# RaphaelHaddad/Real-Time-Brain-Inspired-Video-Memory

Measured on NVIDIA B200. Metric: queries_per_sec_top10_384d, higher is better.
Workload: dtype tf32

## Files before the change

### real-time-brain-inspired-video-memory_b200/csrc/api.cu

```cuda
#include "common.cuh"

#include <dlfcn.h>
#include <stdarg.h>
#include <stdlib.h>
#include <string.h>
#include <time.h>
#include <new>
#include <vector>

namespace vm {

static thread_local char g_err[512] = "";
void set_error(const char *fmt, ...)
{
    va_list ap;
    va_start(ap, fmt);
    vsnprintf(g_err, sizeof(g_err), fmt, ap);
    va_end(ap);
}

int k_convert_rows(const void *src, int src_dtype, void *dst, int dst_dtype, int64_t n, int dim, int ld, cudaStream_t st);
int k_row_inv_norms(const void *rows, int dtype, float *inv_norms, int64_t row0, int64_t n, int ld, int *extreme, cudaStream_t st,
                    const double *exact = nullptr);
int k_invalidate_rows(float *inv_norms, const int64_t *rows_dev, int64_t n, int64_t size, cudaStream_t st);
int k_normalize_queries(const void *q, int q_dtype, int nq, int nq_pad, int dim, int ld, float *out_f32, void *out_bf16,
                        int32_t *zero_me, uint32_t *zero_tab, int zero_tab_n, int tf32_round, int split, bool pdl, cudaStream_t st);
int k_synth_fill(void *rows, int dtype, uint64_t seed, int64_t row0, int64_t n, int dim, int ld, uint64_t dup_period,
                 cudaStream_t st);
int k_merge_candidates(const uint64_t *cand, int lists, int nq, int kp, uint64_t *merged, cudaStream_t st);

int k_slab_top(const SelectArgs &sa, int nq, int kp, uint64_t *merged, int *incomplete, cudaStream_t st);
int k_rescore(const RescoreArgs &a, cudaStream_t st, const int *incomplete);
int k_select_rescore(const SelectArgs &sa, const RescoreArgs &a, cudaStream_t st, bool pdl);
bool select_rescore_fits(int lists, int list_len, int kp, int dtype, int dim, int ld);
int k_collect_rescore(const uint64_t *buf, const int *cnt, int cap, const RescoreArgs &a, cudaStream_t st);
int k_exact(const ExactArgs &a, cudaStream_t st, bool pdl);
int k_merge_topk_lists(const void *idx, const void *score, const void *count, size_t stride_bytes, int lists, int nq, int k,
                       int64_t *out_idx, double *out_score, int32_t *out_count, cudaStream_t st);
int k_p2p_publish(void *flag, unsigned long long gen, cudaStream_t st);
int k_merge_topk_p2p(void *const *peers, int nranks, size_t slot_off, size_t flag_off, unsigned long long gen, int nq, int k,
                     int64_t *out_idx, double *out_score, int32_t *out_count, cudaStream_t st);
int k_merge_max_by_id(const int64_t *idx, const double *score, const int32_t *count, int nq, int k, int k2,
                      int64_t *out_idx, double *out_score, int32_t *out_count, cudaStream_t st);
int k_cosine_pairs(const void *a, const void *b, int dtype, int64_t n, int dim, int zero_rule, int sum_mode, double *out,
                   cudaStream_t st);
int k_pairs_above(int device, const void *x, int dtype, int64_t n, int dim, int ld, float threshold, int64_t cap,
                  int64_t *out_i, int64_t *out_j, float *out_score, int64_t *out_count, int part, int nparts, int flags,
                  cudaStream_t st);
int k_pairs_concat(const void *gathered, size_t per_rank_bytes, int64_t slot, const int64_t *counts, int nranks, int64_t cap,
                   int64_t *out_i, int64_t *out_j, float *out_score, int64_t *out_count, cudaStream_t st);

struct Arena;
int arena_create(Arena **out, int device, size_t max_bytes);
int arena_grow(Arena *a, size_t bytes);
void arena_destroy(Arena *a);
void *arena_base(const Arena *a);
size_t arena_mapped(const Arena *a);

static constexpr int MAXQ = 64;
static constexpr int MAXK = 64;
static constexpr int XCTAS = 148;
static constexpr int MAX_DEVICES = 64;
static constexpr int COLLECT_CAP = 4096;
static constexpr int FLAG_INTERNAL_CAPTURE = 1 << 30;

struct ResultBlock {
    int64_t *idx;
    double *score;
    int32_t *count;
    static ResultBlock at(void *base, int nq, int k)
    {
        char *b = (char *)base;
        return {(int64_t *)b, (double *)(b + (size_t)nq * k * 8), (int32_t *)(b + (size_t)nq * k * 16)};
    }
    ResultBlock from(int q0, int k) const { return {idx + (size_t)q0 * k, score + (size_t)q0 * k, count + q0}; }
};
static constexpr size_t result_bytes(int nq, int k) { return (size_t)nq * k * 16 + (size_t)nq * 4; }
static constexpr size_t packed_bytes(int nq, int k) { return (result_bytes(nq, k) + 7) & ~(size_t)7; }

static void unpack_to_host(const void *pack, int nq, int k, const ResultBlock &out)
{
    const ResultBlock p = ResultBlock::at(const_cast<void *>(pack), nq, k);
    memcpy(out.idx, p.idx, (size_t)nq * k * 8);
    memcpy(out.score, p.score, (size_t)nq * k * 8);
    memcpy(out.count, p.count, (size_t)nq * 4);
}

struct DeviceGuard {
    int prev = -1;
    bool ok = true;
    explicit DeviceGuard(int dev)
    {
        if (cudaGetDevice(&prev) != cudaSuccess) { ok = false; return; }
        if (prev != dev && cudaSetDevice(dev) != cudaSuccess) ok = false;
    }
    ~DeviceGuard() { if (prev >= 0) cudaSetDevice(prev); }
};

struct Buf {
    void *p = nullptr;
    size_t bytes = 0;
    int ensure(size_t need)
    {
        if (need <= bytes) return VM_OK;
        if (p) cudaFree(p);
        p = nullptr; bytes = 0;
        cudaError_t e = cudaMalloc(&p, need);
        if (e != cudaSuccess) { set_error("cudaMalloc(%zu) failed: %s", need, cudaGetErrorString(e)); return VM_ERR_OOM; }
        bytes = need;
        return VM_OK;
    }
    void release() { if (p) cudaFree(p); p = nullptr; bytes = 0; }
};

struct Workspace {
    bool ready = false;
    int lists_max = 0;
    Buf q_raw, q_f32, q_bf16, seed, cand, merged, o_idx, flags, col_thr, col_cnt, col_buf, xs, xr, xc, taken, gather_send, gather_recv, misc, ubuf, done, scnt, sel_inc;
    int32_t *h_uncert = nullptr;
    unsigned char *h_pack = nullptr;
    unsigned char *h_q = nullptr;
    void release()
    {
        Buf *all[] = {&q_raw, &q_f32, &q_bf16, &seed, &cand, &merged, &o_idx, &flags, &col_thr, &col_cnt, &col_buf, &xs, &xr, &xc, &taken,
                      &gather_send, &gather_recv, &misc, &ubuf, &done, &scnt, &sel_inc};
        for (Buf *b : all) b->release();
        if (h_uncert) cudaFreeHost(h_uncert);
        if (h_pack) cudaFreeHost(h_pack);
        if (h_q) cudaFreeHost(h_q);
        h_uncert = nullptr; h_pack = nullptr; h_q = nullptr;
        ready = false;
    }
};

}

using namespace vm;

struct vm_store {
    int device = 0, dim = 0, ld = 0, dtype = VM_F32, sm_count = 148;
    int64_t capacity = 0, size = 0;
    void *rows = nullptr;
    float *inv_norms = nullptr;
    double *rows_exact = nullptr;
    bool owns = false;
    Arena *ar_rows = nullptr, *ar_inv = nullptr, *ar_exact = nullptr;
    int64_t max_capacity = 0;
    const void *exact_rows() const { return rows_exact ? (const void *)rows_exact : (const void *)rows; }
    int exact_dtype() const { return rows_exact ? (int)VM_F64 : dtype; }
    int *extreme = nullptr;
    unsigned long long *cum = nullptr;
    int64_t n_batches = 0, n_queries = 0;
    int last_band_ctas = 0, last_band_nq = 0;
    Buf stage, stage_idx;
    Workspace ws;
    static constexpr int EV_RING = 64;
    cudaEvent_t evr[EV_RING][2] = {};
    int ev_next = 0;
    int ev_pending = 0;
    int ev_cur = -1;
    bool timed = false;
    struct GraphEntry {
        cudaGraphExec_t exec = nullptr;
        uint64_t version = 0;
        int nq = 0, k = 0, flags = 0, score_mode = 0, sum_mode = 0, q_dtype = 0;
        double min_score = 0.0;
        int64_t row_offset = 0;
        vm_topk_stats stats{};
    };
    GraphEntry graphs[4];
    int graph_next = 0;
    uint64_t version = 1;
    uint64_t seen_version = 0;
    int stable_calls = 0;
    cudaStream_t gstream = nullptr;
};

static constexpr size_t XCHG_SLOT_BYTES = (result_bytes(MAXQ, MAXK) + 255) & ~(size_t)255;
static constexpr size_t XCHG_FLAG_OFF = 2 * XCHG_SLOT_BYTES;
static constexpr size_t XCHG_BYTES = XCHG_FLAG_OFF + 256;

struct vm_comm {
    void *nccl = nullptr;
    int nranks = 1, rank = 0, device = 0;
    void *peer[16] = {};
    bool p2p = false;
    unsigned long long gen = 0;
    Buf pl_i, pl_j, pl_s, pl_cnt, pg_cnt, pg_send, pg_recv;
    int64_t *h_counts = nullptr;
};

struct Id128 { char b[128]; };
namespace {
struct NcclApi {
    void *h = nullptr;
    int (*GetUniqueId)(void *) = nullptr;
    int (*CommInitRank)(void **, int,  Id128, int) = nullptr;
    int (*AllGather)(const void *, void *, size_t, int, void *, cudaStream_t) = nullptr;
    int (*Broadcast)(const void *, void *, size_t, int, int, void *, cudaStream_t) = nullptr;
    int (*CommDestroy)(void *) = nullptr;
    const char *(*GetErrorString)(int) = nullptr;
};
}
static NcclApi g_nccl;

static int nccl_load()
{
    if (g_nccl.h) return VM_OK;
    void *h = dlopen("libnccl.so.2", RTLD_NOW | RTLD_GLOBAL);
    if (!h) h = dlopen("libnccl.so", RTLD_NOW | RTLD_GLOBAL);
    VM_REQUIRE(h, VM_ERR_NCCL, "cannot load libnccl.so.2: %s", dlerror());
    g_nccl.GetUniqueId = (int (*)(void *))dlsym(h, "ncclGetUniqueId");
    g_nccl.CommInitRank = (int (*)(void **, int, Id128, int))dlsym(h, "ncclCommInitRank");
    g_nccl.AllGather = (int (*)(const void *, void *, size_t, int, void *, cudaStream_t))dlsym(h, "ncclAllGather");
    g_nccl.Broadcast = (int (*)(const void *, void *, size_t, int, int, void *, cudaStream_t))dlsym(h, "ncclBroadcast");
    g_nccl.CommDestroy = (int (*)(void *))dlsym(h, "ncclCommDestroy");
    g_nccl.GetErrorString = (const char *(*)(int))dlsym(h, "ncclGetErrorString");
    VM_REQUIRE(g_nccl.GetUniqueId && g_nccl.CommInitRank && g_nccl.AllGather && g_nccl.Broadcast && g_nccl.CommDestroy, VM_ERR_NCCL,
               "libnccl lacks a required symbol");
    g_nccl.h = h;
    return VM_OK;
}
#define VM_NCCL_CHECK(expr)                                                                            \
    do {                                                                                               \
        int _r = (expr);                                                                               \
        if (_r != 0) {                                                                                 \
            set_error("%s failed: %s", #expr, g_nccl.GetErrorString ? g_nccl.GetErrorString(_r) : "?"); \
            return VM_ERR_NCCL;                                                                        \
        }                                                                                              \
    } while (0)

static int check_arch(int device, int *sm_count)
{
    cudaDeviceProp p;
    VM_CUDA_CHECK(cudaGetDeviceProperties(&p, device));
    VM_REQUIRE(p.major == 10, VM_ERR_UNSUPPORTED, "device %d is sm_%d%d; libvidmem is built for sm_100a only", device,
               p.major, p.minor);
    if (sm_count) *sm_count = p.multiProcessorCount;
    return VM_OK;
}

static int ws_prepare(vm_store *s)
{
    Workspace &w = s->ws;
    if (w.ready) return VM_OK;
    int lists = 2 * s->sm_count;
    w.lists_max = lists;
    int rc;
#define ENS(b, bytes) if ((rc = (b).ensure(bytes)) != VM_OK) return rc
    ENS(w.q_raw, (size_t)MAXQ * s->dim * 8);
    ENS(w.q_f32, (size_t)MAXQ * s->ld * 4);
    ENS(w.q_bf16, (size_t)2 * MAXQ * s->ld * 2);
    ENS(w.cand, (size_t)lists * MAXQ * (MAXK > SCAN_SLAB ? MAXK : SCAN_SLAB) * 8);
    ENS(w.merged, (size_t)MAXQ * MAXK * 8);
    ENS(w.o_idx, result_bytes(MAXQ, MAXK) + 64);
    ENS(w.flags, (size_t)(MAXQ + 2) * 4);
    ENS(w.seed, (size_t)(SEED_TAB_WORDS + 3 * MAXQ) * 4);
    ENS(w.ubuf, (size_t)MAXQ * SCAN_UNION_CAP * 8);
    ENS(w.done, 64);
    ENS(w.scnt, (size_t)256 * MAXQ * 4);
    ENS(w.sel_inc, (size_t)MAXQ * 4);
    VM_CUDA_CHECK(cudaMemset(w.done.p, 0, 64));
    ENS(w.col_thr, (size_t)MAXQ * 4);
    ENS(w.col_cnt, (size_t)MAXQ * 4);
    ENS(w.col_buf, (size_t)MAXQ * COLLECT_CAP * 8);
    ENS(w.xs, (size_t)XCTAS * MAXQ * MAXK * 8);
    ENS(w.xr, (size_t)XCTAS * MAXQ * MAXK * 4);
    ENS(w.xc, (size_t)XCTAS * MAXQ * 4);
    ENS(w.taken, (size_t)MAXQ * XCTAS * MAXK);
#undef ENS
    VM_CUDA_CHECK(cudaMallocHost((void **)&w.h_uncert, 64));
    VM_CUDA_CHECK(cudaMallocHost((void **)&w.h_pack, result_bytes(MAXQ, MAXK) + 64));
    VM_CUDA_CHECK(cudaMallocHost((void **)&w.h_q, (size_t)MAXQ * s->dim * 8));
    w.ready = true;
    return VM_OK;
}

static double scan_eps_stored(int kernel, int store_dtype, int dim, int split);
static double scan_eps(int kernel, int store_dtype, int dim, int split, bool shadow = false)
{
    const double base = scan_eps_stored(kernel, store_dtype, dim, split);
    if (!shadow) return base;
    return base + (store_dtype == VM_F32 ? 1.1920928955078125e-07 : 1.953125e-3 * 1.01);
}
static double scan_eps_stored(int kernel, int store_dtype, int dim, int split)
{
    const double u = 1.1920928955078125e-07;
    const double fp32_acc = (double)(dim + 16) * u;
    if (kernel == 1) return fp32_acc;
    if (store_dtype == VM_F32)
        return 9.765625e-4 + 4.8828125e-4 + 1e-6 + fp32_acc;
    if (!split) return 3.90625e-3 + fp32_acc;
    return 1.52587890625e-5 * 1.01 + (double)(dim + dim / 8 + 32) * u;
}

extern "C" int vm_version(void) { return VM_ABI_VERSION; }
extern "C" const char *vm_last_error(void) { return g_err; }

extern "C" int vm_device_info(int device, int *sm_count, int *cc_major, int *cc_minor, size_t *total_mem)
{
    cudaDeviceProp p;
    VM_CUDA_CHECK(cudaGetDeviceProperties(&p, device));
    if (sm_count) *sm_count = p.multiProcessorCount;
    if (cc_major) *cc_major = p.major;
    if (cc_minor) *cc_minor = p.minor;
    if (total_mem) *total_mem = p.totalGlobalMem;
    return VM_OK;
}

extern "C" int vm_ld(int dim) { return ld_for_dim(dim); }

static int store_new(vm_store **out, int device, int dim, int dtype, int64_t capacity)
{
    VM_REQUIRE(out, VM_ERR_BADARG, "out is NULL");
    VM_REQUIRE(dim >= 1 && dim <= 4096, VM_ERR_BADARG, "dim %d outside [1, 4096]", dim);
    VM_REQUIRE(dtype == VM_F32 || dtype == VM_BF16, VM_ERR_BADARG, "store dtype must be VM_F32 or VM_BF16");
    VM_REQUIRE(capacity >= 1 && capacity < 0xFFFFFFFFLL, VM_ERR_BADARG, "capacity %lld outside [1, 2^32-2]", (long long)capacity);
    int sms = 0;
    int rc = check_arch(device, &sms);
    if (rc != VM_OK) return rc;
    vm_store *s = new (std::nothrow) vm_store();
    VM_REQUIRE(s, VM_ERR_OOM, "host allocation failed");
    s->device = device; s->dim = dim; s->ld = ld_for_dim(dim); s->dtype = dtype; s->capacity = capacity; s->sm_count = sms;
    {
        DeviceGuard g(device);
        if (cudaMalloc((void **)&s->extreme, 4) != cudaSuccess || cudaMemset(s->extreme, 0, 4) != cudaSuccess ||
            cudaMalloc((void **)&s->cum, 64) != cudaSuccess || cudaMemset(s->cum, 0, 64) != cudaSuccess) {
            set_error("store allocation failed");
            vm_store_destroy(s);
            return VM_ERR_OOM;
        }
    }
    *out = s;
    return VM_OK;
}

extern "C" int vm_store_create(vm_store **out, int device, int dim, int dtype, int64_t capacity)
{
    int rc = store_new(out, device, dim, dtype, capacity);
    if (rc != VM_OK) return rc;
    vm_store *s = *out;
    DeviceGuard g(device);
    s->owns = true;
    size_t bytes = (size_t)capacity * s->ld * dtype_size(dtype);
    cudaError_t e = cudaMalloc(&s->rows, bytes);
    if (e == cudaSuccess) e = cudaMalloc((void **)&s->inv_norms, (size_t)capacity * 4);
    if (e != cudaSuccess) {
        set_error("store allocation of %zu bytes failed: %s", bytes, cudaGetErrorString(e));
        vm_store_destroy(s);
        *out = nullptr;
        return VM_ERR_OOM;
    }
    return VM_OK;
}

extern "C" int vm_store_create_exact(vm_store **out, int device, int dim, int shadow_dtype, int64_t capacity)
{
    int rc = vm_store_create(out, device, dim, shadow_dtype, capacity);
    if (rc != VM_OK) return rc;
    vm_store *s = *out;
    DeviceGuard g(device);
    const size_t bytes = (size_t)capacity * s->ld * 8;
    cudaError_t e = cudaMalloc((void **)&s->rows_exact, bytes);
    if (e != cudaSuccess) {
        set_error("store allocation of %zu bytes (binary64 rows) failed: %s", bytes, cudaGetErrorString(e));
        vm_store_destroy(s);
        *out = nullptr;
        return VM_ERR_OOM;
    }
    return VM_OK;
}

static int store_back(vm_store *s, int64_t capacity)
{
    int rc = arena_grow(s->ar_rows, (size_t)capacity * s->ld * dtype_size(s->dtype));
    if (rc == VM_OK) rc = arena_grow(s->ar_inv, (size_t)capacity * 4);
    if (rc == VM_OK && s->ar_exact) rc = arena_grow(s->ar_exact, (size_t)capacity * s->ld * 8);
    return rc;
}

extern "C" int vm_store_create_growable(vm_store **out, int device, int dim, int dtype, int exact, int64_t initial_capacity,
                                        int64_t max_capacity)
{
    VM_REQUIRE(initial_capacity >= 1 && max_capacity >= initial_capacity, VM_ERR_BADARG, "need 1 <= initial_capacity <= max_capacity");
    int rc = store_new(out, device, dim, dtype, max_capacity);
    if (rc != VM_OK) return rc;
    vm_store *s = *out;
    DeviceGuard g(device);
    s->max_capacity = max_capacity;
    s->capacity = initial_capacity;
    rc = arena_create(&s->ar_rows, device, (size_t)max_capacity * s->ld * dtype_size(dtype));
    if (rc == VM_OK) rc = arena_create(&s->ar_inv, device, (size_t)max_capacity * 4);
    if (rc == VM_OK && exact) rc = arena_create(&s->ar_exact, device, (size_t)max_capacity * s->ld * 8);
    if (rc == VM_OK) rc = store_back(s, initial_capacity);
    if (rc != VM_OK) { vm_store_destroy(s); *out = nullptr; return rc; }
    s->rows = arena_base(s->ar_rows);
    s->inv_norms = (float *)arena_base(s->ar_inv);
    if (exact) s->rows_exact = (double *)arena_base(s->ar_exact);
    return VM_OK;
}

extern "C" int vm_store_reserve(vm_store *s, int64_t capacity)
{
    VM_REQUIRE(s, VM_ERR_BADARG, "store is NULL");
    if (capacity <= s->capacity) return VM_OK;
    VM_REQUIRE(s->ar_rows, VM_ERR_STATE, "store is not growable (created over fixed buffers of %lld rows)", (long long)s->capacity);
    VM_REQUIRE(capacity <= s->max_capacity, VM_ERR_OVERFLOW, "capacity %lld exceeds the reserved maximum %lld", (long long)capacity,
               (long long)s->max_capacity);
    DeviceGuard g(s->device);
    int rc = store_back(s, capacity);
    if (rc != VM_OK) return rc;
    s->capacity = capacity;
    return VM_OK;
}

extern "C" int64_t vm_store_max_capacity(const vm_store *s) { return s ? (s->ar_rows ? s->max_capacity : s->capacity) : -1; }
extern "C" void *vm_store_rows_ptr(const vm_store *s) { return s ? s->rows : nullptr; }
extern "C" float *vm_store_inv_norms_ptr(const vm_store *s) { return s ? s->inv_norms : nullptr; }
extern "C" double *vm_store_rows_exact_ptr(const vm_store *s) { return s ? s->rows_exact : nullptr; }
extern "C" size_t vm_store_resident_bytes(const vm_store *s)
{
    if (!s) return 0;
    if (s->ar_rows) return arena_mapped(s->ar_rows) + arena_mapped(s->ar_inv) + (s->ar_exact ? arena_mapped(s->ar_exact) : 0);
    return (size_t)s->capacity * ((size_t)s->ld * (dtype_size(s->dtype) + (s->rows_exact ? 8 : 0)) + 4);
}

extern "C" int vm_store_attach_exact(vm_store **out, int device, int dim, int shadow_dtype, int64_t capacity, void *rows_dev,
                                     float *inv_norms_dev, double *rows_exact_dev)
{
    VM_REQUIRE(rows_exact_dev && ((uintptr_t)rows_exact_dev & 15) == 0, VM_ERR_BADARG, "binary64 rows buffer must be 16-byte aligned");
    int rc = vm_store_attach(out, device, dim, shadow_dtype, capacity, rows_dev, inv_norms_dev);
    if (rc != VM_OK) return rc;
    (*out)->rows_exact = rows_exact_dev;
    return VM_OK;
}

extern "C" int vm_store_attach(vm_store **out, int device, int dim, int dtype, int64_t capacity, void *rows_dev,
                               float *inv_norms_dev)
{
    VM_REQUIRE(rows_dev && inv_norms_dev, VM_ERR_BADARG, "attach needs device buffers");
    VM_REQUIRE(((uintptr_t)rows_dev & 127) == 0, VM_ERR_BADARG, "rows buffer must be 128-byte aligned");
    int rc = store_new(out, device, dim, dtype, capacity);
    if (rc != VM_OK) return rc;
    (*out)->rows = rows_dev;
    (*out)->inv_norms = inv_norms_dev;
    (*out)->owns = false;
    return VM_OK;
}

extern "C" int vm_store_destroy(vm_store *s)
{
    if (!s) return VM_OK;
    DeviceGuard g(s->device);
    cudaDeviceSynchronize();
    if (s->owns) { cudaFree(s->rows); cudaFree(s->inv_norms); if (s->rows_exact) cudaFree(s->rows_exact); }
    arena_destroy(s->ar_rows); arena_destroy(s->ar_inv); arena_destroy(s->ar_exact);
    if (s->extreme) cudaFree(s->extreme);
    if (s->cum) cudaFree(s->cum);
    s->stage.release(); s->stage_idx.release();
    s->ws.release();
    for (auto &pr : s->evr) { if (pr[0]) cudaEventDestroy(pr[0]); if (pr[1]) cudaEventDestroy(pr[1]); }
    for (auto &ge : s->graphs) if (ge.exec) cudaGraphExecDestroy(ge.exec);
    if (s->gstream) cudaStreamDestroy(s->gstream);
    delete s;
    return VM_OK;
}

extern "C" int64_t vm_store_size(const vm_store *s) { return s ? s->size : -1; }
extern "C" int64_t vm_store_capacity(const vm_store *s) { return s ? s->capacity : -1; }
extern "C" int vm_store_dim(const vm_store *s) { return s ? s->dim : -1; }
extern "C" int vm_store_ld(const vm_store *s) { return s ? s->ld : -1; }

static int store_write(vm_store *s, int64_t row0, const void *rows, int src_dtype, int src_mem, int64_t n, cudaStream_t st)
{
    VM_REQUIRE(src_dtype == VM_F32 || src_dtype == VM_BF16 || src_dtype == VM_F64, VM_ERR_BADARG, "bad source dtype");
    if (n == 0) return VM_OK;
    VM_REQUIRE(rows, VM_ERR_BADARG, "rows is NULL");
    DeviceGuard g(s->device);
    const void *src = rows;
    if (src_mem == VM_MEM_HOST) {
        size_t bytes = (size_t)n * s->dim * dtype_size(src_dtype);
        int rc = s->stage.ensure(bytes);
        if (rc != VM_OK) return rc;
        VM_CUDA_CHECK(cudaMemcpyAsync(s->stage.p, rows, bytes, cudaMemcpyHostToDevice, st));
        src = s->stage.p;
    }
    char *dst = (char *)s->rows + (size_t)row0 * s->ld * dtype_size(s->dtype);
    int rc = k_convert_rows(src, src_dtype, dst, s->dtype, n, s->dim, s->ld, st);
    if (rc != VM_OK) return rc;
    if (s->rows_exact) {
        rc = k_convert_rows(src, src_dtype, s->rows_exact + (size_t)row0 * s->ld, VM_F64, n, s->dim, s->ld, st);
        if (rc != VM_OK) return rc;
    }
    return k_row_inv_norms(s->rows, s->dtype, s->inv_norms, row0, row0 + n, s->ld, s->extreme, st, s->rows_exact);
}

extern "C" int vm_store_append(vm_store *s, const void *rows, int src_dtype, int src_mem, int64_t n, int64_t *first_row,
                               void *stream)
{
    VM_REQUIRE(s, VM_ERR_BADARG, "store is NULL");
    VM_REQUIRE(n >= 0, VM_ERR_BADARG, "n < 0");
    if (s->ar_rows && s->size + n > s->capacity) {
        const int64_t row_bytes = (int64_t)s->ld * (int64_t)(dtype_size(s->dtype) + (s->rows_exact ? 8 : 0)) + 4;
        const int64_t slack_rows = ((int64_t)256 << 20) / row_bytes + 1;
        int64_t want = s->size + n + slack_rows;
        if (want > s->max_capacity) want = s->max_capacity;
        if (want >= s->size + n) {
            int rc = vm_store_reserve(s, want);
            if (rc != VM_OK && want > s->size + n) rc = vm_store_reserve(s, s->size + n);
            if (rc != VM_OK) return rc;
        }
    }
    VM_REQUIRE(s->size + n <= s->capacity, VM_ERR_OVERFLOW, "append of %lld rows exceeds capacity %lld (size %lld)",
               (long long)n, (long long)s->capacity, (long long)s->size);
    int rc = store_write(s, s->size, rows, src_dtype, src_mem, n, (cudaStream_t)stream);
    if (rc != VM_OK) return rc;
    if (first_row) *first_row = s->size;
    s->size += n;
    ++s->version;
    return VM_OK;
}

extern "C" int vm_store_update(vm_store *s, int64_t row0, const void *rows, int src_dtype, int src_mem, int64_t n, void *stream)
{
    VM_REQUIRE(s, VM_ERR_BADARG, "store is NULL");
    VM_REQUIRE(row0 >= 0 && n >= 0 && row0 + n <= s->size, VM_ERR_BADARG, "update range [%lld, %lld) outside [0, %lld)",
               (long long)row0, (long long)(row0 + n), (long long)s->size);
    ++s->version;
    return store_write(s, row0, rows, src_dtype, src_mem, n, (cudaStream_t)stream);
}

extern "C" int vm_store_invalidate(vm_store *s, const int64_t *rows_host, int64_t n, void *stream)
{
    VM_REQUIRE(s, VM_ERR_BADARG, "store is NULL");
    if (n <= 0) return VM_OK;
    VM_REQUIRE(rows_host, VM_ERR_BADARG, "rows is NULL");
    DeviceGuard g(s->device);
    int rc = s->stage_idx.ensure((size_t)n * 8);
    if (rc != VM_OK) return rc;
    VM_CUDA_CHECK(cudaMemcpyAsync(s->stage_idx.p, rows_host, (size_t)n * 8, cudaMemcpyHostToDevice, (cudaStream_t)stream));
    ++s->version;
    return k_invalidate_rows(s->inv_norms, (const int64_t *)s->stage_idx.p, n, s->size, (cudaStream_t)stream);
}

extern "C" int vm_store_set_size(vm_store *s, int64_t n, int64_t recompute_from_row, void *stream)
{
    VM_REQUIRE(s, VM_ERR_BADARG, "store is NULL");
    VM_REQUIRE(n >= 0 && n <= s->capacity, VM_ERR_BADARG, "size %lld outside [0, capacity]", (long long)n);
    DeviceGuard g(s->device);
    s->size = n;
    ++s->version;
    if (recompute_from_row >= 0 && recompute_from_row < n) {
        if (s->rows_exact) {
            const int64_t r0 = recompute_from_row;
            int rc = k_convert_rows((const char *)s->rows + (size_t)r0 * s->ld * dtype_size(s->dtype), s->dtype,
                                    s->rows_exact + (size_t)r0 * s->ld, VM_F64, n - r0, s->ld, s->ld, (cudaStream_t)stream);
            if (rc != VM_OK) return rc;
        }
        return k_row_inv_norms(s->rows, s->dtype, s->inv_norms, recompute_from_row, n, s->ld, s->extreme, (cudaStream_t)stream, s->rows_exact);
    }
    return VM_OK;
}

extern "C" int vm_store_last_scan_ms(vm_store *s, float *ms)
{
    VM_REQUIRE(s && ms, VM_ERR_BADARG, "NULL argument");
    VM_REQUIRE(s->timed, VM_ERR_STATE, "no vm_topk call with VM_FLAG_TIMING has run the scan kernel yet");
    DeviceGuard g(s->device);
    VM_CUDA_CHECK(cudaEventSynchronize(s->evr[s->ev_cur][1]));
    VM_CUDA_CHECK(cudaEventElapsedTime(ms, s->evr[s->ev_cur][0], s->evr[s->ev_cur][1]));
    return VM_OK;
}

extern "C" int vm_store_avg_scan_ms(vm_store *s, float *ms, int *calls)
{
    VM_REQUIRE(s && ms, VM_ERR_BADARG, "NULL argument");
    VM_REQUIRE(s->timed && s->ev_pending > 0, VM_ERR_STATE, "no vm_topk call with VM_FLAG_TIMING since the last read");
    DeviceGuard g(s->device);
    VM_CUDA_CHECK(cudaEventSynchronize(s->evr[s->ev_cur][1]));
    double sum = 0.0;
    const int n = s->ev_pending;
    for (int i = 0; i < n; ++i) {
        const int slot = (s->ev_cur - i + 2 * vm_store::EV_RING) % vm_store::EV_RING;
        float t = 0.0f;
        VM_CUDA_CHECK(cudaEventElapsedTime(&t, s->evr[slot][0], s->evr[slot][1]));
        sum += t;
    }
    *ms = (float)(sum / n);
    if (calls) *calls = n;
    s->ev_pending = 0;
    return VM_OK;
}

extern "C" int vm_store_band_keys(vm_store *s, int nq_cap, int64_t *kept_per_query, int64_t *spilled_per_query, int *nq_out)
{
    VM_REQUIRE(s && kept_per_query && spilled_per_query, VM_ERR_BADARG, "NULL argument");
    VM_REQUIRE(s->ws.ready && s->last_band_ctas > 0, VM_ERR_STATE, "the last top-k call of this store was not a band-keeping tcgen05 scan");
    const int ctas = s->last_band_ctas, nq = s->last_band_nq;
    VM_REQUIRE(nq_cap >= nq, VM_ERR_BADARG, "room for %d queries needed", nq);
    DeviceGuard g(s->device);
    VM_CUDA_CHECK(cudaDeviceSynchronize());
    std::vector<int> sc((size_t)ctas * nq), uc(nq);
    VM_CUDA_CHECK(cudaMemcpy(sc.data(), s->ws.scnt.p, sc.size() * 4, cudaMemcpyDeviceToHost));
    VM_CUDA_CHECK(cudaMemcpy(uc.data(), (int *)s->ws.seed.p + SEED_TAB_WORDS + 2 * MAXQ, (size_t)nq * 4, cudaMemcpyDeviceToHost));
    for (int q = 0; q < nq; ++q) {
        int64_t k = 0;
        for (int c = 0; c < ctas; ++c) k += sc[(size_t)c * nq + q];
        kept_per_query[q] = k;
        spilled_per_query[q] = uc[q];
    }
    if (nq_out) *nq_out = nq;
    return VM_OK;
}

extern "C" int vm_store_read_counters(vm_store *s, vm_store_counters *out, int reset)
{
    VM_REQUIRE(s && out, VM_ERR_BADARG, "NULL argument");
    DeviceGuard g(s->device);
    unsigned long long h[8] = {0, 0, 0, 0, 0, 0, 0, 0};
    VM_CUDA_CHECK(cudaMemcpy(h, s->cum, sizeof(h), cudaMemcpyDeviceToHost));
    out->batches = s->n_batches; out->queries = s->n_queries;
    out->uncertified = (int64_t)h[0]; out->band_settled = (int64_t)h[1]; out->collect_settled = (int64_t)h[2];
    out->full_rescans = (int64_t)h[3];
    out->bound_violations = (int64_t)h[4];
    if (reset) {
        VM_CUDA_CHECK(cudaMemset(s->cum, 0, sizeof(h)));
        s->n_batches = 0; s->n_queries = 0;
    }
    return VM_OK;
}

extern "C" int vm_store_clear(vm_store *s)
{
    VM_REQUIRE(s, VM_ERR_BADARG, "store is NULL");
    DeviceGuard g(s->device);
    VM_CUDA_CHECK(cudaMemset(s->extreme, 0, 4));
    s->size = 0;
    ++s->version;
    return VM_OK;
}

extern "C" size_t vm_topk_packed_bytes(int nq, int k) { return nq > 0 && k > 0 ? packed_bytes(nq, k) : 0; }

namespace {
struct TopkCall {
    vm_store *s;
    const void *queries;
    int q_dtype, q_mem, nq, k;
    double min_score;
    int score_mode, sum_mode, flags;
    int64_t row_offset;
    ResultBlock d;
    cudaStream_t st;
    vm_topk_stats *stats;
    ResultBlock h = {};
};
}

static cudaError_t wait_stream(cudaStream_t st, const vm_store *s = nullptr)
{
    static const bool block = [] { const char *e = getenv("VIDMEM_SYNC"); return e && !strcmp(e, "block"); }();
    if (block) return cudaStreamSynchronize(st);
    if (s) {
        const double est_us = (double)s->size * s->ld * (double)dtype_size(s->dtype) / 6.5e6;
        if (est_us > 400.0) {
            struct timespec ts;
            const long ns = (long)(est_us * 750.0);
            ts.tv_sec = ns / 1000000000L; ts.tv_nsec = ns % 1000000000L;
            nanosleep(&ts, nullptr);
        }
    }
    for (;;) {
        const cudaError_t e = cudaStreamQuery(st);
        if (e != cudaErrorNotReady) return e;
#if defined(__x86_64__) || defined(__i386__)
        __builtin_ia32_pause();
#endif
    }
}

static int pack_out_enqueue(const TopkCall &c)
{
    VM_CUDA_CHECK(cudaMemcpyAsync(c.s->ws.h_pack, c.d.idx, result_bytes(c.nq, c.k), cudaMemcpyDeviceToHost, c.st));
    return VM_OK;
}

static int tc_list_len(int k) { return k <= 16 ? 32 : (k <= 48 ? 64 : 0); }

static int queries_per_pass(const vm_store *s, int k, int flags)
{
    const int kp = tc_list_len(k);
    if (!(flags & (VM_FLAG_FORCE_EXACT | VM_FLAG_FORCE_SIMT)) && kp)
        for (int nq = 64; nq >= 16; nq -= 16)
            if (scan_tc_supported(s->dtype, s->dim, nq, kp)) return nq;
    return MAXQ;
}

static int topk_batch(const TopkCall &c)
{
    vm_store *s = c.s;
    Workspace &w = s->ws;
    cudaStream_t st = c.st;
    const void *q_dev = c.queries;
    if (c.q_mem == VM_MEM_HOST) {
        const size_t qbytes = (size_t)c.nq * s->dim * dtype_size(c.q_dtype);
        memcpy(w.h_q, c.queries, qbytes);
        VM_CUDA_CHECK(cudaMemcpyAsync(w.q_raw.p, w.h_q, qbytes, cudaMemcpyHostToDevice, st));
        q_dev = w.q_raw.p;
    }
    FinalizeArgs fin{c.k, c.min_score, c.score_mode, c.row_offset, c.d.idx, c.d.score, c.d.count};
    ExactArgs ex{s->exact_rows(), s->inv_norms, s->exact_dtype(), s->ld, s->dim, s->size, q_dev, c.q_dtype, c.nq, c.k, c.sum_mode,
                 nullptr, (double *)w.xs.p, (uint32_t *)w.xr.p, (int32_t *)w.xc.p, (uint8_t *)w.taken.p, XCTAS, fin, s->cum,
                 (int *)w.done.p};
    if (!(c.flags & FLAG_INTERNAL_CAPTURE)) { ++s->n_batches; s->n_queries += c.nq; }
    int launches = 0;
    if (c.stats) { c.stats->uncertified = 0; c.stats->candidates = 0; c.stats->scan_ctas = 0; }

    int kernel = 0, kp = 0;
    if (!(c.flags & VM_FLAG_FORCE_EXACT) && s->size > 0) {
        int kp_tc = tc_list_len(c.k);
        int kp_simt = c.k <= 24 ? (c.k + 8 > 16 ? ((c.k + 8 + 7) & ~7) : 16) : 0;
        bool tc_ok = kp_tc > 0 && scan_tc_supported(s->dtype, s->dim, c.nq, kp_tc);
        bool want_tc = !(c.flags & VM_FLAG_FORCE_SIMT);
        if (want_tc && tc_ok) { kernel = 2; kp = kp_tc; }
        else if (kp_simt > 0) { kernel = 1; kp = kp_simt; }
        else if (tc_ok) { kernel = 2; kp = kp_tc; }
    }
    if (kernel == 0) {
        int rc = k_exact(ex, st, false);
        if (rc != VM_OK) return rc;
        launches += 2;
        if (c.h.idx) {
            if ((rc = pack_out_enqueue(c)) != VM_OK) return rc;
            VM_CUDA_CHECK(wait_stream(st, s));
            unpack_to_host(w.h_pack, c.nq, c.k, c.h);
        }
        if (c.stats) { c.stats->scan_kernel = 0; c.stats->scan_launches += launches; }
        return VM_OK;
    }

    int nq_pad = kernel == 2 ? ((c.nq + 15) & ~15) : c.nq;
    const int split = (kernel == 2 && s->dtype == VM_BF16 && !(c.flags & VM_FLAG_NO_SPLIT) &&
                       (c.nq <= 48 || (c.flags & VM_FLAG_SPLIT)) && scan_tc_supported(s->dtype, s->dim, c.nq, kp, 1)) ? 1 : 0;
#ifdef VIDMEM_NO_GRAPH_PDL
    const bool pdl = !(c.flags & (VM_FLAG_TIMING | FLAG_INTERNAL_CAPTURE));
#else
    const bool pdl = !(c.flags & VM_FLAG_TIMING);
#endif
    int rc = k_normalize_queries(q_dev, c.q_dtype, c.nq, nq_pad, s->dim, s->ld, (float *)w.q_f32.p,
                                 (kernel == 2 && s->dtype == VM_BF16) ? w.q_bf16.p : nullptr,
                                 (int32_t *)w.flags.p + c.nq, kernel == 2 ? (uint32_t *)w.seed.p : nullptr,
                                 kernel == 2 ? (int)(w.seed.bytes / 4) : 0, kernel == 2 && s->dtype == VM_F32, split, pdl, st);
    if (rc != VM_OK) return rc;
    ++launches;
    const double eps = scan_eps(kernel, s->dtype, s->dim, split, s->rows_exact != nullptr);

    ScanArgs a;
    ScanInfo sinfo;
    a.rows = s->rows; a.inv_norms = s->inv_norms; a.dtype = s->dtype; a.n = s->size; a.dim = s->dim; a.ld = s->ld;
    a.queries = (const float *)w.q_f32.p; a.nq = c.nq; a.kp = kp; a.cand = (uint64_t *)w.cand.p; a.stream = st;
    a.slab = (uint64_t *)w.cand.p; a.scnt = (int *)w.scnt.p;
    a.ubuf = (uint64_t *)w.ubuf.p; a.ucnt = (int *)w.seed.p + SEED_TAB_WORDS + 2 * MAXQ; a.ucap = SCAN_UNION_CAP;
    a.band = nextafterf((float)(2.0 * eps), INFINITY); a.ksel = c.k; a.split = split; a.pdl = pdl;
    const bool timing = (c.flags & VM_FLAG_TIMING) != 0;
    if (timing) {
        s->ev_cur = s->ev_next;
        s->ev_next = (s->ev_next + 1) % vm_store::EV_RING;
        if (s->ev_pending < vm_store::EV_RING) ++s->ev_pending;
        if (!s->evr[s->ev_cur][0]) { VM_CUDA_CHECK(cudaEventCreate(&s->evr[s->ev_cur][0])); VM_CUDA_CHECK(cudaEventCreate(&s->evr[s->ev_cur][1])); }
        VM_CUDA_CHECK(cudaEventRecord(s->evr[s->ev_cur][0], st));
    }
    if (kernel == 1) {
        int64_t need = (s->size + 31) / 32;
        a.ctas = (int)imin64(need, 2 * s->sm_count);
        rc = launch_scan_simt(a);
        launches += (c.nq + 7) / 8;
    } else {
        int64_t tiles = (s->size + 127) / 128;
        a.ctas = (int)imin64(tiles, s->sm_count);

        a.dump = tiles <= s->sm_count && tiles * SCAN_DUMP_TILE <= SCAN_DUMP_MAX_KEYS &&
                 (size_t)tiles * c.nq * SCAN_DUMP_TILE * 8 <= w.cand.bytes &&
                 select_rescore_fits((int)tiles, SCAN_DUMP_TILE, kp, s->exact_dtype(), s->dim, s->ld);
        s->last_band_ctas = a.dump ? 0 : a.ctas; s->last_band_nq = c.nq;
        rc = launch_scan_tc(a, s->dtype == VM_BF16 ? w.q_bf16.p : w.q_f32.p, (uint32_t *)w.seed.p, (int *)w.flags.p + c.nq + 1, nullptr, &sinfo);
        launches += 1;
    }
    if (rc != VM_OK) return rc;
    if (timing) { VM_CUDA_CHECK(cudaEventRecord(s->evr[s->ev_cur][1], st)); s->timed = true; }

    int32_t *flags = (int32_t *)w.flags.p;
    int32_t *uncert = flags + c.nq;
    RescoreArgs rs{(const uint64_t *)w.merged.p, kp, s->exact_rows(), s->inv_norms, s->exact_dtype(), s->ld, s->dim, s->size, q_dev,
                   c.q_dtype, c.nq, eps, c.sum_mode, fin, flags, uncert, s->extreme,
                   kernel == 2 ? (float *)w.col_thr.p : nullptr, s->cum};
    SelectArgs sel;
    const bool union_src = kernel == 2 && !a.dump;
    if (union_src) {
        sel.slab = a.slab; sel.scnt = a.scnt; sel.ctas = a.ctas; sel.ubuf = a.ubuf; sel.ucnt = a.ucnt; sel.ucap = a.ucap;
        sel.seed_tab = a.ctas <= 256 ? (const uint32_t *)w.seed.p : nullptr; sel.nq_pad = nq_pad; sel.ksel = c.k; sel.band = a.band;
    } else { sel.cand = a.cand; sel.lists = a.ctas; sel.list_len = a.dump ? SCAN_DUMP_TILE : kp; sel.complete = a.dump ? 1 : 0; }
    rc = k_select_rescore(sel, rs, st, pdl);
    if (rc == VM_ERR_UNSUPPORTED && !a.dump) {
        if (union_src) rc = k_slab_top(sel, c.nq, kp, (uint64_t *)w.merged.p, (int *)w.sel_inc.p, st);
        else rc = k_merge_candidates(a.cand, a.ctas, c.nq, kp, (uint64_t *)w.merged.p, st);
        if (rc != VM_OK) return rc;
        rc = k_rescore(rs, st, union_src ? (const int *)w.sel_inc.p : nullptr);
        ++launches;
    }
    if (rc != VM_OK) return rc;
    launches += 1;

    ex.flags = flags;
    int n_uncert = 0, n_full = -1;
    auto run_collect = [&]() -> int {
        VM_CUDA_CHECK(cudaMemsetAsync(w.col_cnt.p, 0, (size_t)c.nq * 4, st));
        ScanCollect sc{(const float *)w.col_thr.p, (uint64_t *)w.col_buf.p, (int *)w.col_cnt.p, COLLECT_CAP, uncert};
        int r = launch_scan_tc(a, s->dtype == VM_BF16 ? w.q_bf16.p : w.q_f32.p, nullptr, nullptr, &sc);
        if (r != VM_OK) return r;
        return k_collect_rescore((const uint64_t *)w.col_buf.p, (const int *)w.col_cnt.p, COLLECT_CAP, rs, st);
    };
    if (c.flags & VM_FLAG_ASYNC) {
        if (c.flags & FLAG_INTERNAL_CAPTURE) {
            VM_CUDA_CHECK(cudaMemcpyAsync(w.h_uncert, uncert, 4, cudaMemcpyDeviceToHost, st));
        } else {
            rc = k_exact(ex, st, pdl);
            if (rc != VM_OK) return rc;
            launches += 1;
        }
        n_uncert = -1;
    } else {
        VM_CUDA_CHECK(cudaMemcpyAsync(w.h_uncert, uncert, 4, cudaMemcpyDeviceToHost, st));
        if (c.h.idx && (rc = pack_out_enqueue(c)) != VM_OK) return rc;
        VM_CUDA_CHECK(wait_stream(st, s));
        n_uncert = *w.h_uncert;
        n_full = 0;
        if (n_uncert > 0) {
            int left = n_uncert;
            if (kernel == 2) {
                if ((rc = run_collect()) != VM_OK) return rc;
                launches += 2;
                VM_CUDA_CHECK(cudaMemcpyAsync(w.h_uncert, uncert, 4, cudaMemcpyDeviceToHost, st));
                VM_CUDA_CHECK(wait_stream(st, s));
                left = *w.h_uncert;
            }
            n_full = left;
            if (left > 0) {
                rc = k_exact(ex, st, false);
                if (rc != VM_OK) return rc;
                launches += 1;
            }
            if (c.h.idx) {
                if ((rc = pack_out_enqueue(c)) != VM_OK) return rc;
                VM_CUDA_CHECK(wait_stream(st, s));
            }
        }
        if (c.h.idx) unpack_to_host(w.h_pack, c.nq, c.k, c.h);
    }
    if (c.stats) {
        c.stats->scan_kernel = kernel;
        c.stats->scan_launches += launches;
        c.stats->uncertified += n_uncert > 0 ? n_uncert : 0;
        c.stats->full_rescans = n_full;
        c.stats->candidates = kp;
        c.stats->scan_ctas = a.ctas;
        c.stats->scan_stages = kernel == 2 ? sinfo.stages : 0;
        c.stats->scan_variant = kernel == 2 ? sinfo.variant : 0;
    }
    return VM_OK;
}

static constexpr int GRAPH_SKIPPED = 1;

static int graph_capture(const TopkCall &c, vm_store::GraphEntry *ge)
{
    vm_store *s = c.s;
    Workspace &w = s->ws;
    vm_topk_stats cs{};
    TopkCall cc = c;
    cc.queries = w.q_raw.p; cc.q_mem = VM_MEM_DEVICE; cc.flags |= VM_FLAG_ASYNC | FLAG_INTERNAL_CAPTURE;
    cc.d = ResultBlock::at(w.o_idx.p, c.nq, c.k); cc.st = s->gstream; cc.stats = &cs;
    const size_t qbytes = (size_t)c.nq * s->dim * dtype_size(c.q_dtype);
    cudaGraph_t graph = nullptr;
    VM_CUDA_CHECK(cudaStreamBeginCapture(s->gstream, cudaStreamCaptureModeRelaxed));
    int rc = VM_OK;
    if (cudaMemcpyAsync(w.q_raw.p, w.h_q, qbytes, cudaMemcpyHostToDevice, s->gstream) != cudaSuccess) rc = VM_ERR_CUDA;
    if (rc == VM_OK) rc = topk_batch(cc);
    if (rc == VM_OK && cudaMemcpyAsync(w.h_pack, cc.d.idx, result_bytes(c.nq, c.k), cudaMemcpyDeviceToHost, s->gstream) != cudaSuccess)
        rc = VM_ERR_CUDA;
    cudaError_t ce = cudaStreamEndCapture(s->gstream, &graph);
    if (rc != VM_OK || ce != cudaSuccess || !graph) {
        if (graph) cudaGraphDestroy(graph);
        if (rc == VM_OK) { set_error("graph capture failed: %s", cudaGetErrorString(ce)); rc = VM_ERR_CUDA; }
        cudaGetLastError();
        return rc;
    }
    ce = cudaGraphInstantiate(&ge->exec, graph, 0);
    cudaGraphDestroy(graph);
    if (ce != cudaSuccess) { ge->exec = nullptr; set_error("cudaGraphInstantiate failed: %s", cudaGetErrorString(ce)); return VM_ERR_CUDA; }
    ge->version = s->version; ge->nq = c.nq; ge->k = c.k; ge->flags = c.flags; ge->score_mode = c.score_mode;
    ge->sum_mode = c.sum_mode; ge->q_dtype = c.q_dtype; ge->min_score = c.min_score; ge->row_offset = c.row_offset; ge->stats = cs;
    return VM_OK;
}

static int topk_graph(const TopkCall &c, int out_mem, bool sharded, const ResultBlock &out)
{
    vm_store *s = c.s;
    Workspace &w = s->ws;
    static const bool no_graph = getenv("VIDMEM_NO_GRAPH") != nullptr;
    if (s->seen_version == s->version) { if (s->stable_calls < 1 << 20) ++s->stable_calls; }
    else { s->seen_version = s->version; s->stable_calls = 0; }
    if (no_graph || s->stable_calls < 16 || sharded || c.st != nullptr || c.q_mem != VM_MEM_HOST || out_mem != VM_MEM_HOST ||
        (c.flags & (VM_FLAG_ASYNC | VM_FLAG_TIMING | VM_FLAG_FORCE_EXACT)) || s->size == 0 ||
        c.nq > queries_per_pass(s, c.k, c.flags))
        return GRAPH_SKIPPED;
    if (!s->gstream) VM_CUDA_CHECK(cudaStreamCreate(&s->gstream));
    vm_store::GraphEntry *ge = nullptr;
    for (auto &e : s->graphs)
        if (e.exec && e.version == s->version && e.nq == c.nq && e.k == c.k && e.flags == c.flags && e.score_mode == c.score_mode &&
            e.sum_mode == c.sum_mode && e.q_dtype == c.q_dtype && e.row_offset == c.row_offset &&
            memcmp(&e.min_score, &c.min_score, sizeof(double)) == 0) { ge = &e; break; }
    if (!ge) {
        ge = &s->graphs[s->graph_next];
        s->graph_next = (s->graph_next + 1) & 3;
        if (ge->exec) { cudaGraphExecDestroy(ge->exec); ge->exec = nullptr; }
        const int rc = graph_capture(c, ge);
        if (rc != VM_OK) return rc;
    }
    memcpy(w.h_q, c.queries, (size_t)c.nq * s->dim * dtype_size(c.q_dtype));
    ++s->n_batches; s->n_queries += c.nq;
    VM_CUDA_CHECK(cudaGraphLaunch(ge->exec, s->gstream));
    VM_CUDA_CHECK(wait_stream(s->gstream, s));
    const int uncertified = ge->stats.scan_kernel != 0 ? *w.h_uncert : 0;
    if (uncertified > 0) {
        TopkCall rerun = c;
        rerun.d = ResultBlock::at(w.o_idx.p, c.nq, c.k); rerun.st = s->gstream; rerun.h = out;
        return topk_batch(rerun);
    }
    unpack_to_host(w.h_pack, c.nq, c.k, out);
    if (c.stats) { *c.stats = ge->stats; c.stats->uncertified = uncertified; }
    return VM_OK;
}

static size_t xchg_slot_off(unsigned long long gen) { return (size_t)(gen & 1) * XCHG_SLOT_BYTES; }

static ResultBlock batch_dest(vm_store *s, const vm_comm *comm, bool sharded, int out_mem, const ResultBlock &out, int nb, int k)
{
    if (sharded && comm->p2p) return ResultBlock::at((char *)comm->peer[comm->rank] + xchg_slot_off(comm->gen), nb, k);
    if (sharded) return ResultBlock::at(s->ws.gather_send.p, nb, k);
    return out_mem == VM_MEM_DEVICE ? out : ResultBlock::at(s->ws.o_idx.p, nb, k);
}

static int exchange_merge(vm_store *s, vm_comm *comm, int nb, int k, const ResultBlock &m, cudaStream_t st)
{
    if (comm->p2p) {
        const int rc = k_p2p_publish((char *)comm->peer[comm->rank] + XCHG_FLAG_OFF, comm->gen, st);
        if (rc != VM_OK) return rc;
        return k_merge_topk_p2p(comm->peer, comm->nranks, xchg_slot_off(comm->gen), XCHG_FLAG_OFF, comm->gen, nb, k, m.idx, m.score,
                                m.count, st);
    }
    const Workspace &w = s->ws;
    VM_NCCL_CHECK(g_nccl.AllGather(w.gather_send.p, w.gather_recv.p, packed_bytes(nb, k),  0, comm->nccl, st));
    const ResultBlock r = ResultBlock::at(w.gather_recv.p, nb, k);
    return k_merge_topk_lists(r.idx, r.score, r.count, packed_bytes(nb, k), comm->nranks, nb, k, m.idx, m.score, m.count, st);
}

static int topk_common(vm_store *s, vm_comm *comm, int64_t row_offset, const void *queries, int q_dtype, int q_mem, int nq,
                       int k, double min_score, int score_mode, int sum_mode, int flags, int64_t *out_idx,
                       double *out_score, int32_t *out_count, int out_mem, vm_topk_stats *stats, void *stream)
{
    VM_REQUIRE(s, VM_ERR_BADARG, "store is NULL");
    VM_REQUIRE(nq >= 0, VM_ERR_BADARG, "nq < 0");
    VM_REQUIRE(k >= 1 && k <= MAXK, VM_ERR_BADARG, "k %d outside [1, %d]", k, MAXK);
    VM_REQUIRE(q_dtype == VM_F32 || q_dtype == VM_BF16 || q_dtype == VM_F64, VM_ERR_BADARG, "bad query dtype");
    VM_REQUIRE(score_mode == VM_SCORE_RAW || score_mode == VM_SCORE_NEO4J, VM_ERR_BADARG, "bad score_mode");
    VM_REQUIRE(sum_mode == VM_SUM_NAIVE || sum_mode == VM_SUM_NEUMAIER, VM_ERR_BADARG, "bad sum_mode");
    VM_REQUIRE(!(flags & VM_FLAG_ASYNC) || (out_mem == VM_MEM_DEVICE && q_mem == VM_MEM_DEVICE), VM_ERR_BADARG,
               "VM_FLAG_ASYNC needs device queries and device outputs");
    if (stats) memset(stats, 0, sizeof(*stats));
    if (nq == 0) return VM_OK;
    VM_REQUIRE(queries && out_idx && out_score && out_count, VM_ERR_BADARG, "NULL buffer");
    DeviceGuard g(s->device);
    VM_REQUIRE(g.ok, VM_ERR_CUDA, "cannot select device %d", s->device);
    int rc = ws_prepare(s);
    if (rc != VM_OK) return rc;
    const bool sharded = comm && comm->nranks > 1;
    const ResultBlock out{out_idx, out_score, out_count};
    const TopkCall call{s, queries, q_dtype, q_mem, nq, k, min_score, score_mode, sum_mode, flags, row_offset, {}, (cudaStream_t)stream,
                        stats};
    if ((rc = topk_graph(call, out_mem, sharded, out)) != GRAPH_SKIPPED) return rc;

    Workspace &w = s->ws;
    const int bq = queries_per_pass(s, k, flags);
    for (int q0 = 0; q0 < nq; q0 += bq) {
        const int nb = nq - q0 < bq ? nq - q0 : bq;
        const ResultBlock out_b = out.from(q0, k);
        if (sharded && comm->p2p) {
            ++comm->gen;
        } else if (sharded) {
            if ((rc = w.gather_send.ensure(packed_bytes(nb, k))) != VM_OK) return rc;
            if ((rc = w.gather_recv.ensure(packed_bytes(nb, k) * comm->nranks)) != VM_OK) return rc;
        }
        TopkCall c = call;
        c.queries = (const char *)queries + (size_t)q0 * s->dim * dtype_size(q_dtype);
        c.nq = nb;
        c.d = batch_dest(s, comm, sharded, out_mem, out_b, nb, k);
        if (out_mem == VM_MEM_HOST) {
            if (sharded) c.flags |= VM_FLAG_ASYNC;
            else c.h = out_b;
        }
        if ((rc = topk_batch(c)) != VM_OK) return rc;
        if (!sharded) continue;
        const ResultBlock ws = ResultBlock::at(w.o_idx.p, nb, k);
        if ((rc = exchange_merge(s, comm, nb, k, out_mem == VM_MEM_DEVICE ? out_b : ws, c.st)) != VM_OK) return rc;
        if (stats) stats->scan_launches += 2;
        if (out_mem == VM_MEM_HOST) {
            VM_CUDA_CHECK(cudaMemcpyAsync(w.h_pack, ws.idx, result_bytes(nb, k), cudaMemcpyDeviceToHost, c.st));
            VM_CUDA_CHECK(wait_stream(c.st, s));
            unpack_to_host(w.h_pack, nb, k, out_b);
        }
    }
    return VM_OK;
}

extern "C" int vm_topk(vm_store *s, const void *queries, int q_dtype, int q_mem, int nq, int k, double min_score,
                       int score_mode, int sum_mode, int flags, int64_t *out_idx, double *out_score, int32_t *out_count,
                       int out_mem, vm_topk_stats *stats, void *stream)
{
    return topk_common(s, nullptr, 0, queries, q_dtype, q_mem, nq, k, min_score, score_mode, sum_mode, flags, out_idx,
                       out_score, out_count, out_mem, stats, stream);
}

extern "C" int vm_topk_sharded(vm_store *s, vm_comm *comm, int64_t row_offset, const void *queries, int q_dtype, int q_mem,
                               int nq, int k, double min_score, int score_mode, int sum_mode, int flags, int64_t *out_idx,
                               double *out_score, int32_t *out_count, int out_mem, vm_topk_stats *stats, void *stream)
{
    VM_REQUIRE(comm, VM_ERR_BADARG, "comm is NULL");
    return topk_common(s, comm, row_offset, queries, q_dtype, q_mem, nq, k, min_score, score_mode, sum_mode, flags, out_idx,
                       out_score, out_count, out_mem, stats, stream);
}

extern "C" int vm_merge_topk_lists(int device, const int64_t *idx_dev, const double *score_dev, const int32_t *count_dev,
                                   int nlists, int nq, int k, int64_t *out_idx_dev, double *out_score_dev,
                                   int32_t *out_count_dev, void *stream)
{
    VM_REQUIRE(idx_dev && score_dev && count_dev && out_idx_dev && out_score_dev && out_count_dev, VM_ERR_BADARG, "NULL buffer");
    VM_REQUIRE(nlists >= 1 && nq >= 1 && k >= 1, VM_ERR_BADARG, "bad shape");
    DeviceGuard g(device);
    size_t stride = (size_t)nq * k * 8;
    VM_REQUIRE(device >= 0 && device < MAX_DEVICES, VM_ERR_BADARG, "device index %d outside [0, %d)", device, MAX_DEVICES);
    static thread_local Buf cnt_wide_dev[MAX_DEVICES];
    Buf &cnt_wide = cnt_wide_dev[device];
    int rc = cnt_wide.ensure(stride * nlists);
    if (rc != VM_OK) return rc;
    VM_CUDA_CHECK(cudaMemcpy2DAsync(cnt_wide.p, stride, count_dev, (size_t)nq * 4, (size_t)nq * 4, nlists,
                                    cudaMemcpyDeviceToDevice, (cudaStream_t)stream));
    return k_merge_topk_lists(idx_dev, score_dev, cnt_wide.p, stride, nlists, nq, k, out_idx_dev, out_score_dev,
                              out_count_dev, (cudaStream_t)stream);
}

extern "C" int vm_merge_topk_packed(int device, const void *packed_dev, int nlists, int nq, int k, int64_t *out_idx_dev,
                                    double *out_score_dev, int32_t *out_count_dev, void *stream)
{
    VM_REQUIRE(packed_dev && out_idx_dev && out_score_dev && out_count_dev, VM_ERR_BADARG, "NULL buffer");
    VM_REQUIRE(nlists >= 1 && nq >= 1 && k >= 1, VM_ERR_BADARG, "bad shape");
    DeviceGuard g(device);
    const ResultBlock r = ResultBlock::at(const_cast<void *>(packed_dev), nq, k);
    return k_merge_topk_lists(r.idx, r.score, r.count, packed_bytes(nq, k), nlists, nq, k, out_idx_dev, out_score_dev,
                              out_count_dev, (cudaStream_t)stream);
}

extern "C" int vm_merge_max_by_id(int device, const int64_t *idx_dev, const double *score_dev, const int32_t *count_dev,
                                  int nq, int k, int k2, int64_t *out_idx_dev, double *out_score_dev, int32_t *out_count_dev,
                                  void *stream)
{
    VM_REQUIRE(idx_dev && score_dev && count_dev && out_idx_dev && out_score_dev && out_count_dev, VM_ERR_BADARG, "NULL buffer");
    VM_REQUIRE(nq >= 1 && k >= 1 && k2 >= 1, VM_ERR_BADARG, "bad shape");
    DeviceGuard g(device);
    return k_merge_max_by_id(idx_dev, score_dev, count_dev, nq, k, k2, out_idx_dev, out_score_dev, out_count_dev,
                             (cudaStream_t)stream);
}

extern "C" int vm_cosine_pairs(int device, const void *a, const void *b, int dtype, int mem, int64_t n, int dim, int zero_rule,
                               int sum_mode, double *out, int out_mem, void *stream)
{
    VM_REQUIRE(n >= 0 && dim >= 0, VM_ERR_BADARG, "bad shape");
    VM_REQUIRE(dtype == VM_F32 || dtype == VM_F64, VM_ERR_BADARG, "dtype must be VM_F32 or VM_F64");
    VM_REQUIRE(zero_rule >= 0 && zero_rule <= 2, VM_ERR_BADARG, "zero_rule %d outside [0, 2]", zero_rule);
    if (n == 0) return VM_OK;
    VM_REQUIRE(a && b && out, VM_ERR_BADARG, "NULL buffer");
    int rc = check_arch(device, nullptr);
    if (rc != VM_OK) return rc;
    DeviceGuard g(device);
    cudaStream_t st = (cudaStream_t)stream;
    VM_REQUIRE(device >= 0 && device < MAX_DEVICES, VM_ERR_BADARG, "device index %d outside [0, %d)", device, MAX_DEVICES);
    static thread_local Buf scratch[MAX_DEVICES][3];
    Buf &da = scratch[device][0], &db = scratch[device][1], &dout = scratch[device][2];
    size_t bytes = (size_t)n * dim * dtype_size(dtype);
    const void *pa = a, *pb = b;
    if (mem == VM_MEM_HOST) {
        if ((rc = da.ensure(bytes ? bytes : 8)) != VM_OK || (rc = db.ensure(bytes ? bytes : 8)) != VM_OK) return rc;
        VM_CUDA_CHECK(cudaMemcpyAsync(da.p, a, bytes, cudaMemcpyHostToDevice, st));
        VM_CUDA_CHECK(cudaMemcpyAsync(db.p, b, bytes, cudaMemcpyHostToDevice, st));
        pa = da.p; pb = db.p;
    }
    double *po = out;
    if (out_mem == VM_MEM_HOST) {
        if ((rc = dout.ensure((size_t)n * 8)) != VM_OK) return rc;
        po = (double *)dout.p;
    }
    rc = k_cosine_pairs(pa, pb, dtype, n, dim, zero_rule, sum_mode, po, st);
    if (rc != VM_OK) return rc;
    if (out_mem == VM_MEM_HOST) {
        VM_CUDA_CHECK(cudaMemcpyAsync(out, po, (size_t)n * 8, cudaMemcpyDeviceToHost, st));
        VM_CUDA_CHECK(cudaStreamSynchronize(st));
    }
    return VM_OK;
}

extern "C" int vm_pairs_above(int device, const void *x_dev, int dtype, int64_t n, int dim, float threshold, int64_t cap,
                              int64_t *out_i_dev, int64_t *out_j_dev, float *out_score_dev, int64_t *out_count_dev, int part,
                              int nparts, int flags, void *stream)
{
    VM_REQUIRE(x_dev && out_count_dev, VM_ERR_BADARG, "NULL buffer");
    VM_REQUIRE(cap == 0 || (out_i_dev && out_j_dev && out_score_dev), VM_ERR_BADARG, "NULL output with cap > 0");
    VM_REQUIRE(dtype == VM_F32 || dtype == VM_BF16, VM_ERR_BADARG, "dtype must be VM_F32 or VM_BF16");
    VM_REQUIRE(n >= 0 && n < (1LL << 31), VM_ERR_BADARG, "n outside [0, 2^31)");
    VM_REQUIRE(dim >= 1 && dim <= 4096, VM_ERR_BADARG, "dim outside [1, 4096]");
    VM_REQUIRE(nparts >= 1 && part >= 0 && part < nparts, VM_ERR_BADARG, "bad part/nparts");
    int rc = check_arch(device, nullptr);
    if (rc != VM_OK) return rc;
    DeviceGuard g(device);
    return k_pairs_above(device, x_dev, dtype, n, dim, ld_for_dim(dim), threshold, cap, out_i_dev, out_j_dev, out_score_dev,
                         out_count_dev, part, nparts, flags, (cudaStream_t)stream);
}

extern "C" int vm_pairs_above_sharded(vm_comm *comm, void *x_dev, int dtype, int64_t n, int dim, float threshold, int64_t cap,
                                      int64_t *out_i_dev, int64_t *out_j_dev, float *out_score_dev, int64_t *out_count_dev,
                                      int root, int flags, void *stream)
{
    VM_REQUIRE(comm, VM_ERR_BADARG, "comm is NULL");
    VM_REQUIRE(x_dev && out_count_dev, VM_ERR_BADARG, "NULL buffer");
    VM_REQUIRE(cap >= 1 && out_i_dev && out_j_dev && out_score_dev, VM_ERR_BADARG, "cap < 1 or NULL output");
    VM_REQUIRE(dtype == VM_F32 || dtype == VM_BF16, VM_ERR_BADARG, "dtype must be VM_F32 or VM_BF16");
    VM_REQUIRE(n >= 0 && n < (1LL << 31), VM_ERR_BADARG, "n outside [0, 2^31)");
    VM_REQUIRE(dim >= 1 && dim <= 4096, VM_ERR_BADARG, "dim outside [1, 4096]");
    VM_REQUIRE(root >= -1 && root < comm->nranks, VM_ERR_BADARG, "root %d outside [-1, %d)", root, comm->nranks);
    int rc = check_arch(comm->device, nullptr);
    if (rc != VM_OK) return rc;
    DeviceGuard g(comm->device);
    cudaStream_t st = (cudaStream_t)stream;
    const int G = comm->nranks, ld = ld_for_dim(dim);
    if (root >= 0 && G > 1 && n > 0)
        VM_NCCL_CHECK(g_nccl.Broadcast(x_dev, x_dev, (size_t)n * ld * dtype_size(dtype),  0, root, comm->nccl, st));
#define ENS(b, bytes) if ((rc = (b).ensure(bytes)) != VM_OK) return rc
    ENS(comm->pl_i, (size_t)cap * 8); ENS(comm->pl_j, (size_t)cap * 8); ENS(comm->pl_s, (size_t)cap * 4);
    ENS(comm->pl_cnt, 8); ENS(comm->pg_cnt, (size_t)G * 8);
    if (!comm->h_counts) VM_CUDA_CHECK(cudaMallocHost((void **)&comm->h_counts, 16 * 8));
    rc = k_pairs_above(comm->device, x_dev, dtype, n, dim, ld, threshold, cap, (int64_t *)comm->pl_i.p, (int64_t *)comm->pl_j.p,
                       (float *)comm->pl_s.p, (int64_t *)comm->pl_cnt.p, comm->rank, G, 0, st);
    if (rc != VM_OK) return rc;
    VM_NCCL_CHECK(g_nccl.AllGather(comm->pl_cnt.p, comm->pg_cnt.p, 8,  0, comm->nccl, st));
    int64_t slot = cap;
// ... 98 lines not shown
```

### real-time-brain-inspired-video-memory_b200/csrc/common.cuh

```cuda
#pragma once
#include <cuda_runtime.h>
#include <cuda_bf16.h>
#include <stdint.h>
#include <stdio.h>
#include <math.h>
#include <utility>
#include "../../include/vidmem.h"

namespace vm {

void set_error(const char *fmt, ...);
#define VM_CUDA_CHECK(expr)                                                                      \
    do {                                                                                         \
        cudaError_t _e = (expr);                                                                 \
        if (_e != cudaSuccess) {                                                                 \
            vm::set_error("%s failed: %s (%s:%d)", #expr, cudaGetErrorString(_e), __FILE__, __LINE__); \
            return VM_ERR_CUDA;                                                                  \
        }                                                                                        \
    } while (0)
#define VM_REQUIRE(cond, code, ...)          \
    do {                                     \
        if (!(cond)) {                       \
            vm::set_error(__VA_ARGS__);      \
            return (code);                   \
        }                                    \
    } while (0)

__device__ __forceinline__ void pdl_wait() { asm volatile("griddepcontrol.wait;" ::: "memory"); }
__device__ __forceinline__ void pdl_launch_dependents() { asm volatile("griddepcontrol.launch_dependents;" ::: "memory"); }

template <typename... KArgs, typename... Args>
static inline cudaError_t launch_pdl(void (*kernel)(KArgs...), dim3 grid, dim3 block, size_t smem, cudaStream_t st, bool pdl,
                                     Args &&...args)
{
    cudaLaunchConfig_t cfg = {};
    cfg.gridDim = grid; cfg.blockDim = block; cfg.dynamicSmemBytes = smem; cfg.stream = st;
    cudaLaunchAttribute at[1];
    at[0].id = cudaLaunchAttributeProgrammaticStreamSerialization;
    at[0].val.programmaticStreamSerializationAllowed = 1;
    cfg.attrs = at;
    cfg.numAttrs = pdl ? 1 : 0;
    return cudaLaunchKernelEx(&cfg, kernel, std::forward<Args>(args)...);
}

template <auto Kernel>
static inline cudaError_t max_smem_once(int bytes)
{
    static bool set[64] = {};
    int dev = 0;
    cudaError_t e = cudaGetDevice(&dev);
    if (e != cudaSuccess || set[dev & 63]) return e;
    e = cudaFuncSetAttribute(Kernel, cudaFuncAttributeMaxDynamicSharedMemorySize, bytes);
    if (e == cudaSuccess) set[dev & 63] = true;
    return e;
}

__host__ __device__ __forceinline__ uint32_t f32_ordered(float f)
{
#ifdef __CUDA_ARCH__
    uint32_t b = __float_as_uint(f);
#else
    uint32_t b;
    memcpy(&b, &f, 4);
#endif
    return (b & 0x80000000u) ? ~b : (b | 0x80000000u);
}
__host__ __device__ __forceinline__ float f32_from_ordered(uint32_t o)
{
    uint32_t b = (o & 0x80000000u) ? (o & 0x7FFFFFFFu) : ~o;
#ifdef __CUDA_ARCH__
    return __uint_as_float(b);
#else
    float f;
    memcpy(&f, &b, 4);
    return f;
#endif
}
__host__ __device__ __forceinline__ uint64_t make_key(float score, uint32_t row)
{
    return ((uint64_t)f32_ordered(score) << 32) | (uint64_t)(0xFFFFFFFFu - row);
}
__host__ __device__ __forceinline__ uint32_t key_row(uint64_t k) { return 0xFFFFFFFFu - (uint32_t)(k & 0xFFFFFFFFu); }
__host__ __device__ __forceinline__ float key_score(uint64_t k) { return f32_from_ordered((uint32_t)(k >> 32)); }

static constexpr int SEED_TAB_WORDS = 256 * 64;
#ifdef __CUDACC__
__device__ __forceinline__ float seed_select(const uint32_t *seed_tab, int G, int nq_pad, int q, int k, int lane)
{
    uint32_t vals[8];
#pragma unroll
    for (int t = 0; t < 8; ++t) {
        const int i = lane + 32 * t;
        vals[t] = i < G ? __ldcg(seed_tab + (size_t)i * nq_pad + q) : 0u;
    }
    uint32_t prefix = 0;
    int need = k;
    for (int bit = 31; bit >= 16; --bit) {
        const uint32_t hi = bit == 31 ? 0u : (0xFFFFFFFFu << (bit + 1));
        int cnt = 0;
#pragma unroll
        for (int t = 0; t < 8; ++t) cnt += ((vals[t] & hi) == prefix && ((vals[t] >> bit) & 1u)) ? 1 : 0;
        const int tot = __reduce_add_sync(0xffffffffu, cnt);
        if (tot >= need) prefix |= 1u << bit;
        else need -= tot;
    }
    float sd = f32_from_ordered(prefix);
    if (!(sd > -INFINITY) || G < k) sd = -INFINITY;
    return sd;
}

__device__ __forceinline__ float band_floor(float L, float band)
{
    if (!(L > -INFINITY)) return -INFINITY;
    const float t = __fsub_rd(L, band);
    return nextafterf(t, -INFINITY);
}

#endif

struct RefSum {
    double s, c;
    __device__ __forceinline__ void init() { s = 0.0; c = 0.0; }
    template <bool NEUMAIER>
    __device__ __forceinline__ void add(double x)
    {
        double t = __dadd_rn(s, x);
        if (NEUMAIER) {
            const bool big = fabs(s) >= fabs(x);
            const double hi = big ? s : x, lo = big ? x : s;
            c = __dadd_rn(c, __dadd_rn(__dadd_rn(hi, -t), lo));
        }
        s = t;
    }
    template <bool NEUMAIER>
    __device__ __forceinline__ void add_block(const double (&x)[8])
    {
        double t[8];
        t[0] = __dadd_rn(s, x[0]);
#pragma unroll
        for (int u = 1; u < 8; ++u) t[u] = __dadd_rn(t[u - 1], x[u]);
        if (NEUMAIER) {
#pragma unroll
            for (int u = 0; u < 8; ++u) {
                const double prev = u ? t[u - 1] : s;
                const bool big = fabs(prev) >= fabs(x[u]);
                const double hi = big ? prev : x[u], lo = big ? x[u] : prev;
                c = __dadd_rn(c, __dadd_rn(__dadd_rn(hi, -t[u]), lo));
            }
        }
        s = t[7];
    }
    template <bool NEUMAIER>
    __device__ __forceinline__ double result() const
    {
        double r = s;
        if (NEUMAIER && c != 0.0 && isfinite(c)) r = __dadd_rn(r, c);
        return r;
    }
};

template <bool NEUMAIER, typename F>
__device__ __forceinline__ void ref_sum_range(RefSum &acc, int lo, int hi, F prod)
{
    int i = lo;
    for (; i + 8 <= hi; i += 8) {
        double x[8];
#pragma unroll
        for (int u = 0; u < 8; ++u) x[u] = prod(i + u);
        acc.add_block<NEUMAIER>(x);
    }
    for (; i < hi; ++i) acc.add<NEUMAIER>(prod(i));
}

__device__ __forceinline__ float load_as_float(const float *p, int64_t i) { return p[i]; }
__device__ __forceinline__ float load_as_float(const __nv_bfloat16 *p, int64_t i) { return __bfloat162float(p[i]); }
__device__ __forceinline__ double load_elem(const float *p, int64_t i) { return (double)p[i]; }
__device__ __forceinline__ double load_elem(const __nv_bfloat16 *p, int64_t i) { return (double)__bfloat162float(p[i]); }
__device__ __forceinline__ double load_elem(const double *p, int64_t i) { return p[i]; }
__device__ __forceinline__ double load_as_double(const void *p, int dtype, int64_t i)
{
    if (dtype == VM_F32) return (double)((const float *)p)[i];
    if (dtype == VM_BF16) return (double)__bfloat162float(((const __nv_bfloat16 *)p)[i]);
    return ((const double *)p)[i];
}

static inline int64_t imin64(int64_t a, int64_t b) { return a < b ? a : b; }
static inline int ld_for_dim(int dim) { return (dim + 7) & ~7; }
static inline size_t dtype_size(int dt) { return dt == VM_F32 ? 4 : dt == VM_BF16 ? 2 : 8; }

struct ScanArgs {
    const void *rows;
    const float *inv_norms;
    int dtype;
    int64_t n;
    int dim, ld;
    const float *queries;
    int nq;
    int kp;
    uint64_t *cand;
    int ctas;
    cudaStream_t stream;
    int dump = 0;
    uint64_t *slab = nullptr;
    int *scnt = nullptr;
    uint64_t *ubuf = nullptr;
    int *ucnt = nullptr;
    int ucap = 0;
    float band = 0.0f;
    int ksel = 0;
    int split = 0;
    bool pdl = false;
};
static constexpr int SCAN_UNION_CAP = 16384;
static constexpr int SCAN_SLAB = 128;
static constexpr int SELECT_KEY_CAP = 4096;
static constexpr int SCAN_DUMP_TILE = 128;
static constexpr int SCAN_DUMP_MAX_KEYS = 9472;
int launch_scan_simt(const ScanArgs &a);
int scan_simt_max_queries();
struct ScanCollect {
    const float *thr;
    uint64_t *buf;
    int *cnt;
    int cap;
    const int *pending;
};
struct ScanInfo { int stages = 0, variant = 0; };
int launch_scan_tc(const ScanArgs &a, const void *queries_store_dtype, uint32_t *seed_tab, int *seed_ctr,
                   const ScanCollect *sc = nullptr, ScanInfo *info = nullptr);
bool scan_tc_supported(int dtype, int dim, int nq, int kp, int split = 0);


struct FinalizeArgs {
    int k;
    double min_score;
    int score_mode;
    int64_t row_offset;
    int64_t *out_idx;
    double *out_score;
    int32_t *out_count;
};
struct RescoreArgs {
    const uint64_t *merged;
    int kp;
    const void *rows;
    const float *inv_norms;
    int dtype, ld, dim;
    int64_t n_rows;
    const void *queries;
    int q_dtype, nq;
    double eps;
    int sum_mode;
    FinalizeArgs fin;
    int32_t *flags, *uncertified_count;
    const int *extreme;
    float *collect_thr;
    unsigned long long *cum = nullptr;
};
struct SelectArgs {
    const uint64_t *cand = nullptr;
    int lists = 0, list_len = 0;
    int complete = 0;
    const uint64_t *slab = nullptr;
    const int *scnt = nullptr;
    int ctas = 0;
    const uint64_t *ubuf = nullptr;
    const int *ucnt = nullptr;
    int ucap = 0;
    const uint32_t *seed_tab = nullptr;
    int nq_pad = 0, ksel = 0;
    float band = 0.0f;
};
struct ExactArgs {
    const void *rows;
    const float *inv_norms;
    int dtype, ld, dim;
    int64_t n;
    const void *queries;
    int q_dtype, nq, k, sum_mode;
    int32_t *flags;
    double *xlist_score;
    uint32_t *xlist_row;
    int32_t *xlist_cnt;
    uint8_t *taken;
    int ctas;
    FinalizeArgs fin;
    unsigned long long *cum = nullptr;
    int *done_ctr = nullptr;
};

}
```

### real-time-brain-inspired-video-memory_b200/csrc/scan_tc.cu

```cuda
#include "tc_common.cuh"

namespace vm {
using namespace tc;

static constexpr int TC_BLOCK_M = 128;
static constexpr int TC_STAGE_BYTES = TC_BLOCK_M * 128;
static constexpr int TC_ACC = 8;
static constexpr int TC_THREADS_SVC = 288;
static constexpr int TC_THREADS = 192;
static constexpr int TC_TMEM_COLS = 512;
static constexpr int TC_MAX_STAGES = 8;

struct CollectArgs {
    const float *thr;
    uint64_t *buf;
    int *cnt;
    int cap;
    const int *pending;
};

struct BandArgs {
    uint64_t *slab;
    int *scnt;
    uint64_t *ubuf;
    int *ucnt;
    int ucap;
    float band;
    int ksel;
    int use_seed;
};

struct TcLayout {
    int nq_pad, KB, stages, split;
    uint32_t off_b, off_a, off_tauf, off_lcnt, off_cmax, off_wmax, off_flags, off_bars, off_tmem, total;
};

static TcLayout make_layout(int dtype, int ld, int nq, int split = 0)
{
    TcLayout L{};
    const int es = dtype == VM_F32 ? 4 : 2;
    L.nq_pad = (nq + 15) & ~15;
    L.KB = (ld * es + 127) / 128;
    L.split = (split && dtype == VM_BF16) ? 1 : 0;
    uint32_t o = 0;
    L.off_b = o; o += (uint32_t)L.KB * L.nq_pad * 128 * (L.split ? 2 : 1);
    const uint32_t epi = (uint32_t)L.nq_pad * (4 + 4 + 4 + 16) + 64 + 8 * (2 * TC_MAX_STAGES + 1 + 2 * TC_ACC) + 16;
    int64_t room = 227 * 1024 - 2048 - (int64_t)o - epi;
    L.stages = (int)(room / TC_STAGE_BYTES);
    if (L.stages > TC_MAX_STAGES) L.stages = TC_MAX_STAGES;
    if (L.stages < 0) L.stages = 0;
    L.off_a = o; o += (uint32_t)L.stages * TC_STAGE_BYTES;
    L.off_tauf = o; o += (uint32_t)L.nq_pad * 4;
    L.off_lcnt = o; o += (uint32_t)L.nq_pad * 4;
    L.off_cmax = o; o += (uint32_t)L.nq_pad * 4;
    L.off_wmax = o; o += (uint32_t)L.nq_pad * 16;
    L.off_flags = o; o += 64;
    L.off_bars = o; o += 8 * (2 * TC_MAX_STAGES + 1 + 2 * TC_ACC);
    L.off_tmem = o; o += 16;
    L.total = o + 1024;
#ifdef VIDMEM_AB_SMEMPAD
    if (L.total < 220 * 1024) L.total = 220 * 1024;
#endif
    return L;
}

__device__ __forceinline__ uint32_t own_kth_score(const uint64_t *slab, int n, int k, int lane)
{
    constexpr int PER = SCAN_SLAB / 32;
    uint32_t vals[PER];
#pragma unroll
    for (int t = 0; t < PER; ++t) {
        const int i = lane + 32 * t;
        vals[t] = i < n ? (uint32_t)(__ldcg(slab + i) >> 32) : 0u;
    }
    uint32_t prefix = 0;
    int need = k;
    for (int bit = 31; bit >= 12; --bit) {
        const uint32_t hi = bit == 31 ? 0u : (0xFFFFFFFFu << (bit + 1));
        int cnt = 0;
#pragma unroll
        for (int t = 0; t < PER; ++t) cnt += ((vals[t] & hi) == prefix && ((vals[t] >> bit) & 1u)) ? 1 : 0;
        const int tot = __reduce_add_sync(0xffffffffu, cnt);
        if (tot >= need) prefix |= 1u << bit;
        else need -= tot;
    }
    int ge = 0;
#pragma unroll
    for (int t = 0; t < PER; ++t) ge += (vals[t] != 0u && vals[t] >= prefix) ? 1 : 0;
    ge = __reduce_add_sync(0xffffffffu, ge);
    return (ge >= k && prefix != 0u) ? prefix : 0u;
}

template <bool TF32, bool DUMP, bool SPLIT>
__global__ void __launch_bounds__(DUMP ? TC_THREADS : TC_THREADS_SVC, 1)
scan_tc_kernel(const __grid_constant__ CUtensorMap tmA, const __grid_constant__ CUtensorMap tmB,
               const float *__restrict__ inv_norms, int64_t n, int num_tiles, int nq, TcLayout L, uint64_t *__restrict__ dump_keys,
               uint32_t *__restrict__ seed_tab, int *__restrict__ seed_ctr, CollectArgs col, BandArgs ub, int svc_sleep)
{
    const bool collect = !DUMP && col.thr != nullptr;
#ifndef VIDMEM_AB_NOPDL
    pdl_launch_dependents();
#endif
    if (collect) {
        pdl_wait();
        if (*col.pending == 0) return;
    }

    extern __shared__ __align__(16) uint8_t smem_raw[];
    uint8_t *base = smem_raw + ((1024u - (smem_u32(smem_raw) & 1023u)) & 1023u);
    uint8_t *sB = base + L.off_b;
    uint8_t *sA = base + L.off_a;
    float *tauf = (float *)(base + L.off_tauf);
    int *lcnt = (int *)(base + L.off_lcnt);
    uint32_t *cmax = (uint32_t *)(base + L.off_cmax);
    uint32_t *wmax = (uint32_t *)(base + L.off_wmax);
    volatile int *s_done = (volatile int *)(base + L.off_flags);
    uint64_t *bars = (uint64_t *)(base + L.off_bars);
    uint64_t *full = bars, *empty = bars + TC_MAX_STAGES, *qfull = bars + 2 * TC_MAX_STAGES;
    uint64_t *tfull = qfull + 1, *tempty = tfull + TC_ACC;
    uint32_t *tmem_slot = (uint32_t *)(base + L.off_tmem);

    const int warp = __shfl_sync(0xffffffffu, threadIdx.x >> 5, 0);
    const int lane = threadIdx.x & 31;
    const int nq_pad = L.nq_pad, KB = L.KB, stages = L.stages;
    constexpr int ELEMS = TF32 ? 32 : 64;

    if (warp == 0 && lane == 0) {
        tma_prefetch_desc(&tmA);
        tma_prefetch_desc(&tmB);
        for (int s = 0; s < stages; ++s) { mbar_init(&full[s], 1); mbar_init(&empty[s], 1); }
        mbar_init(qfull, 1);
        for (int a = 0; a < TC_ACC; ++a) { mbar_init(&tfull[a], 1); mbar_init(&tempty[a], 4); }
        fence_barrier_init();
    }
    if (warp == 1) tmem_alloc(tmem_slot, TC_TMEM_COLS);
#ifndef VIDMEM_AB_NOPDL
    if (!collect) pdl_wait();
#endif
    if (warp >= 2 && warp < 6) {
        const int e = threadIdx.x - 64;
        if (e < nq_pad) {
            lcnt[e] = 0;
            cmax[e] = 0u;
            tauf[e] = collect ? (e < nq ? col.thr[e] : INFINITY) : (e < nq ? -INFINITY : INFINITY);
        }
        if (e < 2) s_done[e] = 0;
    }
    tc_fence_before();
    __syncthreads();
    tc_fence_after();
    const uint32_t tmem_base = *tmem_slot;
    uint32_t *gbound = seed_tab ? seed_tab + SEED_TAB_WORDS : nullptr;

    if (warp == 0) {
        if (elect_one()) {
            constexpr int QPARTS = SPLIT ? 2 : 1;
            mbar_arrive_expect_tx(qfull, (uint32_t)(KB * QPARTS) * nq_pad * 128);
            for (int part = 0; part < QPARTS; ++part)
                for (int kb = 0; kb < KB; ++kb)
                    tma_load_2d(&tmB, qfull, sB + (size_t)(part * KB + kb) * nq_pad * 128, kb * ELEMS, part * nq_pad, L2_EVICT_LAST);
        }
        __syncwarp();
        int stage = 0;
        uint32_t phase = 0;
        for (int tile = blockIdx.x; tile < num_tiles; tile += gridDim.x) {
            for (int kb = 0; kb < KB; ++kb) {
                mbar_wait(&empty[stage], phase ^ 1);
                if (elect_one()) {
                    mbar_arrive_expect_tx(&full[stage], TC_STAGE_BYTES);
                    tma_load_2d(&tmA, &full[stage], sA + (size_t)stage * TC_STAGE_BYTES, kb * ELEMS, tile * TC_BLOCK_M, L2_EVICT_FIRST);
                }
                __syncwarp();
                if (++stage == stages) { stage = 0; phase ^= 1; }
            }
        }
    } else if (warp == 1) {
        const uint32_t idesc = make_idesc(TF32 ? 2u : 1u, TC_BLOCK_M, (uint32_t)nq_pad);
        mbar_wait(qfull, 0);
        tc_fence_after();
        int stage = 0, acc = 0;
        uint32_t phase = 0, acc_phase = 0;
        const uint64_t da0 = make_smem_desc_sw128(smem_u32(sA)), db0 = make_smem_desc_sw128(smem_u32(sB));
        const uint32_t kb_step = (uint32_t)(nq_pad * 128) >> 4, lo_step = (uint32_t)(KB * nq_pad * 128) >> 4;
        for (int tile = blockIdx.x; tile < num_tiles; tile += gridDim.x) {
            mbar_wait(&tempty[acc], acc_phase ^ 1);
            tc_fence_after();
            const uint32_t d_tmem = tmem_base + (uint32_t)(acc * nq_pad);
            for (int kb = 0; kb < KB; ++kb) {
                mbar_wait(&full[stage], phase);
                tc_fence_after();
                if (elect_one()) {
                    const uint64_t da = da0 + (uint64_t)((uint32_t)stage * (TC_STAGE_BYTES >> 4));
                    const uint64_t db = db0 + (uint64_t)((uint32_t)kb * kb_step);
#pragma unroll
                    for (int j = 0; j < 4; ++j) {
                        umma<TF32>(d_tmem, da + 2 * j, db + 2 * j, idesc, (uint32_t)((kb | j) != 0));
                        if constexpr (SPLIT) umma<TF32>(d_tmem, da + 2 * j, db + lo_step + 2 * j, idesc, 1u);
                    }
                    umma_commit(&empty[stage]);
                    if (kb == KB - 1) umma_commit(&tfull[acc]);
                }
                __syncwarp();
                if (++stage == stages) { stage = 0; phase ^= 1; }
            }
            if (++acc == TC_ACC) { acc = 0; acc_phase ^= 1; }
        }
    } else if (warp < 6) {
        const int e = threadIdx.x - 64;
        const int quad = warp & 3;
        const int row_in_tile = quad * 32 + lane;
        int acc = 0;
        uint32_t acc_phase = 0;
        if constexpr (DUMP) {
            for (int tile = blockIdx.x; tile < num_tiles; tile += gridDim.x) {
                const int64_t r = (int64_t)tile * TC_BLOCK_M + row_in_tile;
                const float iv = r < n ? __ldg(inv_norms + r) : -1.0f;
                mbar_wait(&tfull[acc], acc_phase);
                tc_fence_after();
                const uint32_t taddr = tmem_base + ((uint32_t)(quad * 32) << 16) + (uint32_t)(acc * nq_pad);
                uint64_t *out = dump_keys + (int64_t)tile * nq * TC_BLOCK_M + row_in_tile;
                for (int c = 0; c < nq_pad; c += 16) {
                    uint32_t v[16];
                    tmem_ld16(taddr + c, v);
                    tmem_ld_wait();
#pragma unroll
                    for (int j = 0; j < 16; ++j)
                        if (c + j < nq)
                            out[(int64_t)(c + j) * TC_BLOCK_M] = iv >= 0.0f ? make_key(__uint_as_float(v[j]) * iv, (uint32_t)r) : 0ull;
                }
                tc_fence_before();
                __syncwarp();
                if (lane == 0) mbar_arrive(&tempty[acc]);
                if (++acc == TC_ACC) { acc = 0; acc_phase ^= 1; }
            }
        } else {
        if (ub.use_seed && !collect) {
            const int64_t row0 = (int64_t)blockIdx.x * TC_BLOCK_M + row_in_tile;
            const float inv0 = row0 < n ? __ldg(inv_norms + row0) : -1.0f;
            mbar_wait(&tfull[0], 0);
            tc_fence_after();
            const uint32_t taddr0 = tmem_base + ((uint32_t)(quad * 32) << 16);
            for (int c = 0; c < nq_pad; c += 16) {
                uint32_t v[16];
                tmem_ld16(taddr0 + c, v);
                tmem_ld_wait();
#pragma unroll
                for (int j = 0; j < 16; ++j) {
                    const float sc = inv0 >= 0.0f ? __uint_as_float(v[j]) * inv0 : -INFINITY;
                    const uint32_t mx = __reduce_max_sync(0xffffffffu, f32_ordered(sc));
                    if (lane == 0) wmax[(warp - 2) * nq_pad + c + j] = mx;
                }
            }
            named_bar_sync(1, 128);
            if (e < nq_pad) {
                uint32_t m = wmax[e];
#pragma unroll
                for (int w = 1; w < 4; ++w) m = max(m, wmax[w * nq_pad + e]);
                seed_tab[(size_t)blockIdx.x * nq_pad + e] = m;
                cmax[e] = m;
            }
            __threadfence();
            named_bar_sync(1, 128);
            if (e == 0) {
                atomicAdd(seed_ctr, 1);
                const long long t0 = clock64();
                while (*(volatile int *)seed_ctr < (int)gridDim.x)
                    if (clock64() - t0 > 400000) break;
                __threadfence();
            }
            named_bar_sync(1, 128);
            const int G = (int)gridDim.x;
            int *pub_ctr = reinterpret_cast<int *>(gbound + 64);
            if (warp == 2) {
                for (int q = blockIdx.x; q < nq; q += G) {
                    const float sd = seed_select(seed_tab, G, nq_pad, q, ub.ksel, lane);
                    if (lane == 0) {
                        if (sd > -INFINITY) atomicMax(gbound + q, f32_ordered(sd));
                        __threadfence();
                        atomicAdd(pub_ctr, 1);
                    }
                }
                if (lane == 0) {
                    const long long t0 = clock64();
                    while (*(volatile int *)pub_ctr < nq)
                        if (clock64() - t0 > 200000) break;
                    __threadfence();
                }
            }
            named_bar_sync(1, 128);
            if (e < nq) {
                const uint32_t o = __ldcg(gbound + e);
                if (o != 0u) tauf[e] = band_floor(f32_from_ordered(o), ub.band);
            }
            named_bar_sync(1, 128);
        }
        if (!collect && e == 0) s_done[1] = 1;
        uint64_t *my_slab = collect ? nullptr : ub.slab + (size_t)blockIdx.x * nq * SCAN_SLAB;
        int64_t row = (int64_t)blockIdx.x * TC_BLOCK_M + row_in_tile;
        float inv = row < n ? __ldg(inv_norms + row) : -1.0f;
        for (int tile = blockIdx.x; tile < num_tiles; tile += gridDim.x) {
            const int64_t row_next = row + (int64_t)gridDim.x * TC_BLOCK_M;
            const float inv_next = (tile + (int)gridDim.x < num_tiles && row_next < n) ? __ldg(inv_norms + row_next) : -1.0f;
            const bool valid = inv >= 0.0f;
            mbar_wait(&tfull[acc], acc_phase);
            tc_fence_after();
            const uint32_t taddr = tmem_base + ((uint32_t)(quad * 32) << 16) + (uint32_t)(acc * nq_pad);
            auto process = [&](const uint32_t (&v)[16], int c) {
                float tf[16];
#pragma unroll
                for (int j4 = 0; j4 < 4; ++j4) {
                    const float4 t4 = *reinterpret_cast<const float4 *>(tauf + c + 4 * j4);
                    tf[4 * j4] = t4.x; tf[4 * j4 + 1] = t4.y; tf[4 * j4 + 2] = t4.z; tf[4 * j4 + 3] = t4.w;
                }
                if (valid) {
                    uint32_t hits = 0;
#pragma unroll
                    for (int j = 0; j < 16; ++j) hits |= (__uint_as_float(v[j]) * inv >= tf[j]) ? (1u << j) : 0u;
                    hits &= nq - c >= 16 ? 0xFFFFu : ((1u << (nq - c > 0 ? nq - c : 0)) - 1u);
                    while (hits) {
                        const int j = __ffs(hits) - 1;
                        hits &= hits - 1;
                        const int q = c + j;
                        float s = 0.0f;
#pragma unroll
                        for (int jj = 0; jj < 16; ++jj) s = (jj == j) ? __uint_as_float(v[jj]) * inv : s;
                        const uint64_t key = make_key(s, (uint32_t)row);
                        if (collect) {
                            const int pos = atomicAdd(col.cnt + q, 1);
                            if (pos < col.cap) col.buf[(size_t)q * col.cap + pos] = key;
                        } else {
#ifdef VIDMEM_AB_NORARE
                            if (key == 1) tauf[q] = 0.0f;
                            continue;
#endif
                            const int pos = atomicAdd(&lcnt[q], 1);
                            atomicMax(&cmax[q], (uint32_t)(key >> 32));
                            if (pos < SCAN_SLAB) __stcg(my_slab + (size_t)q * SCAN_SLAB + pos, key);
                            else {
                                const int p = atomicAdd(ub.ucnt + q, 1);
                                if (p < ub.ucap) __stcg(ub.ubuf + (size_t)q * ub.ucap + p, key);
                                else tauf[q] = INFINITY;
                            }
                        }
                    }
                }
            };
            uint32_t va[16], vb[16];
#ifdef VIDMEM_AB_NOEPI
            if (tile < 0)
#endif
            tmem_ld16(taddr, va);
#ifdef VIDMEM_AB_NOEPI
            if (tile < 0)
#endif
            for (int c = 0; c < nq_pad; c += 32) {
                tmem_ld_wait();
                if (c + 16 < nq_pad) tmem_ld16(taddr + c + 16, vb);
                process(va, c);
                if (c + 16 < nq_pad) {
                    tmem_ld_wait();
                    if (c + 32 < nq_pad) tmem_ld16(taddr + c + 32, va);
                    process(vb, c + 16);
                }
            }
#ifdef VIDMEM_AB_TILEBAR
            named_bar_sync(1, 128);
#endif
            tc_fence_before();
            __syncwarp();
            if (lane == 0) mbar_arrive(&tempty[acc]);
            if (++acc == TC_ACC) { acc = 0; acc_phase ^= 1; }
            row = row_next;
            inv = inv_next;
        }
        if (!collect) {
            named_bar_sync(1, 128);
            if (e < nq) {
                ub.scnt[(size_t)blockIdx.x * nq + e] = lcnt[e];
                if (seed_tab != nullptr) __stcg(seed_tab + (size_t)blockIdx.x * nq_pad + e, cmax[e]);
            }
        }
        }
        __syncwarp();
        if (lane == 0) atomicAdd((int *)s_done, 1);
    } else {
#ifdef VIDMEM_AB_NOSVC
        if (false) {
#else
        if (!DUMP && warp == 8 && seed_tab != nullptr && !collect) {
#endif
            const int G = (int)gridDim.x;
            while (s_done[1] == 0 && s_done[0] < 4) __nanosleep(100);
            uint32_t pub0 = 0xFFFFFFFFu, pub1 = 0xFFFFFFFFu;
            uint32_t kth_done = 0;
            const uint64_t *my_slab = ub.slab + (size_t)blockIdx.x * nq * SCAN_SLAB;
            while (!__any_sync(0xffffffffu, s_done[0] >= 4)) {
#pragma unroll
                for (int h = 0; h < 2; ++h) {
                    const int q = lane + 32 * h;
                    if (q < nq) {
                        const uint32_t c = *(volatile uint32_t *)(cmax + q);
                        uint32_t &pub = h ? pub1 : pub0;
                        if (c != pub && c != 0u) { __stcg(seed_tab + (size_t)blockIdx.x * nq_pad + q, c); pub = c; }
                    }
                }
                __syncwarp();
                if (G >= ub.ksel)
                    for (int q = blockIdx.x; q < nq; q += G) {
                        const float sd = seed_select(seed_tab, G, nq_pad, q, ub.ksel, lane);
                        if (lane == 0 && sd > -INFINITY) atomicMax(gbound + q, f32_ordered(sd));
                    }
                __syncwarp();
#ifndef VIDMEM_AB_KTH_LEVELS
#define VIDMEM_AB_KTH_LEVELS 2
#endif
#ifndef VIDMEM_AB_KTH_PER_ROUND
#define VIDMEM_AB_KTH_PER_ROUND 1
#endif
                {
                    constexpr int LV = VIDMEM_AB_KTH_LEVELS;
                    int served = 0;
#pragma unroll
                    for (int h = 0; h < 2; ++h) {
                        const int q = lane + 32 * h;
                        int level = 0;
                        if (q < nq) {
                            const int have = *(volatile int *)(lcnt + q);
#pragma unroll
                            for (int l = 1; l <= LV; ++l) level = have >= (SCAN_SLAB >> (LV - l)) ? l : level;
                        }
                        const int done = (int)((kth_done >> (4 * h)) & 15u);
                        unsigned todo = __ballot_sync(0xffffffffu, level > done && (SCAN_SLAB >> (LV - level)) >= ub.ksel);
                        while (todo && (VIDMEM_AB_KTH_PER_ROUND == 0 || served < VIDMEM_AB_KTH_PER_ROUND)) {
                            const int src = __ffs(todo) - 1;
                            todo &= todo - 1;
                            ++served;
                            const int lv = __shfl_sync(0xffffffffu, level, src);
                            const int qq = src + 32 * h;
                            const uint32_t ok = own_kth_score(my_slab + (size_t)qq * SCAN_SLAB, SCAN_SLAB >> (LV - lv), ub.ksel, lane);
                            if (lane == src && ok != 0u) {
                                atomicMax(gbound + qq, ok);
                                kth_done = (kth_done & ~(15u << (4 * h))) | ((uint32_t)lv << (4 * h));
                            }
                        }
                    }
                }
                __syncwarp();
#pragma unroll
                for (int h = 0; h < 2; ++h) {
                    const int q = lane + 32 * h;
                    if (q < nq) {
                        const uint32_t o = __ldcg(gbound + q);
                        if (o != 0u) {
                            const float f = band_floor(f32_from_ordered(o), ub.band);
                            if (f > tauf[q]) *(volatile float *)(tauf + q) = f;
                        }
                    }
                }
                __nanosleep(svc_sleep);
            }
        }
    }

    tc_fence_before();
    __syncthreads();
    if (warp == 1) {
        tc_fence_after();
        tmem_dealloc(tmem_base, TC_TMEM_COLS);
    }
}

bool scan_tc_supported(int dtype, int dim, int nq, int kp, int split)
{
    (void)kp;
    if (dtype != VM_F32 && dtype != VM_BF16) return false;
    if (nq < 1 || nq > 64) return false;
    TcLayout L = make_layout(dtype, ld_for_dim(dim), nq, split);
    return L.stages >= 3;
}

int launch_scan_tc(const ScanArgs &a, const void *queries_store_dtype, uint32_t *seed_tab, int *seed_ctr, const ScanCollect *sc,
                   ScanInfo *info)
{
    VM_REQUIRE(a.n >= 1 && a.n < 0x7FFFFF00LL, VM_ERR_UNSUPPORTED, "tcgen05 scan: shard rows %lld outside [1, 2^31)", (long long)a.n);
    TcLayout L = make_layout(a.dtype, a.ld, a.nq, a.split);
    VM_REQUIRE(L.stages >= 3, VM_ERR_UNSUPPORTED, "tcgen05 scan: dim %d x %d queries does not fit shared memory", a.dim, a.nq);
    CUtensorMap tmA, tmB;
    int rc = make_tmap_2d_cached(&tmA, a.rows, a.dtype, (uint64_t)a.n, (uint64_t)a.ld, (uint64_t)a.ld, TC_BLOCK_M);
    if (rc != VM_OK) return rc;
    rc = make_tmap_2d_cached(&tmB, queries_store_dtype, a.dtype, (uint64_t)L.nq_pad * (L.split ? 2 : 1), (uint64_t)a.ld, (uint64_t)a.ld,
                             (uint32_t)L.nq_pad);
    if (rc != VM_OK) return rc;
    const int num_tiles = (int)((a.n + TC_BLOCK_M - 1) / TC_BLOCK_M);
    const bool dump = a.dump && !sc;
    if (sc || dump || a.ctas > 256) { seed_tab = nullptr; seed_ctr = nullptr; }
    CollectArgs col{};
    if (sc) { col.thr = sc->thr; col.buf = sc->buf; col.cnt = sc->cnt; col.cap = sc->cap; col.pending = sc->pending; }
    BandArgs ub{a.slab, a.scnt, a.ubuf, a.ucnt, a.ucap, a.band, a.ksel, 0};
    ub.use_seed = (seed_tab && seed_ctr && a.ksel >= 1 && a.ctas >= a.ksel) ? 1 : 0;
    if (!sc && !dump)
        VM_REQUIRE(ub.slab && ub.scnt && ub.ubuf && ub.ucnt && ub.ucap > 0 && ub.ksel >= 1, VM_ERR_BADARG, "tcgen05 scan: slab / spill buffers missing");
    if (dump) VM_REQUIRE(TC_BLOCK_M == SCAN_DUMP_TILE && (int64_t)num_tiles * TC_BLOCK_M <= SCAN_DUMP_MAX_KEYS && a.ctas == num_tiles,
                         VM_ERR_UNSUPPORTED, "tcgen05 scan: dump mode needs one CTA per tile and at most %d rows", SCAN_DUMP_MAX_KEYS);
#ifdef VIDMEM_AB_SVCSLEEP
    const int svc_sleep = VIDMEM_AB_SVCSLEEP;
#else
    const int svc_sleep = a.dtype == VM_F32 ? 500 : 200;
#endif
    if (info && !sc) { info->stages = L.stages; info->variant = dump ? 1 : 2; }
    const bool pdl = a.pdl && !sc;
#ifdef VIDMEM_AB_CLASSIC_LAUNCH
#define LAUNCH_IMPL(TF, DU, SP) scan_tc_kernel<TF, DU, SP><<<a.ctas, DU ? TC_THREADS : TC_THREADS_SVC, L.total, a.stream>>>(tmA, tmB, a.inv_norms, a.n, num_tiles, a.nq, L, a.cand, seed_tab, seed_ctr, col, ub, svc_sleep)
#else
#define LAUNCH_IMPL(TF, DU, SP) VM_CUDA_CHECK(launch_pdl(scan_tc_kernel<TF, DU, SP>, dim3(a.ctas), dim3(DU ? TC_THREADS : TC_THREADS_SVC), L.total, a.stream, pdl, \
                                 tmA, tmB, a.inv_norms, a.n, num_tiles, a.nq, L, a.cand, seed_tab, seed_ctr, col, ub, svc_sleep))
#endif
#define LAUNCH_TC(TF, DU, SP)                                                                                                \
    do {                                                                                                                   \
        VM_CUDA_CHECK((max_smem_once<scan_tc_kernel<TF, DU, SP>>(227 * 1024)));                                              \
        LAUNCH_IMPL(TF, DU, SP);                                                                                           \
    } while (0)
    if (a.dtype == VM_F32) { if (dump) LAUNCH_TC(true, true, false); else LAUNCH_TC(true, false, false); }
    else if (L.split) { if (dump) LAUNCH_TC(false, true, true); else LAUNCH_TC(false, false, true); }
    else { if (dump) LAUNCH_TC(false, true, false); else LAUNCH_TC(false, false, false); }
#undef LAUNCH_TC
#undef LAUNCH_IMPL
    VM_CUDA_CHECK(cudaGetLastError());
    return VM_OK;
}

}
```

### real-time-brain-inspired-video-memory_b200/csrc/select.cu

```cuda
#include "common.cuh"

#include <type_traits>

namespace vm {

static constexpr int MERGE_THREADS = 512;
static constexpr int MERGE_SURV = 1024;

__device__ uint64_t radix_select_kth(const uint64_t *skeys, int total, int kp, int *hist, int *s_bin, int *s_need)
{
    const int tid = threadIdx.x, lane = tid & 31;
    uint64_t prefix = 0;
    int need = kp;
    for (int pass = 0; pass < 8; ++pass) {
        const int shift = 56 - 8 * pass;
        const uint64_t hmask = pass == 0 ? 0ull : (~0ull << (shift + 8));
        if (tid < 256) hist[tid] = 0;
        __syncthreads();
        for (int e = tid; e < total; e += MERGE_THREADS) {
            const uint64_t k = skeys[e];
            const bool act = k != 0 && (k & hmask) == prefix;
            const int bin = act ? (int)((k >> shift) & 0xFF) : -1;
            const unsigned peers = __match_any_sync(__activemask(), bin);
            if (act && (__ffs(peers) - 1) == lane) atomicAdd(&hist[bin], __popc(peers));
// ... 396 lines not shown
        const int g_lo = c == 0 ? 0 : (c == 1 ? c1 : c2), g_hi = c == 0 ? c1 : (c == 1 ? c2 : gpr);
        const int w = g_hi - g_lo;
        for (int e = tid; e < kp * w; e += THREADS) {
            const int r = e / w, g = g_lo + (e - r * w);
            const uint32_t rid = s_rid[r];
            if (rid != NO_ROW)
                cp_async16(srow + (size_t)r * pitch + (size_t)g * 16,
                           reinterpret_cast<const unsigned char *>(rows + (int64_t)rid * ld) + (size_t)g * 16);
        }
        cp_async_commit();
    }
    const int kind = j < kp ? 0 : (j < 2 * kp ? 1 : ((j == 2 * kp && s_qq != nullptr) ? 2 : 3));
    const int cidx = kind == 0 ? j : (kind == 1 ? j - kp : 0);
    const bool active = kind == 2 || (kind < 2 && s_rid[cidx] != NO_ROW);
    const T *mine = reinterpret_cast<const T *>(srow + (size_t)cidx * pitch);
    constexpr int EPG = 16 / (int)sizeof(T);
    RefSum acc;
    acc.init();
#pragma unroll
    for (int c = 0; c < 3; ++c) {
        if (c == 0) cp_async_wait<2>();
        else if (c == 1) cp_async_wait<1>();
        else cp_async_wait<0>();
        __syncthreads();
        const int g_lo = c == 0 ? 0 : (c == 1 ? c1 : c2), g_hi = c == 0 ? c1 : (c == 1 ? c2 : gpr);
        const int i_lo = g_lo * EPG, i_hi = min(g_hi * EPG, dim);
        if (active) {
            if (kind == 0)
                ref_sum_range<NEUMAIER>(acc, i_lo, i_hi, [&](int i) { return __dmul_rn(sq[i], load_elem(mine, i)); });
            else if (kind == 1)
                ref_sum_range<NEUMAIER>(acc, i_lo, i_hi, [&](int i) { const double y = load_elem(mine, i); return __dmul_rn(y, y); });
            else
                ref_sum_range<NEUMAIER>(acc, i_lo, i_hi, [&](int i) { const double x = sq[i]; return __dmul_rn(x, x); });
        }
    }
    if (active) {
        const double r = acc.result<NEUMAIER>();
        if (kind == 0) s_dot[cidx] = r;
        else if (kind == 1) s_rr[cidx] = r;
        else *s_qq = r;
    }
    __syncthreads();
}

struct SelectSrc {
    const uint64_t *cand;
    int lists, list_len;
    int complete;
    const uint64_t *slab;
    const int *scnt;
    int ctas;
    const uint64_t *ubuf;
    const int *ucnt;
    int ucap;
    const uint32_t *seed_tab;
    int nq_pad, ksel;
    float band;
    int key_cap;
    int band_cap;
};

template <int THREADS>
__device__ int load_slab_keys(const SelectSrc &src, int q, int nq, uint64_t *skeys, int *s_cnts, int *s_total, float *s_bf, bool *incomplete)
{
    const int tid = threadIdx.x, lane = tid & 31, warp = tid >> 5;
    if (warp == 0) {
        float Lb = -INFINITY;
        if (src.seed_tab != nullptr) {
            if (src.ctas >= src.ksel) Lb = seed_select(src.seed_tab, src.ctas, src.nq_pad, q, src.ksel, lane);
            const uint32_t o = __ldcg(src.seed_tab + SEED_TAB_WORDS + q);
            if (o != 0u) Lb = fmaxf(Lb, f32_from_ordered(o));
        }
        if (lane == 0) { *s_bf = band_floor(Lb, src.band); *s_total = 0; }
    }
    for (int c = tid; c < src.ctas; c += THREADS) s_cnts[c] = min(src.scnt[(size_t)c * nq + q], SCAN_SLAB);
    __syncthreads();
    const float bf = *s_bf;
    constexpr int WARPS = THREADS / 32, PER = SCAN_SLAB / 32, BATCH = 4;
    for (int c0 = warp; c0 < src.ctas; c0 += WARPS * BATCH) {
        uint64_t kk[BATCH][PER];
#pragma unroll
        for (int b = 0; b < BATCH; ++b) {
            const int c = c0 + b * WARPS;
            const int cnt = c < src.ctas ? s_cnts[c] : 0;
#pragma unroll
            for (int t = 0; t < PER; ++t)
                kk[b][t] = (lane + 32 * t < cnt) ? __ldcg(src.slab + ((size_t)c * nq + q) * SCAN_SLAB + lane + 32 * t) : 0ull;
        }
#pragma unroll
        for (int b = 0; b < BATCH; ++b)
#pragma unroll
            for (int t = 0; t < PER; ++t) {
                const uint64_t k = kk[b][t];
                if (k != 0 && key_score(k) >= bf) {
                    const int p = atomicAdd(s_total, 1);
                    if (p < src.key_cap) skeys[p] = k;
                }
            }
    }
    const int spilled = src.ucnt[q];
    const int ns = min(spilled, src.ucap);
    for (int e = tid; e < ns; e += THREADS) {
        const uint64_t k = __ldcg(src.ubuf + (size_t)q * src.ucap + e);
        if (k != 0 && key_score(k) >= bf) {
            const int p = atomicAdd(s_total, 1);
            if (p < src.key_cap) skeys[p] = k;
        }
    }
    __syncthreads();
    const int got = *s_total;
    *incomplete = spilled > src.ucap || got > src.key_cap;
    return min(got, src.key_cap);
}

__global__ void __launch_bounds__(SR_THREADS) slab_top_kernel(SelectSrc src, int nq, int kp, uint64_t *__restrict__ merged,
                                                             int *__restrict__ incomplete)
{
    extern __shared__ __align__(16) unsigned char st_smem[];
    uint64_t *skeys = reinterpret_cast<uint64_t *>(st_smem);
    __shared__ int s_cnts[256];
    __shared__ int s_total, s_bin, s_need, s_m;
    __shared__ int hist[256];
    __shared__ float s_bf;
    const int q = blockIdx.x, tid = threadIdx.x;
    bool inc = false;
    const int total = load_slab_keys<SR_THREADS>(src, q, nq, skeys, s_cnts, &s_total, &s_bf, &inc);
    for (int e = tid; e < kp; e += SR_THREADS) merged[(int64_t)q * kp + e] = 0;
    if (tid == 0) { incomplete[q] = inc ? 1 : 0; s_m = 0; }
    __syncthreads();
    if (total <= MERGE_SURV) {
        for (int e = tid; e < total; e += SR_THREADS) {
            const uint64_t k = skeys[e];
            int rank = 0;
            for (int i = 0; i < total; ++i) rank += skeys[i] > k ? 1 : 0;
            if (rank < kp) merged[(int64_t)q * kp + rank] = k;
        }
        return;
    }
    const uint64_t Tk = radix_select_kth(skeys, total, kp, hist, &s_bin, &s_need);
    for (int e = tid; e < total; e += SR_THREADS) {
        const uint64_t k = skeys[e];
        if (k > Tk) merged[(int64_t)q * kp + atomicAdd(&s_m, 1)] = k;
        else if (k == Tk) merged[(int64_t)q * kp + kp - 1] = k;
    }
}

template <bool NEUMAIER, typename T>
__global__ void __launch_bounds__(SR_THREADS, 1) select_rescore_kernel(SelectSrc src, int nq, int kp,
                                                                   const T *__restrict__ rows, int ld, int dim, int64_t n_rows,
                                                                   const void *__restrict__ queries, int q_dtype, double eps,
                                                                   FinalizeArgs f, int32_t *__restrict__ flags,
                                                                   int32_t *__restrict__ uncertified_count,
                                                                   const int *__restrict__ extreme, float *__restrict__ collect_thr,
                                                                   unsigned long long *__restrict__ cum, const float *__restrict__ inv_norms)
{
    extern __shared__ __align__(16) unsigned char sr_smem[];
    uint64_t *skeys = reinterpret_cast<uint64_t *>(sr_smem);
    uint32_t *lmax = reinterpret_cast<uint32_t *>(skeys + src.key_cap);
    double *sq = reinterpret_cast<double *>(lmax + ((src.lists + 3) & ~3));
    const int pitch = ld * (int)sizeof(T) + 16;
    unsigned char *srow = reinterpret_cast<unsigned char *>(sq + ((dim + 1) & ~1));
    double *b_sc = reinterpret_cast<double *>(srow + (((size_t)kp * pitch + 15) & ~(size_t)15));
    uint32_t *b_row = reinterpret_cast<uint32_t *>(b_sc + src.band_cap);
    __shared__ uint64_t s_top[64];
    __shared__ uint32_t s_rid[64];
    __shared__ uint64_t surv[MERGE_SURV];
    __shared__ int hist[256];
    __shared__ int s_bin, s_need, s_m, s_nz, s_cnt, s_band, s_viol, s_out, s_total;
    __shared__ int s_cnts[256];
    __shared__ uint32_t s_L;
    __shared__ float s_thr, s_bf;
    __shared__ double s_dot[64], s_rr[64], s_qq, s_score[64];
    const int q = blockIdx.x, tid = threadIdx.x, lane = tid & 31, warp = tid >> 5;

    pdl_launch_dependents();
    if (tid == 0) { s_m = 0; s_nz = 0; s_cnt = 0; s_band = 0; s_viol = 0; s_thr = -INFINITY; }
    if (tid < 64) s_top[tid] = 0;
    pdl_wait();
    __syncthreads();

    const bool union_mode = src.slab != nullptr;
    int total, lists = src.lists, list_len = src.list_len;
    bool overflow = false;
    int nz = 0;
    if (union_mode) {
        total = load_slab_keys<SR_THREADS>(src, q, nq, skeys, s_cnts, &s_total, &s_bf, &overflow);
        lists = 0;
        if (tid == 0) nz = total;
    } else {
        total = lists * list_len;
#pragma unroll 10
        for (int e = tid; e < total; e += SR_THREADS) {
            const int l = e / list_len, j = e - l * list_len;
            const uint64_t k = src.cand[((int64_t)l * nq + q) * list_len + j];
            skeys[e] = k;
            nz += k != 0;
        }
    }
    for (int i = tid; i < dim; i += SR_THREADS) sq[i] = load_as_double(queries, q_dtype, (int64_t)q * dim + i);
    if (nz) atomicAdd(&s_nz, nz);
    __syncthreads();
    const int nonzero = s_nz;
    bool done = false;
    if (total <= MERGE_SURV) {
        for (int e = tid; e < total; e += SR_THREADS) {
            const uint64_t k = skeys[e];
            if (k == 0) continue;
            int rank = 0;
            for (int i = 0; i < total; ++i) rank += skeys[i] > k ? 1 : 0;
            if (rank < kp) s_top[rank] = k;
        }
        done = true;
    } else if (nonzero >= kp && lists >= kp && lists <= 256) {
        for (int l = warp; l < lists; l += SR_THREADS / 32) {
            uint32_t m = 0;
            for (int j = lane; j < list_len; j += 32) m = max(m, (uint32_t)(skeys[l * list_len + j] >> 32));
            m = __reduce_max_sync(0xffffffffu, m);
            if (lane == 0) lmax[l] = m;
        }
        __syncthreads();
        if (warp == 0) {
            uint32_t vals[8];
#pragma unroll
            for (int t = 0; t < 8; ++t) vals[t] = (lane + 32 * t) < lists ? lmax[lane + 32 * t] : 0u;
            uint32_t prefix = 0;
            int need = kp;
            for (int bit = 31; bit >= 12; --bit) {
                const uint32_t hi = bit == 31 ? 0u : (0xFFFFFFFFu << (bit + 1));
                int cnt = 0;
#pragma unroll
                for (int t = 0; t < 8; ++t) cnt += ((vals[t] & hi) == prefix && ((vals[t] >> bit) & 1u)) ? 1 : 0;
                const int tot = __reduce_add_sync(0xffffffffu, cnt);
                if (tot >= need) prefix |= 1u << bit;
                else need -= tot;
            }
            if (lane == 0) s_L = prefix;
        }
        __syncthreads();
        const uint32_t Lb = s_L;
        if (Lb != 0) {
            for (int e = tid; e < total; e += SR_THREADS) {
                const uint64_t k = skeys[e];
                if ((uint32_t)(k >> 32) >= Lb && k != 0) {
                    const int p = atomicAdd(&s_m, 1);
                    if (p < MERGE_SURV) surv[p] = k;
                }
            }
            __syncthreads();
            const int m = s_m;
            if (m >= kp && m <= MERGE_SURV) {
                for (int e = tid; e < m; e += SR_THREADS) {
                    const uint64_t k = surv[e];
                    int rank = 0;
                    for (int i = 0; i < m; ++i) rank += surv[i] > k ? 1 : 0;
                    if (rank < kp) s_top[rank] = k;
                }
                done = true;
            }
        }
    }
    if (!done) {
        __syncthreads();
        uint64_t Tk = 1;
        if (nonzero >= kp) Tk = radix_select_kth(skeys, total, kp, hist, &s_bin, &s_need);
        if (tid == 0) s_m = 0;
        __syncthreads();
        for (int e = tid; e < total; e += SR_THREADS) {
            const uint64_t k = skeys[e];
            if (k >= Tk && k != 0) {
                if (nonzero >= kp && k == Tk) s_top[kp - 1] = k;
                else s_top[atomicAdd(&s_m, 1)] = k;
            }
        }
    }
    __syncthreads();

    const int j = tid;
    const uint64_t mykey = j < 64 ? s_top[j] : 0;
    const bool cand_valid = j < kp && mykey != 0;
    if (j < 64) s_rid[j] = cand_valid ? key_row(mykey) : NO_ROW;
    __syncthreads();
    stage_and_chain<NEUMAIER, T, SR_THREADS>(rows, ld, dim, kp, s_rid, srow, pitch, sq, s_dot, s_rr, &s_qq);

    double sc = 0.0;
    const uint32_t row = cand_valid ? key_row(mykey) : 0;
    const double n1 = __dsqrt_rn(s_qq);
    if (n1 == 0.0) {
        if (tid == 0) {
            int c = 0;
            const double outv = convert_score(0.0, f.score_mode);
            if (outv > f.min_score)
                for (int64_t r = 0; r < n_rows && c < f.k; ++r)
                    if (__ldg(inv_norms + r) >= 0.0f) {
                        f.out_idx[(int64_t)q * f.k + c] = r + f.row_offset;
                        f.out_score[(int64_t)q * f.k + c] = outv;
                        ++c;
                    }
            for (int t = c; t < f.k; ++t) { f.out_idx[(int64_t)q * f.k + t] = -1; f.out_score[(int64_t)q * f.k + t] = 0.0; }
            f.out_count[q] = c;
            flags[q] = 0;
            if (collect_thr) collect_thr[q] = INFINITY;
        }
        return;
    }
    if (cand_valid) {
        const double n2 = __dsqrt_rn(s_rr[j]);
        sc = (n1 == 0.0 || n2 == 0.0) ? 0.0 : __ddiv_rn(s_dot[j], __dmul_rn(n1, n2));
        if (fabs((double)key_score(mykey) - sc) > eps) atomicAdd(&s_viol, 1);
    }
    if (j < 64) s_score[j] = sc;
    __syncthreads();
    int ncand = 0;
    for (int i = 0; i < kp; ++i) ncand += s_top[i] != 0;
    int rank = 0;
    if (cand_valid)
        for (int i = 0; i < kp; ++i)
            if (s_top[i] != 0 && i != j && better(s_score[i], key_row(s_top[i]), sc, row)) ++rank;
    const double outv = convert_score(sc, f.score_mode);
    const bool emit = cand_valid && rank < f.k && outv > f.min_score;
    if (emit) {
        f.out_idx[(int64_t)q * f.k + rank] = (int64_t)row + f.row_offset;
        f.out_score[(int64_t)q * f.k + rank] = outv;
        atomicAdd(&s_cnt, 1);
    }
    if (cand_valid && ncand >= f.k && rank == f.k - 1) {
        float t = (float)(sc - eps);
        t = nextafterf(nextafterf(t, -INFINITY), -INFINITY);
        s_thr = t;
    }
    __syncthreads();
    const float thr = s_thr;
// ... 48 lines not shown
            }
            __syncthreads();
        }
        band_emit<SR_THREADS>(band, b_sc, b_row, &s_out, f, q);
        if (tid == 0) {
            flags[q] = 0;
            if (collect_thr) collect_thr[q] = INFINITY;
            if (cum) atomicAdd(cum + 1, 1ull);
        }
        return;
    }
    if (tid == 0) {
        flags[q] = bound_ok ? 1 : 2;
        if (collect_thr) {
            float t = thr > -INFINITY ? (float)((double)thr - eps) : -INFINITY;
            t = nextafterf(t, -INFINITY);
            collect_thr[q] = bound_ok ? t : INFINITY;
        }
        atomicAdd(uncertified_count, 1);
        f.out_count[q] = s_cnt;
    }
    const int cnt = s_cnt;
    for (int t = cnt + tid; t < f.k; t += SR_THREADS) {
        f.out_idx[(int64_t)q * f.k + t] = -1;
        f.out_score[(int64_t)q * f.k + t] = 0.0;
    }
}

static constexpr int CR_THREADS = 512;
template <bool NEUMAIER, typename T>
__global__ void __launch_bounds__(CR_THREADS, 1) collect_rescore_kernel(const uint64_t *__restrict__ buf, const int *__restrict__ cnt, int cap,
                                                                       const T *__restrict__ rows, int ld, int dim,
                                                                       const void *__restrict__ queries, int q_dtype, FinalizeArgs f,
                                                                       int32_t *__restrict__ flags, int32_t *__restrict__ uncertified_count,
                                                                       int nq, unsigned long long *__restrict__ cum, int stage_rows)
{
    extern __shared__ __align__(16) unsigned char cr_smem[];
    double *sq = reinterpret_cast<double *>(cr_smem);
    double *s_sc = sq + ((dim + 1) & ~1);
    double *s_rr = s_sc + cap;
    uint32_t *s_row = reinterpret_cast<uint32_t *>(s_sc + (stage_rows > 0 ? cap : 2 * cap));
    const int pitch = ld * (int)sizeof(T) + 16;
    unsigned char *srow = reinterpret_cast<unsigned char *>(s_row + ((cap + 3) & ~3));
    __shared__ double s_n1;
    __shared__ int s_out;
    __shared__ uint32_t s_rid[64];
    __shared__ double s_dot[64], s_r2[64];
    const int q = blockIdx.x, tid = threadIdx.x;
    if (flags[nq] == 0 || flags[q] != 1) return;
    const int m = cnt[q];
    if (m > cap) {
        if (tid == 0) flags[q] = 2;
        return;
    }
    for (int i = tid; i < dim; i += CR_THREADS) sq[i] = load_as_double(queries, q_dtype, (int64_t)q * dim + i);
    for (int e = tid; e < m; e += CR_THREADS) s_row[e] = key_row(buf[(size_t)q * cap + e]);
    __syncthreads();
    if (tid == 0) {
        RefSum qq; qq.init();
        ref_sum_range<NEUMAIER>(qq, 0, dim, [&](int i) { return __dmul_rn(sq[i], sq[i]); });
        s_n1 = __dsqrt_rn(qq.result<NEUMAIER>());
    }
    __syncthreads();
    if (stage_rows > 0) {
        const double n1 = s_n1;
        for (int b0 = 0; b0 < m; b0 += stage_rows) {
            const int c = min(stage_rows, m - b0);
            if (tid < 64) s_rid[tid] = tid < c ? s_row[b0 + tid] : NO_ROW;
            __syncthreads();
            stage_and_chain<NEUMAIER, T, CR_THREADS>(rows, ld, dim, stage_rows, s_rid, srow, pitch, sq, s_dot, s_r2, nullptr);
            if (tid < c) {
                const double n2 = __dsqrt_rn(s_r2[tid]);
                s_sc[b0 + tid] = (n1 == 0.0 || n2 == 0.0) ? 0.0 : __ddiv_rn(s_dot[tid], __dmul_rn(n1, n2));
            }
            __syncthreads();
        }
    } else {
        band_score_global<NEUMAIER, T, CR_THREADS>(rows, ld, dim, sq, s_n1, m, s_sc, s_rr, s_row);
    }
    band_emit<CR_THREADS>(m, s_sc, s_row, &s_out, f, q);
    if (tid == 0) {
        flags[q] = 0;
        atomicSub(uncertified_count, 1);
        if (cum) atomicAdd(cum + 2, 1ull);
    }
}

#define XK 64

template <int THREADS>
__device__ void exact_merge_query(const double *__restrict__ xlist_score, const uint32_t *__restrict__ xlist_row,
                                  const int32_t *__restrict__ xlist_cnt, int lists, int nq, int k, int q, const FinalizeArgs &f,
                                  uint8_t *__restrict__ taken, double *w_s, uint32_t *w_r, int *w_p, int *s_out)
{
    const int tid = threadIdx.x, lane = tid & 31, warp = tid >> 5;
    const int total = lists * k;
    uint8_t *tk = taken + (int64_t)q * total;
    for (int e = tid; e < total; e += THREADS) tk[e] = 0;
    if (tid == 0) *s_out = 0;
    __syncthreads();
    auto scan_local = [&](double &bs, uint32_t &br, int &bp) {
        bp = -1; bs = 0.0; br = 0;
        for (int e = tid; e < total; e += THREADS) {
            int l = e / k, j = e - l * k;
            if (tk[e] || j >= xlist_cnt[(int64_t)l * nq + q]) continue;
            int64_t g = ((int64_t)l * nq + q) * k + j;
            double s = xlist_score[g];
            uint32_t r = xlist_row[g];
            if (bp < 0 || better(s, r, bs, br)) { bs = s; br = r; bp = e; }
        }
    };
    double bs; uint32_t br; int bp;
    scan_local(bs, br, bp);
    for (int r = 0; r < f.k; ++r) {
        double ms = bs; uint32_t mr = br; int mp = bp;
        for (int o = 16; o > 0; o >>= 1) {
            double ts = __shfl_xor_sync(0xffffffffu, ms, o);
            uint32_t tr = __shfl_xor_sync(0xffffffffu, mr, o);
            int tp = __shfl_xor_sync(0xffffffffu, mp, o);
            if (tp >= 0 && (mp < 0 || better(ts, tr, ms, mr))) { ms = ts; mr = tr; mp = tp; }
        }
        if (lane == 0) { w_s[warp] = ms; w_r[warp] = mr; w_p[warp] = mp; }
        __syncthreads();
        ms = w_s[0]; mr = w_r[0]; mp = w_p[0];
        for (int w = 1; w < THREADS / 32; ++w)
            if (w_p[w] >= 0 && (mp < 0 || better(w_s[w], w_r[w], ms, mr))) { ms = w_s[w]; mr = w_r[w]; mp = w_p[w]; }
        if (mp < 0) break;
        double outv = convert_score(ms, f.score_mode);
        if (tid == 0 && outv > f.min_score) {
            f.out_idx[(int64_t)q * f.k + r] = (int64_t)mr + f.row_offset;
            f.out_score[(int64_t)q * f.k + r] = outv;
            *s_out = r + 1;
        }
        if (mp == bp) {
            tk[bp] = 1;
            scan_local(bs, br, bp);
        }
        __syncthreads();
    }
    __syncthreads();
    int cnt = *s_out;
    if (tid == 0) f.out_count[q] = cnt;
    for (int t = cnt + tid; t < f.k; t += THREADS) {
        f.out_idx[(int64_t)q * f.k + t] = -1;
        f.out_score[(int64_t)q * f.k + t] = 0.0;
    }
    __syncthreads();
}

static constexpr int XS_THREADS = 256;
static constexpr int XS_CG = 24;
static constexpr int XS_PITCH = XS_CG * 16 + 16;

template <bool NEUMAIER, typename T>
__global__ void __launch_bounds__(XS_THREADS) exact_scan_kernel(const T *__restrict__ rows, const float *__restrict__ inv_norms,
                                                               int64_t n, int ld, int dim, const void *__restrict__ queries,
                                                               int q_dtype, int nq, int32_t *__restrict__ flags, int k,
                                                               double *__restrict__ xlist_score, uint32_t *__restrict__ xlist_row,
                                                               int32_t *__restrict__ xlist_cnt, unsigned long long *__restrict__ cum,
                                                               int *__restrict__ done_ctr, FinalizeArgs f, uint8_t *__restrict__ taken)
{
    pdl_launch_dependents();
    pdl_wait();
    if (flags && flags[nq] == 0) return;
    if (flags && cum && blockIdx.x == 0 && threadIdx.x == 0) atomicAdd(cum + 3, (unsigned long long)flags[nq]);
    extern __shared__ __align__(16) unsigned char xs_smem[];
    double *sq = reinterpret_cast<double *>(xs_smem);
    unsigned char *buf0 = reinterpret_cast<unsigned char *>(sq + ((dim + 1) & ~1));
    __shared__ double l_score[XK], n_score[XK];
    __shared__ uint32_t l_row[XK], n_row[XK];
    __shared__ double c_score[128];
    __shared__ uint32_t c_row[128];
    __shared__ double s_dotv[128], s_rrv[128];
    __shared__ int l_cnt, c_cnt;
    __shared__ double s_n1;
    const int tid = threadIdx.x, rt = tid & 127;
    const bool is_rr = tid >= 128;
    const int gpr = ld * (int)sizeof(T) / 16;
    const int nchunks = (gpr + XS_CG - 1) / XS_CG;
    constexpr int EPG = 16 / (int)sizeof(T);
    for (int q = 0; q < nq; ++q) {
        if (flags && flags[q] == 0) continue;
        __syncthreads();
        for (int i = tid; i < dim; i += XS_THREADS) sq[i] = load_as_double(queries, q_dtype, (int64_t)q * dim + i);
        if (tid == 0) { l_cnt = 0; c_cnt = 0; }
        __syncthreads();
        if (tid == 0) {
            RefSum qq; qq.init();
            ref_sum_range<NEUMAIER>(qq, 0, dim, [&](int i) { return __dmul_rn(sq[i], sq[i]); });
            s_n1 = __dsqrt_rn(qq.result<NEUMAIER>());
        }
        __syncthreads();
        const double n1 = s_n1;
        const int64_t ntiles = (n + 127) / 128;
        const int my_tiles = (int)((ntiles - blockIdx.x + gridDim.x - 1) / gridDim.x);
        const int total_steps = my_tiles > 0 ? my_tiles * nchunks : 0;
        auto issue = [&](int st) {
            if (st < total_steps) {
                const int64_t tile = blockIdx.x + (int64_t)(st / nchunks) * gridDim.x;
                const int c = st % nchunks;
                unsigned char *buf = buf0 + (size_t)(st % 3) * 128 * XS_PITCH;
                const int g0 = c * XS_CG, gw = min(XS_CG, gpr - g0);
                for (int e = tid; e < 128 * gw; e += XS_THREADS) {
                    const int rr_ = e / gw, g = e - rr_ * gw;
                    const int64_t row = tile * 128 + rr_;
                    if (row < n)
                        cp_async16(buf + (size_t)rr_ * XS_PITCH + (size_t)g * 16,
                                   reinterpret_cast<const unsigned char *>(rows + row * (int64_t)ld) + (size_t)(g0 + g) * 16);
                }
            }
            cp_async_commit();
        };
        issue(0);
        issue(1);
        RefSum acc;
        acc.init();
        for (int st = 0; st < total_steps; ++st) {
            const int64_t tile = blockIdx.x + (int64_t)(st / nchunks) * gridDim.x;
            const int c = st % nchunks;
            const int64_t r = tile * 128 + rt;
            const bool live = r < n && inv_norms[r] >= 0.0f;
            issue(st + 2);
            cp_async_wait<2>();
            __syncthreads();
            const unsigned char *cur = buf0 + (size_t)(st % 3) * 128 * XS_PITCH;
            const int i_lo = c * XS_CG * EPG, i_hi = min((c + 1) * XS_CG * EPG, dim);
            if (live && i_lo < i_hi) {
                const T *mine = reinterpret_cast<const T *>(cur + (size_t)rt * XS_PITCH);
                if (!is_rr)
                    ref_sum_range<NEUMAIER>(acc, i_lo, i_hi, [&](int i) { return __dmul_rn(sq[i], load_elem(mine, i - i_lo)); });
                else
                    ref_sum_range<NEUMAIER>(acc, i_lo, i_hi, [&](int i) { const double y = load_elem(mine, i - i_lo); return __dmul_rn(y, y); });
            }
            if (c + 1 < nchunks) {
                __syncthreads();
                continue;
            }
            if (live) { if (is_rr) s_rrv[rt] = acc.result<NEUMAIER>(); else s_dotv[rt] = acc.result<NEUMAIER>(); }
            acc.init();
            __syncthreads();
            double sc = 0.0;
            bool hit = false;
            if (live && !is_rr) {
                const double n2 = __dsqrt_rn(s_rrv[rt]);
                sc = (n1 == 0.0 || n2 == 0.0) ? 0.0 : __ddiv_rn(s_dotv[rt], __dmul_rn(n1, n2));
                const int lc = l_cnt;
                hit = lc < k || better(sc, (uint32_t)r, l_score[lc - 1], l_row[lc - 1]);
            }
            if (hit) {
                const int p = atomicAdd(&c_cnt, 1);
                c_score[p] = sc;
                c_row[p] = (uint32_t)r;
            }
            const int cc = __syncthreads_count(hit ? 1 : 0);
            const int lc = l_cnt;
            if (cc > 0) {
                for (int e = tid; e < lc + cc; e += XS_THREADS) {
                    const double se = e < lc ? l_score[e] : c_score[e - lc];
                    const uint32_t re = e < lc ? l_row[e] : c_row[e - lc];
                    int rank = 0;
                    for (int i = 0; i < lc; ++i) rank += better(l_score[i], l_row[i], se, re) ? 1 : 0;
                    for (int i = 0; i < cc; ++i) rank += better(c_score[i], c_row[i], se, re) ? 1 : 0;
                    if (rank < k) { n_score[rank] = se; n_row[rank] = re; }
                }
                __syncthreads();
                const int nl = min(k, lc + cc);
                for (int e = tid; e < nl; e += XS_THREADS) { l_score[e] = n_score[e]; l_row[e] = n_row[e]; }
                if (tid == 0) { l_cnt = nl; c_cnt = 0; }
                __syncthreads();
            }
        }
        cp_async_wait<0>();
        __syncthreads();
        const int lc = l_cnt;
        const int64_t base = ((int64_t)blockIdx.x * nq + q) * k;
        for (int e = tid; e < lc; e += XS_THREADS) { xlist_score[base + e] = l_score[e]; xlist_row[base + e] = l_row[e]; }
        if (tid == 0) xlist_cnt[(int64_t)blockIdx.x * nq + q] = lc;
    }
    if (done_ctr == nullptr) return;
    __shared__ int s_last, s_out;
    __shared__ double w_s[XS_THREADS / 32];
    __shared__ uint32_t w_r[XS_THREADS / 32];
    __shared__ int w_p[XS_THREADS / 32];
    __threadfence();
    __syncthreads();
    if (tid == 0) s_last = atomicAdd(done_ctr, 1) == (int)gridDim.x - 1;
    __syncthreads();
    if (!s_last) return;
    __threadfence();
    for (int q = 0; q < nq; ++q) {
        if (flags[q] == 0) continue;
        exact_merge_query<XS_THREADS>(xlist_score, xlist_row, xlist_cnt, (int)gridDim.x, nq, k, q, f, taken, w_s, w_r, w_p, &s_out);
        if (tid == 0) flags[q] = 0;
    }
    if (tid == 0) { *done_ctr = 0; flags[nq] = 0; }
}

__global__ void __launch_bounds__(256) exact_merge_kernel(const double *__restrict__ xlist_score, const uint32_t *__restrict__ xlist_row,
                                                         const int32_t *__restrict__ xlist_cnt, int lists, int nq, int k,
                                                         const int32_t *__restrict__ flags, FinalizeArgs f, uint8_t *__restrict__ taken)
{
    __shared__ double w_s[8];
    __shared__ uint32_t w_r[8];
    __shared__ int w_p[8];
    __shared__ int s_out;
    const int q = blockIdx.x;
    if (flags && (flags[nq] == 0 || flags[q] == 0)) return;
    exact_merge_query<256>(xlist_score, xlist_row, xlist_cnt, lists, nq, k, q, f, taken, w_s, w_r, w_p, &s_out);
}

__global__ void __launch_bounds__(256) merge_topk_lists_kernel(const char *__restrict__ idx_b, const char *__restrict__ score_b,
                                                              const char *__restrict__ count_b, size_t stride, int lists, int nq, int k,
                                                              int64_t *__restrict__ out_idx, double *__restrict__ out_score,
                                                              int32_t *__restrict__ out_count)
{
    extern __shared__ unsigned char smem_raw[];
    const int q = blockIdx.x, tid = threadIdx.x;
    const int total = lists * k;
    double *s_s = (double *)smem_raw;
    int64_t *s_i = (int64_t *)(s_s + total);
    int *s_v = (int *)(s_i + total);
    for (int e = tid; e < total; e += 256) {
        int l = e / k, j = e - l * k;
        const int64_t *idx = (const int64_t *)(idx_b + (size_t)l * stride);
        const double *score = (const double *)(score_b + (size_t)l * stride);
        const int32_t *count = (const int32_t *)(count_b + (size_t)l * stride);
        int64_t g = (int64_t)q * k + j;
        bool v = j < count[q];
        s_s[e] = v ? score[g] : 0.0;
        s_i[e] = v ? idx[g] : -1;
        s_v[e] = v ? 1 : 0;
    }
    __syncthreads();
    int nvalid = 0;
    for (int e = 0; e < total; ++e) nvalid += s_v[e];
    for (int e = tid; e < total; e += 256) {
        if (!s_v[e]) continue;
        int rank = 0;
        for (int i = 0; i < total; ++i)
            if (s_v[i] && (s_s[i] > s_s[e] || (s_s[i] == s_s[e] && s_i[i] < s_i[e]))) ++rank;
        if (rank < k) { out_idx[(int64_t)q * k + rank] = s_i[e]; out_score[(int64_t)q * k + rank] = s_s[e]; }
    }
    int cnt = min(nvalid, k);
    if (tid == 0) out_count[q] = cnt;
    for (int t = cnt + tid; t < k; t += 256) { out_idx[(int64_t)q * k + t] = -1; out_score[(int64_t)q * k + t] = 0.0; }
}

struct PeerPtrs { const unsigned char *p[16]; };

__global__ void p2p_publish_kernel(unsigned long long *flag, unsigned long long gen)
{
    __threadfence_system();
    asm volatile("st.release.sys.global.u64 [%0], %1;" ::"l"(flag), "l"(gen) : "memory");
}

__global__ void __launch_bounds__(256) merge_topk_p2p_kernel(PeerPtrs peers, int nranks, size_t slot_off, size_t flag_off,
                                                            unsigned long long gen, int nq, int k,
                                                            int64_t *__restrict__ out_idx, double *__restrict__ out_score,
                                                            int32_t *__restrict__ out_count)
{
    extern __shared__ unsigned char smem_raw[];
    const int q = blockIdx.x, tid = threadIdx.x;
    const int total = nranks * k;
    double *s_s = (double *)smem_raw;
    int64_t *s_i = (int64_t *)(s_s + total);
    int *s_v = (int *)(s_i + total);
    if (tid < nranks) {
        const unsigned long long *f = reinterpret_cast<const unsigned long long *>(peers.p[tid] + flag_off);
        unsigned long long v;
        const long long t0 = clock64();
        for (;;) {
            asm volatile("ld.acquire.sys.global.u64 %0, [%1];" : "=l"(v) : "l"(f) : "memory");
            if (v >= gen) break;
            if (clock64() - t0 > 4000000000LL) { printf("vidmem: peer %d never published batch %llu\n", tid, gen); __trap(); }
        }
    }
    __syncthreads();
    for (int e = tid; e < total; e += 256) {
        const int l = e / k, j = e - l * k;
        const unsigned char *b = peers.p[l] + slot_off;
        const int64_t *idx = reinterpret_cast<const int64_t *>(b);
        const double *score = reinterpret_cast<const double *>(b + (size_t)nq * k * 8);
        const int32_t *count = reinterpret_cast<const int32_t *>(b + (size_t)nq * k * 16);
        const bool v = j < __ldcv(count + q);
        s_s[e] = v ? __ldcv(score + (size_t)q * k + j) : 0.0;
        s_i[e] = v ? __ldcv(idx + (size_t)q * k + j) : -1;
        s_v[e] = v ? 1 : 0;
    }
    __syncthreads();
    int nvalid = 0;
    for (int e = 0; e < total; ++e) nvalid += s_v[e];
    for (int e = tid; e < total; e += 256) {
        if (!s_v[e]) continue;
        int rank = 0;
        for (int i = 0; i < total; ++i)
            if (s_v[i] && (s_s[i] > s_s[e] || (s_s[i] == s_s[e] && s_i[i] < s_i[e]))) ++rank;
        if (rank < k) { out_idx[(int64_t)q * k + rank] = s_i[e]; out_score[(int64_t)q * k + rank] = s_s[e]; }
    }
    const int cnt = min(nvalid, k);
    if (tid == 0) out_count[q] = cnt;
    for (int t = cnt + tid; t < k; t += 256) { out_idx[(int64_t)q * k + t] = -1; out_score[(int64_t)q * k + t] = 0.0; }
}

__global__ void __launch_bounds__(256) merge_max_by_id_kernel(const int64_t *__restrict__ idx, const double *__restrict__ score,
                                                             const int32_t *__restrict__ count, int nq, int k, int k2,
                                                             int64_t *__restrict__ out_idx, double *__restrict__ out_score,
                                                             int32_t *__restrict__ out_count)
{
    extern __shared__ unsigned char smem_raw[];
    const int tid = threadIdx.x, total = nq * k;
    double *s_s = (double *)smem_raw;
    int64_t *s_i = (int64_t *)(s_s + total);
    int *s_rep = (int *)(s_i + total);
    __shared__ int s_n;
    if (tid == 0) s_n = 0;
    for (int e = tid; e < total; e += 256) {
        int qi = e / k, j = e - qi * k;
        bool v = j < count[qi];
        s_i[e] = v ? idx[e] : -1;
        s_s[e] = v ? score[e] : 0.0;
        s_rep[e] = 0;
    }
    __syncthreads();
    for (int e = tid; e < total; e += 256) {
        if (s_i[e] < 0) continue;
        bool first = true;
        for (int i = 0; i < e; ++i)
            if (s_i[i] == s_i[e]) { first = false; break; }
        if (!first) continue;
        double m = s_s[e];
        for (int i = e + 1; i < total; ++i)
            if (s_i[i] == s_i[e] && score[i] > m) m = score[i];
        s_rep[e] = 1;
        s_s[e] = m;
        atomicAdd(&s_n, 1);
    }
    __syncthreads();
    for (int e = tid; e < total; e += 256) {
        if (!s_rep[e]) continue;
        int rank = 0;
        for (int i = 0; i < total; ++i)
            if (s_rep[i] && (s_s[i] > s_s[e] || (s_s[i] == s_s[e] && i < e))) ++rank;
        if (rank < k2) { out_idx[rank] = s_i[e]; out_score[rank] = s_s[e]; }
    }
    if (tid == 0) *out_count = min(s_n, k2);
}

template <bool NEUMAIER>
__global__ void cosine_pairs_kernel(const void *__restrict__ a, const void *__restrict__ b, int dtype, int64_t n, int dim,
                                    int zero_rule, double *__restrict__ out)
{
    int64_t i = blockIdx.x * (int64_t)blockDim.x + threadIdx.x;
    if (i >= n) return;
    RefSum dot, aa, bb;
    dot.init(); aa.init(); bb.init();
    for (int c = 0; c < dim; ++c) {
        double x = load_as_double(a, dtype, i * dim + c), y = load_as_double(b, dtype, i * dim + c);
        dot.add<NEUMAIER>(__dmul_rn(x, y));
        aa.add<NEUMAIER>(__dmul_rn(x, x));
        bb.add<NEUMAIER>(__dmul_rn(y, y));
    }
    double n1, n2;
    if (zero_rule == 2) { n1 = pow(aa.result<NEUMAIER>(), 0.5); n2 = pow(bb.result<NEUMAIER>(), 0.5); }
    else { n1 = __dsqrt_rn(aa.result<NEUMAIER>()); n2 = __dsqrt_rn(bb.result<NEUMAIER>()); }
    double den = __dmul_rn(n1, n2);
    bool zero = zero_rule == 1 ? (den == 0.0) : (n1 == 0.0 || n2 == 0.0);
    out[i] = zero ? 0.0 : __ddiv_rn(dot.result<NEUMAIER>(), den);
}

int k_merge_candidates(const uint64_t *cand, int lists, int nq, int kp, uint64_t *merged, cudaStream_t st)
{
    size_t smem = (size_t)lists * kp * sizeof(uint64_t) + (size_t)lists * sizeof(uint32_t) + 16;
    VM_CUDA_CHECK((max_smem_once<merge_candidates_kernel>(200 * 1024)));
    VM_REQUIRE(smem <= 200 * 1024, VM_ERR_UNSUPPORTED, "candidate merge: %d lists x %d exceeds shared memory", lists, kp);
    merge_candidates_kernel<<<nq, MERGE_THREADS, smem, st>>>(cand, lists, nq, kp, merged);
    VM_CUDA_CHECK(cudaGetLastError());
    return VM_OK;
}


template <typename F>
static int with_sum_mode(int sum_mode, F &&f)
{
    return sum_mode == VM_SUM_NEUMAIER ? f(std::true_type{}) : f(std::false_type{});
}

template <typename F>
static int with_row_type(int dtype, int sum_mode, F &&f)
{
    auto by_sum = [&](auto *tag) { return with_sum_mode(sum_mode, [&](auto neu) { return f(neu, tag); }); };
    if (dtype == VM_F32) return by_sum((float *)nullptr);
    if (dtype == VM_F64) return by_sum((double *)nullptr);
    return by_sum((__nv_bfloat16 *)nullptr);
}

int k_rescore(const RescoreArgs &a, cudaStream_t st, const int *incomplete)
{
    const int ssz = a.dtype == VM_F64 ? 8 : 4;
    int chunk = RS_SMEM_ROW_BYTES / (ssz * a.kp) - 1;
    chunk &= ~7;
    if (chunk > a.ld) chunk = a.ld;
    const size_t smem = (size_t)chunk * sizeof(double) + (size_t)a.kp * (chunk + 1) * ssz + 16;
    return with_row_type(a.dtype, a.sum_mode, [&](auto neu, auto *tag) -> int {
        using T = std::remove_pointer_t<decltype(tag)>;
        constexpr bool NEU = decltype(neu)::value;
        VM_CUDA_CHECK((max_smem_once<rescore_kernel<NEU, T>>(160 * 1024)));
        rescore_kernel<NEU, T><<<a.nq, RS_THREADS, smem, st>>>(a.merged, a.kp, (const T *)a.rows, a.inv_norms, a.ld, a.dim,
                                                               a.n_rows, a.queries, a.q_dtype, a.eps, a.fin, a.flags,
                                                               a.uncertified_count, chunk, a.extreme, a.collect_thr, a.cum, incomplete);
        VM_CUDA_CHECK(cudaGetLastError());
        return VM_OK;
    });
}


static constexpr size_t SR_SMEM_LIMIT = 180 * 1024;
static size_t select_rescore_base_smem(int key_cap, int lists, int kp, int dtype, int dim, int ld)
{
    const int es = (int)dtype_size(dtype);
    const size_t rows_area = (((size_t)kp * ((size_t)ld * es + 16) + 15) & ~(size_t)15) + 16;
    return (size_t)key_cap * 8 + (size_t)((lists + 3) & ~3) * 4 + (size_t)((dim + 1) & ~1) * 8 + rows_area + 32;
}
static int select_band_cap(int key_cap, int lists, int kp, int dtype, int dim, int ld)
{
    const size_t base = select_rescore_base_smem(key_cap, lists, kp, dtype, dim, ld);
    if (base + (size_t)BAND_CAP_MIN * 12 > SR_SMEM_LIMIT) return 0;
    size_t cap = (SR_SMEM_LIMIT - base) / 12;
    cap &= ~(size_t)63;
    if (cap > (size_t)BAND_CAP_MAX) cap = BAND_CAP_MAX;
    return (int)cap;
}
bool select_rescore_fits(int lists, int list_len, int kp, int dtype, int dim, int ld)
{
    const int key_cap = lists > 0 ? lists * list_len : SELECT_KEY_CAP;
    return select_band_cap(key_cap, lists, kp, dtype, dim, ld) >= BAND_CAP_MIN && kp <= 64 && 2 * kp + 1 <= SR_THREADS;
}

static SelectSrc make_src(const SelectArgs &sa)
{
    const bool slab_mode = sa.slab != nullptr;
    const int lists = slab_mode ? 0 : sa.lists;
    return SelectSrc{sa.cand, lists, sa.list_len, sa.complete, sa.slab, sa.scnt, sa.ctas, sa.ubuf, sa.ucnt, sa.ucap, sa.seed_tab,
                     sa.nq_pad, sa.ksel, sa.band, slab_mode ? SELECT_KEY_CAP : lists * sa.list_len, 0};
}

int k_select_rescore(const SelectArgs &sa, const RescoreArgs &a, cudaStream_t st, bool pdl)
{
    SelectSrc src = make_src(sa);
    VM_REQUIRE(src.slab == nullptr || src.ctas <= 256, VM_ERR_UNSUPPORTED, "select: %d scan CTAs exceed 256", src.ctas);
    if (!select_rescore_fits(src.lists, src.list_len, a.kp, a.dtype, a.dim, a.ld)) return VM_ERR_UNSUPPORTED;
    src.band_cap = select_band_cap(src.key_cap, src.lists, a.kp, a.dtype, a.dim, a.ld);
    const size_t smem = select_rescore_base_smem(src.key_cap, src.lists, a.kp, a.dtype, a.dim, a.ld) + (size_t)src.band_cap * 12;
    return with_row_type(a.dtype, a.sum_mode, [&](auto neu, auto *tag) -> int {
        using T = std::remove_pointer_t<decltype(tag)>;
        constexpr bool NEU = decltype(neu)::value;
        VM_CUDA_CHECK((max_smem_once<select_rescore_kernel<NEU, T>>(180 * 1024)));
        VM_CUDA_CHECK(launch_pdl(select_rescore_kernel<NEU, T>, dim3(a.nq), dim3(SR_THREADS), smem, st, pdl, src, a.nq, a.kp,
                                 (const T *)a.rows, a.ld, a.dim, a.n_rows, a.queries, a.q_dtype, a.eps, a.fin, a.flags,
                                 a.uncertified_count, a.extreme, a.collect_thr, a.cum, a.inv_norms));
        VM_CUDA_CHECK(cudaGetLastError());
        return VM_OK;
    });
}

int k_slab_top(const SelectArgs &sa, int nq, int kp, uint64_t *merged, int *incomplete, cudaStream_t st)
{
    const SelectSrc src = make_src(sa);
    VM_REQUIRE(src.slab != nullptr && src.ctas <= 256, VM_ERR_UNSUPPORTED, "slab selection: bad source");
    slab_top_kernel<<<nq, SR_THREADS, (size_t)src.key_cap * 8, st>>>(src, nq, kp, merged, incomplete);
    VM_CUDA_CHECK(cudaGetLastError());
    return VM_OK;
}

int k_collect_rescore(const uint64_t *buf, const int *cnt, int cap, const RescoreArgs &a, cudaStream_t st)
{
    const size_t head = (size_t)((a.dim + 1) & ~1) * 8;
    const size_t staged = head + (size_t)cap * 8 + (size_t)((cap + 3) & ~3) * 4 + (size_t)32 * ((size_t)a.ld * dtype_size(a.dtype) + 16) + 64;
    const int stage_rows = staged <= 200 * 1024 ? 32 : 0;
    const size_t smem = stage_rows ? staged : head + (size_t)cap * (8 + 8 + 4) + 32;
    VM_REQUIRE(smem <= 200 * 1024, VM_ERR_UNSUPPORTED, "collect pass: buffer of %d rows exceeds shared memory", cap);
    return with_row_type(a.dtype, a.sum_mode, [&](auto neu, auto *tag) -> int {
        using T = std::remove_pointer_t<decltype(tag)>;
        constexpr bool NEU = decltype(neu)::value;
        VM_CUDA_CHECK((max_smem_once<collect_rescore_kernel<NEU, T>>(200 * 1024)));
        collect_rescore_kernel<NEU, T><<<a.nq, CR_THREADS, smem, st>>>(buf, cnt, cap, (const T *)a.rows, a.ld, a.dim, a.queries,
                                                                       a.q_dtype, a.fin, a.flags, a.uncertified_count, a.nq, a.cum, stage_rows);
        VM_CUDA_CHECK(cudaGetLastError());
        return VM_OK;
    });
}

int k_exact(const ExactArgs &a, cudaStream_t st, bool pdl)
{
    VM_REQUIRE((size_t)a.dim * sizeof(double) <= 40 * 1024, VM_ERR_UNSUPPORTED, "exact scan: dim %d too large", a.dim);
    const size_t smem = (size_t)((a.dim + 1) & ~1) * sizeof(double) + (size_t)3 * 128 * XS_PITCH + 16;
    const bool conditional = a.flags != nullptr && a.done_ctr != nullptr;
    const int rc = with_row_type(a.dtype, a.sum_mode, [&](auto neu, auto *tag) -> int {
        using T = std::remove_pointer_t<decltype(tag)>;
        constexpr bool NEU = decltype(neu)::value;
        VM_CUDA_CHECK((max_smem_once<exact_scan_kernel<NEU, T>>(200 * 1024)));
        VM_CUDA_CHECK(launch_pdl(exact_scan_kernel<NEU, T>, dim3(a.ctas), dim3(XS_THREADS), smem, st, pdl && conditional, (const T *)a.rows,
                                 a.inv_norms, a.n, a.ld, a.dim, a.queries, a.q_dtype, a.nq, a.flags, a.k, a.xlist_score, a.xlist_row,
                                 a.xlist_cnt, a.cum, conditional ? a.done_ctr : (int *)nullptr, a.fin, a.taken));
        VM_CUDA_CHECK(cudaGetLastError());
        return VM_OK;
    });
    if (rc != VM_OK || conditional) return rc;
    exact_merge_kernel<<<a.nq, 256, 0, st>>>(a.xlist_score, a.xlist_row, a.xlist_cnt, a.ctas, a.nq, a.k, a.flags, a.fin, a.taken);
    VM_CUDA_CHECK(cudaGetLastError());
    return VM_OK;
}

int k_merge_topk_lists(const void *idx, const void *score, const void *count, size_t stride_bytes, int lists, int nq, int k,
                       int64_t *out_idx, double *out_score, int32_t *out_count, cudaStream_t st)
{
    int total = lists * k;
    VM_REQUIRE(total <= 4096, VM_ERR_UNSUPPORTED, "merge_topk_lists: lists*k = %d > 4096", total);
    size_t smem = (size_t)total * (8 + 8 + 4);
    VM_CUDA_CHECK((max_smem_once<merge_topk_lists_kernel>(100 * 1024)));
    merge_topk_lists_kernel<<<nq, 256, smem, st>>>((const char *)idx, (const char *)score, (const char *)count, stride_bytes, lists, nq, k,
                                                  out_idx, out_score, out_count);
    VM_CUDA_CHECK(cudaGetLastError());
    return VM_OK;
}

int k_p2p_publish(void *flag, unsigned long long gen, cudaStream_t st)
{
    p2p_publish_kernel<<<1, 1, 0, st>>>((unsigned long long *)flag, gen);
    VM_CUDA_CHECK(cudaGetLastError());
    return VM_OK;
}

int k_merge_topk_p2p(void *const *peers, int nranks, size_t slot_off, size_t flag_off, unsigned long long gen, int nq, int k,
                     int64_t *out_idx, double *out_score, int32_t *out_count, cudaStream_t st)
{
    VM_REQUIRE(nranks >= 1 && nranks <= 16, VM_ERR_UNSUPPORTED, "peer exchange supports up to 16 ranks");
    const int total = nranks * k;
    VM_REQUIRE(total <= 4096, VM_ERR_UNSUPPORTED, "merge: nranks*k = %d > 4096", total);
    PeerPtrs pp{};
    for (int r = 0; r < nranks; ++r) pp.p[r] = (const unsigned char *)peers[r];
    const size_t smem = (size_t)total * (8 + 8 + 4);
    VM_CUDA_CHECK((max_smem_once<merge_topk_p2p_kernel>(100 * 1024)));
    merge_topk_p2p_kernel<<<nq, 256, smem, st>>>(pp, nranks, slot_off, flag_off, gen, nq, k, out_idx, out_score, out_count);
    VM_CUDA_CHECK(cudaGetLastError());
    return VM_OK;
}

int k_merge_max_by_id(const int64_t *idx, const double *score, const int32_t *count, int nq, int k, int k2,
                      int64_t *out_idx, double *out_score, int32_t *out_count, cudaStream_t st)
{
    int total = nq * k;
    VM_REQUIRE(total <= 4096, VM_ERR_UNSUPPORTED, "merge_max_by_id: nq*k = %d > 4096", total);
    size_t smem = (size_t)total * (8 + 8 + 4);
    VM_CUDA_CHECK((max_smem_once<merge_max_by_id_kernel>(100 * 1024)));
    merge_max_by_id_kernel<<<1, 256, smem, st>>>(idx, score, count, nq, k, k2, out_idx, out_score, out_count);
    VM_CUDA_CHECK(cudaGetLastError());
    return VM_OK;
}

int k_cosine_pairs(const void *a, const void *b, int dtype, int64_t n, int dim, int zero_rule, int sum_mode, double *out,
                   cudaStream_t st)
{
    if (n <= 0) return VM_OK;
    int grid = (int)((n + 127) / 128);
    return with_sum_mode(sum_mode, [&](auto neu) -> int {
        cosine_pairs_kernel<decltype(neu)::value><<<grid, 128, 0, st>>>(a, b, dtype, n, dim, zero_rule, out);
        VM_CUDA_CHECK(cudaGetLastError());
        return VM_OK;
    });
}

}
```

### real-time-brain-inspired-video-memory_b200/csrc/store.cu

```cuda
#include "common.cuh"
#include "synth.cuh"

namespace vm {

template <typename DST>
__global__ void convert_rows_kernel(const void *__restrict__ src, int src_dtype, DST *__restrict__ dst, int64_t n,
                                    int dim, int ld)
{
    int64_t total = n * (int64_t)ld;
    for (int64_t e = blockIdx.x * (int64_t)blockDim.x + threadIdx.x; e < total; e += (int64_t)gridDim.x * blockDim.x) {
        int64_t r = e / ld;
        int c = (int)(e - r * ld);
        double dv = 0.0;
        if (c < dim) dv = load_as_double(src, src_dtype, r * dim + c);
        if constexpr (sizeof(DST) == 8) dst[e] = dv;
        else {
            const float v = (float)dv;
            if constexpr (sizeof(DST) == 4) dst[e] = v;
            else dst[e] = __float2bfloat16_rn(v);
        }
    }
}

template <typename T>
__global__ void row_inv_norms_kernel(const T *__restrict__ rows, float *__restrict__ inv_norms, int64_t row0,
                                     int64_t n, int ld, int *__restrict__ extreme, const double *__restrict__ exact)
{
    int lane = threadIdx.x & 31;
    int64_t warp = (blockIdx.x * (int64_t)blockDim.x + threadIdx.x) >> 5;
    int64_t nwarps = ((int64_t)gridDim.x * blockDim.x) >> 5;
    for (int64_t r = row0 + warp; r < n; r += nwarps) {
        const T *p = rows + r * (int64_t)ld;
        double ss = 0.0;
        for (int c = lane; c < ld; c += 32) {
            double v = (double)load_as_float(p, c);
            ss += v * v;
        }
        for (int o = 16; o > 0; o >>= 1) ss += __shfl_xor_sync(0xffffffffu, ss, o);
        double se = 0.0;
        if (exact != nullptr) {
            for (int c = lane; c < ld; c += 32) {
                const double v = exact[r * (int64_t)ld + c] * 0x1p-600;
                se += v * v;
            }
            for (int o = 16; o > 0; o >>= 1) se += __shfl_xor_sync(0xffffffffu, se, o);
        }
        if (lane == 0) {
            float inv = 0.0f;
            if (!isfinite(ss)) {
                inv = -1.0f;
                if (exact != nullptr && isfinite(se)) { inv = 0.0f; if (extreme) atomicAdd(extreme, 1); }
            } else if (ss > 0.0) {
                inv = (float)(1.0 / sqrt(ss));
                if (extreme && (ss < 7.52316384526264e-37 || ss > 1.329227995784916e+36)) atomicAdd(extreme, 1);
            } else if (exact != nullptr && se != 0.0) {
                if (extreme) atomicAdd(extreme, 1);
            }
            inv_norms[r] = inv;
        }
    }
}

__global__ void invalidate_rows_kernel(float *inv_norms, const int64_t *rows, int64_t n, int64_t size)
{
    int64_t i = blockIdx.x * (int64_t)blockDim.x + threadIdx.x;
    if (i < n && rows[i] >= 0 && rows[i] < size) inv_norms[rows[i]] = -1.0f;
}

__global__ void normalize_queries_kernel(const void *__restrict__ q, int q_dtype, int nq, int nq_pad, int dim, int ld,
                                         float *__restrict__ out_f32, __nv_bfloat16 *__restrict__ out_bf16,
                                         int32_t *__restrict__ zero_me, uint32_t *__restrict__ zero_tab, int zero_tab_n,
                                         int tf32_round, int split)
{
    pdl_launch_dependents();
    pdl_wait();
    if (zero_me && blockIdx.x == 0 && threadIdx.x < 2) zero_me[threadIdx.x] = 0;
    for (int i = blockIdx.x * blockDim.x + threadIdx.x; i < zero_tab_n; i += gridDim.x * blockDim.x) zero_tab[i] = 0u;
    int lane = threadIdx.x & 31;
    int w = (blockIdx.x * blockDim.x + threadIdx.x) >> 5;
    if (w >= nq_pad) return;
    double ss = 0.0;
    if (w < nq)
        for (int c = lane; c < dim; c += 32) {
            double v = load_as_double(q, q_dtype, (int64_t)w * dim + c);
            ss += v * v;
        }
    for (int o = 16; o > 0; o >>= 1) ss += __shfl_xor_sync(0xffffffffu, ss, o);
    double inv = (ss > 0.0 && isfinite(ss)) ? 1.0 / sqrt(ss) : 0.0;
    for (int c = lane; c < ld; c += 32) {
        float v = 0.0f;
        if (w < nq && c < dim) v = (float)(load_as_double(q, q_dtype, (int64_t)w * dim + c) * inv);
        float vf = v;
        if (tf32_round) vf = __uint_as_float((__float_as_uint(v) + 0x1000u) & 0xFFFFE000u);
        out_f32[(int64_t)w * ld + c] = vf;
        if (out_bf16) {
            const __nv_bfloat16 hi = __float2bfloat16_rn(v);
            out_bf16[(int64_t)w * ld + c] = hi;
            if (split) out_bf16[((int64_t)nq_pad + w) * ld + c] = __float2bfloat16_rn(v - __bfloat162float(hi));
        }
    }
}

template <typename T>
__global__ void synth_fill_kernel(T *__restrict__ rows, uint64_t seed, int64_t row0, int64_t n, int dim, int ld,
                                  uint64_t dup_period)
{
    int groups = ld >> 3;
    int64_t total = n * (int64_t)groups;
    uint64_t hk = splitmix64(seed ^ 0xD6E8FEB86659FD93ULL);
    for (int64_t e = blockIdx.x * (int64_t)blockDim.x + threadIdx.x; e < total; e += (int64_t)gridDim.x * blockDim.x) {
        int64_t i = e / groups;
        int g = (int)(e - i * groups);
        uint64_t row = (uint64_t)(row0 + i);
        uint64_t own = splitmix64(splitmix64(seed * 0x9E3779B97F4A7C15ULL + row) + (uint64_t)g);
        uint64_t par = 0, sel = 0;
        bool planted = false;
        if (dup_period > 0 && row > 0) {
            uint64_t hr = splitmix64(hk + row);
            if (hr % dup_period == 0) {
                planted = true;
                uint64_t parent = splitmix64(hr) % row;
                par = splitmix64(splitmix64(seed * 0x9E3779B97F4A7C15ULL + parent) + (uint64_t)g);
                sel = splitmix64(hr + 0x632BE59BD9B4E019ULL + (uint64_t)g);
            }
        }
        T *dst = rows + i * (int64_t)ld + g * 8;
#pragma unroll
        for (int b = 0; b < 8; ++b) {
            int col = g * 8 + b;
            int v = synth_int(own, b);
            if (planted && (((sel >> (8 * b)) & 15ULL) != 0ULL)) v = synth_int(par, b);
            float f = col < dim ? (float)v * (1.0f / 128.0f) : 0.0f;
            if constexpr (sizeof(T) == 4) dst[b] = f;
            else dst[b] = __float2bfloat16_rn(f);
        }
    }
}

int k_convert_rows(const void *src, int src_dtype, void *dst, int dst_dtype, int64_t n, int dim, int ld, cudaStream_t st)
{
    if (n <= 0) return VM_OK;
    int64_t total = n * (int64_t)ld;
    int grid = (int)vm::imin64((total + 255) / 256, 148 * 16);
    if (dst_dtype == VM_F32) convert_rows_kernel<float><<<grid, 256, 0, st>>>(src, src_dtype, (float *)dst, n, dim, ld);
    else if (dst_dtype == VM_F64) convert_rows_kernel<double><<<grid, 256, 0, st>>>(src, src_dtype, (double *)dst, n, dim, ld);
    else convert_rows_kernel<__nv_bfloat16><<<grid, 256, 0, st>>>(src, src_dtype, (__nv_bfloat16 *)dst, n, dim, ld);
    VM_CUDA_CHECK(cudaGetLastError());
    return VM_OK;
}

int k_row_inv_norms(const void *rows, int dtype, float *inv_norms, int64_t row0, int64_t n, int ld, int *extreme, cudaStream_t st,
                    const double *exact)
{
    if (n <= row0) return VM_OK;
    int64_t warps = n - row0;
    int grid = (int)vm::imin64((warps * 32 + 255) / 256, 148 * 16);
    if (dtype == VM_F32) row_inv_norms_kernel<float><<<grid, 256, 0, st>>>((const float *)rows, inv_norms, row0, n, ld, extreme, exact);
    else row_inv_norms_kernel<__nv_bfloat16><<<grid, 256, 0, st>>>((const __nv_bfloat16 *)rows, inv_norms, row0, n, ld, extreme, exact);
    VM_CUDA_CHECK(cudaGetLastError());
    return VM_OK;
}

int k_invalidate_rows(float *inv_norms, const int64_t *rows_dev, int64_t n, int64_t size, cudaStream_t st)
{
    if (n <= 0) return VM_OK;
    invalidate_rows_kernel<<<(int)((n + 255) / 256), 256, 0, st>>>(inv_norms, rows_dev, n, size);
    VM_CUDA_CHECK(cudaGetLastError());
    return VM_OK;
}

int k_normalize_queries(const void *q, int q_dtype, int nq, int nq_pad, int dim, int ld, float *out_f32,
                        void *out_bf16, int32_t *zero_me, uint32_t *zero_tab, int zero_tab_n, int tf32_round, int split, bool pdl,
                        cudaStream_t st)
{
    int threads = 128;
    int grid = (nq_pad * 32 + threads - 1) / threads;
    VM_CUDA_CHECK(launch_pdl(normalize_queries_kernel, dim3(grid), dim3(threads), 0, st, pdl, q, q_dtype, nq, nq_pad, dim, ld, out_f32,
                             (__nv_bfloat16 *)out_bf16, zero_me, zero_tab, zero_tab_n, tf32_round, split));
    VM_CUDA_CHECK(cudaGetLastError());
    return VM_OK;
}

int k_synth_fill(void *rows, int dtype, uint64_t seed, int64_t row0, int64_t n, int dim, int ld, uint64_t dup_period,
                 cudaStream_t st)
{
    if (n <= 0) return VM_OK;
    int64_t total = n * (int64_t)(ld >> 3);
    int grid = (int)vm::imin64((total + 255) / 256, 148 * 32);
    if (dtype == VM_F32) synth_fill_kernel<float><<<grid, 256, 0, st>>>((float *)rows, seed, row0, n, dim, ld, dup_period);
    else synth_fill_kernel<__nv_bfloat16><<<grid, 256, 0, st>>>((__nv_bfloat16 *)rows, seed, row0, n, dim, ld, dup_period);
    VM_CUDA_CHECK(cudaGetLastError());
    return VM_OK;
}

}
```

Baseline: 260,600.

## Double-buffer per-call workspace and overlap consecutive async top-k calls via sequence flags

Splits the per-query workspace into two slots that alternate between consecutive asynchronous calls. Cross-call ordering moves from full PDL waits to device-side sequence counters (call_done), so normalize waits only for the call two back and rescore for the previous call. The next batch's query prep and scan can then overlap the tail of the previous one. It also adds a persistent tile counter and a lean exact-scan variant with less shared memory. The cost is doubled workspace memory, extra spin-waits on device flags, and more complex ordering logic that could deadlock or race if the sequence numbers go wrong.

```diff
diff --git a/real-time-brain-inspired-video-memory_b200/csrc/api.cu b/real-time-brain-inspired-video-memory_b200/csrc/api.cu
--- a/real-time-brain-inspired-video-memory_b200/csrc/api.cu
+++ b/real-time-brain-inspired-video-memory_b200/csrc/api.cu
@@ -24,7 +24,8 @@
                     const double *exact = nullptr);
 int k_invalidate_rows(float *inv_norms, const int64_t *rows_dev, int64_t n, int64_t size, cudaStream_t st);
 int k_normalize_queries(const void *q, int q_dtype, int nq, int nq_pad, int dim, int ld, float *out_f32, void *out_bf16,
-                        int32_t *zero_me, uint32_t *zero_tab, int zero_tab_n, int tf32_round, int split, bool pdl, cudaStream_t st);
+                        int32_t *zero_me, uint32_t *zero_tab, int zero_tab_n, int tf32_round, int split, bool pdl,
+                        const unsigned *call_done, unsigned call_need, cudaStream_t st);
 int k_synth_fill(void *rows, int dtype, uint64_t seed, int64_t row0, int64_t n, int dim, int ld, uint64_t dup_period,
                  cudaStream_t st);
 int k_merge_candidates(const uint64_t *cand, int lists, int nq, int kp, uint64_t *merged, cudaStream_t st);
@@ -113,18 +114,37 @@
     void release() { if (p) cudaFree(p); p = nullptr; bytes = 0; }
 };
 
+struct Slot {
+    Buf q_f32, q_bf16, seed, cand, merged, flags, col_thr, col_cnt, col_buf, xs, xr, xc, taken, ubuf, done, scnt, sel_inc;
+    void release()
+    {
+        Buf *all[] = {&q_f32, &q_bf16, &seed, &cand, &merged, &flags, &col_thr, &col_cnt, &col_buf, &xs, &xr, &xc, &taken, &ubuf, &done,
+                      &scnt, &sel_inc};
+        for (Buf *b : all) b->release();
+    }
+    size_t bytes() const
+    {
+        const Buf *all[] = {&q_f32, &q_bf16, &seed, &cand, &merged, &flags, &col_thr, &col_cnt, &col_buf, &xs, &xr, &xc, &taken, &ubuf,
+                            &done, &scnt, &sel_inc};
+        size_t t = 0;
+        for (const Buf *b : all) t += b->bytes;
+        return t;
+    }
+};
+
 struct Workspace {
     bool ready = false;
     int lists_max = 0;
-    Buf q_raw, q_f32, q_bf16, seed, cand, merged, o_idx, flags, col_thr, col_cnt, col_buf, xs, xr, xc, taken, gather_send, gather_recv, misc, ubuf, done, scnt, sel_inc;
+    Buf q_raw, o_idx, gather_send, gather_recv, misc;
+    Slot slot[2];
     int32_t *h_uncert = nullptr;
     unsigned char *h_pack = nullptr;
     unsigned char *h_q = nullptr;
     void release()
     {
-        Buf *all[] = {&q_raw, &q_f32, &q_bf16, &seed, &cand, &merged, &o_idx, &flags, &col_thr, &col_cnt, &col_buf, &xs, &xr, &xc, &taken,
-                      &gather_send, &gather_recv, &misc, &ubuf, &done, &scnt, &sel_inc};
+        Buf *all[] = {&q_raw, &o_idx, &gather_send, &gather_recv, &misc};
         for (Buf *b : all) b->release();
+        for (Slot &sl : slot) sl.release();
         if (h_uncert) cudaFreeHost(h_uncert);
         if (h_pack) cudaFreeHost(h_pack);
         if (h_q) cudaFreeHost(h_q);
@@ -150,6 +170,11 @@
     int exact_dtype() const { return rows_exact ? (int)VM_F64 : dtype; }
     int *extreme = nullptr;
     unsigned long long *cum = nullptr;
+    unsigned *call_done = nullptr;
+    unsigned seq = 0;
+    int pipe_run = 0;
+    cudaStream_t pipe_stream = nullptr;
+    int last_slot = 0;
     int64_t n_batches = 0, n_queries = 0;
     int last_band_ctas = 0, last_band_nq = 0;
     Buf stage, stage_idx;
@@ -249,25 +274,27 @@
     int rc;
 #define ENS(b, bytes) if ((rc = (b).ensure(bytes)) != VM_OK) return rc
     ENS(w.q_raw, (size_t)MAXQ * s->dim * 8);
-    ENS(w.q_f32, (size_t)MAXQ * s->ld * 4);
-    ENS(w.q_bf16, (size_t)2 * MAXQ * s->ld * 2);
-    ENS(w.cand, (size_t)lists * MAXQ * (MAXK > SCAN_SLAB ? MAXK : SCAN_SLAB) * 8);
-    ENS(w.merged, (size_t)MAXQ * MAXK * 8);
     ENS(w.o_idx, result_bytes(MAXQ, MAXK) + 64);
-    ENS(w.flags, (size_t)(MAXQ + 2) * 4);
-    ENS(w.seed, (size_t)(SEED_TAB_WORDS + 3 * MAXQ) * 4);
-    ENS(w.ubuf, (size_t)MAXQ * SCAN_UNION_CAP * 8);
-    ENS(w.done, 64);
-    ENS(w.scnt, (size_t)256 * MAXQ * 4);
-    ENS(w.sel_inc, (size_t)MAXQ * 4);
-    VM_CUDA_CHECK(cudaMemset(w.done.p, 0, 64));
-    ENS(w.col_thr, (size_t)MAXQ * 4);
-    ENS(w.col_cnt, (size_t)MAXQ * 4);
-    ENS(w.col_buf, (size_t)MAXQ * COLLECT_CAP * 8);
-    ENS(w.xs, (size_t)XCTAS * MAXQ * MAXK * 8);
-    ENS(w.xr, (size_t)XCTAS * MAXQ * MAXK * 4);
-    ENS(w.xc, (size_t)XCTAS * MAXQ * 4);
-    ENS(w.taken, (size_t)MAXQ * XCTAS * MAXK);
+    for (Slot &b : w.slot) {
+        ENS(b.q_f32, (size_t)MAXQ * s->ld * 4);
+        ENS(b.q_bf16, (size_t)2 * MAXQ * s->ld * 2);
+        ENS(b.cand, (size_t)lists * MAXQ * (MAXK > SCAN_SLAB ? MAXK : SCAN_SLAB) * 8);
+        ENS(b.merged, (size_t)MAXQ * MAXK * 8);
+        ENS(b.flags, (size_t)(MAXQ + 2) * 4);
+        ENS(b.seed, (size_t)SEED_BLOCK_WORDS * 4);
+        ENS(b.ubuf, (size_t)MAXQ * SCAN_UNION_CAP * 8);
+        ENS(b.done, 64);
+        ENS(b.scnt, (size_t)256 * MAXQ * 4);
+        ENS(b.sel_inc, (size_t)MAXQ * 4);
+        VM_CUDA_CHECK(cudaMemset(b.done.p, 0, 64));
+        ENS(b.col_thr, (size_t)MAXQ * 4);
+        ENS(b.col_cnt, (size_t)MAXQ * 4);
+        ENS(b.col_buf, (size_t)MAXQ * COLLECT_CAP * 8);
+        ENS(b.xs, (size_t)XCTAS * MAXQ * MAXK * 8);
+        ENS(b.xr, (size_t)XCTAS * MAXQ * MAXK * 4);
+        ENS(b.xc, (size_t)XCTAS * MAXQ * 4);
+        ENS(b.taken, (size_t)MAXQ * XCTAS * MAXK);
+    }
 #undef ENS
     VM_CUDA_CHECK(cudaMallocHost((void **)&w.h_uncert, 64));
     VM_CUDA_CHECK(cudaMallocHost((void **)&w.h_pack, result_bytes(MAXQ, MAXK) + 64));
@@ -325,7 +352,8 @@
     {
         DeviceGuard g(device);
         if (cudaMalloc((void **)&s->extreme, 4) != cudaSuccess || cudaMemset(s->extreme, 0, 4) != cudaSuccess ||
-            cudaMalloc((void **)&s->cum, 64) != cudaSuccess || cudaMemset(s->cum, 0, 64) != cudaSuccess) {
+            cudaMalloc((void **)&s->cum, 64) != cudaSuccess || cudaMemset(s->cum, 0, 64) != cudaSuccess ||
+            cudaMalloc((void **)&s->call_done, 4) != cudaSuccess || cudaMemset(s->call_done, 0, 4) != cudaSuccess) {
             set_error("store allocation failed");
             vm_store_destroy(s);
             return VM_ERR_OOM;
@@ -457,6 +485,7 @@
     arena_destroy(s->ar_rows); arena_destroy(s->ar_inv); arena_destroy(s->ar_exact);
     if (s->extreme) cudaFree(s->extreme);
     if (s->cum) cudaFree(s->cum);
+    if (s->call_done) cudaFree(s->call_done);
     s->stage.release(); s->stage_idx.release();
     s->ws.release();
     for (auto &pr : s->evr) { if (pr[0]) cudaEventDestroy(pr[0]); if (pr[1]) cudaEventDestroy(pr[1]); }
@@ -601,8 +630,9 @@
     DeviceGuard g(s->device);
     VM_CUDA_CHECK(cudaDeviceSynchronize());
     std::vector<int> sc((size_t)ctas * nq), uc(nq);
-    VM_CUDA_CHECK(cudaMemcpy(sc.data(), s->ws.scnt.p, sc.size() * 4, cudaMemcpyDeviceToHost));
-    VM_CUDA_CHECK(cudaMemcpy(uc.data(), (int *)s->ws.seed.p + SEED_TAB_WORDS + 2 * MAXQ, (size_t)nq * 4, cudaMemcpyDeviceToHost));
+    const Slot &b = s->ws.slot[s->last_slot];
+    VM_CUDA_CHECK(cudaMemcpy(sc.data(), b.scnt.p, sc.size() * 4, cudaMemcpyDeviceToHost));
+    VM_CUDA_CHECK(cudaMemcpy(uc.data(), (int *)b.seed.p + SEED_TAB_WORDS + 2 * MAXQ, (size_t)nq * 4, cudaMemcpyDeviceToHost));
     for (int q = 0; q < nq; ++q) {
         int64_t k = 0;
         for (int c = 0; c < ctas; ++c) k += sc[(size_t)c * nq + q];
@@ -653,6 +683,7 @@
     ResultBlock d;
     cudaStream_t st;
     vm_topk_stats *stats;
+    bool sharded = false;
     ResultBlock h = {};
 };
 }
@@ -709,9 +740,6 @@
         q_dev = w.q_raw.p;
     }
     FinalizeArgs fin{c.k, c.min_score, c.score_mode, c.row_offset, c.d.idx, c.d.score, c.d.count};
-    ExactArgs ex{s->exact_rows(), s->inv_norms, s->exact_dtype(), s->ld, s->dim, s->size, q_dev, c.q_dtype, c.nq, c.k, c.sum_mode,
-                 nullptr, (double *)w.xs.p, (uint32_t *)w.xr.p, (int32_t *)w.xc.p, (uint8_t *)w.taken.p, XCTAS, fin, s->cum,
-                 (int *)w.done.p};
     if (!(c.flags & FLAG_INTERNAL_CAPTURE)) { ++s->n_batches; s->n_queries += c.nq; }
     int launches = 0;
     if (c.stats) { c.stats->uncertified = 0; c.stats->candidates = 0; c.stats->scan_ctas = 0; }
@@ -726,6 +754,24 @@
         else if (kp_simt > 0) { kernel = 1; kp = kp_simt; }
         else if (tc_ok) { kernel = 2; kp = kp_tc; }
     }
+
+#ifdef VIDMEM_NO_GRAPH_PDL
+    const bool pdl = !(c.flags & (VM_FLAG_TIMING | FLAG_INTERNAL_CAPTURE));
+#else
+    const bool pdl = !(c.flags & VM_FLAG_TIMING);
+#endif
+    const bool pipelined = kernel != 0 && pdl && (c.flags & VM_FLAG_ASYNC) && !(c.flags & FLAG_INTERNAL_CAPTURE) && !c.sharded;
+    const int run = pipelined && s->pipe_stream == st ? s->pipe_run : 0;
+    unsigned seq = 0;
+    if (pipelined) { seq = ++s->seq; s->pipe_run = run < 2 ? run + 1 : 2; s->pipe_stream = st; }
+    else s->pipe_run = 0;
+    s->last_slot = pipelined ? (int)(seq & 1) : 0;
+    Slot &b = w.slot[s->last_slot];
+    ExactArgs ex{s->exact_rows(), s->inv_norms, s->exact_dtype(), s->ld, s->dim, s->size, q_dev, c.q_dtype, c.nq, c.k, c.sum_mode,
+                 nullptr, (double *)b.xs.p, (uint32_t *)b.xr.p, (int32_t *)b.xc.p, (uint8_t *)b.taken.p, XCTAS, fin, s->cum,
+                 (int *)b.done.p};
+    if (pipelined) { ex.call_done = s->call_done; ex.call_seq = seq; }
+
     if (kernel == 0) {
         int rc = k_exact(ex, st, false);
         if (rc != VM_OK) return rc;
@@ -742,15 +788,11 @@
     int nq_pad = kernel == 2 ? ((c.nq + 15) & ~15) : c.nq;
     const int split = (kernel == 2 && s->dtype == VM_BF16 && !(c.flags & VM_FLAG_NO_SPLIT) &&
                        (c.nq <= 48 || (c.flags & VM_FLAG_SPLIT)) && scan_tc_supported(s->dtype, s->dim, c.nq, kp, 1)) ? 1 : 0;
-#ifdef VIDMEM_NO_GRAPH_PDL
-    const bool pdl = !(c.flags & (VM_FLAG_TIMING | FLAG_INTERNAL_CAPTURE));
-#else
-    const bool pdl = !(c.flags & VM_FLAG_TIMING);
-#endif
-    int rc = k_normalize_queries(q_dev, c.q_dtype, c.nq, nq_pad, s->dim, s->ld, (float *)w.q_f32.p,
-                                 (kernel == 2 && s->dtype == VM_BF16) ? w.q_bf16.p : nullptr,
-                                 (int32_t *)w.flags.p + c.nq, kernel == 2 ? (uint32_t *)w.seed.p : nullptr,
-                                 kernel == 2 ? (int)(w.seed.bytes / 4) : 0, kernel == 2 && s->dtype == VM_F32, split, pdl, st);
+    int rc = k_normalize_queries(q_dev, c.q_dtype, c.nq, nq_pad, s->dim, s->ld, (float *)b.q_f32.p,
+                                 (kernel == 2 && s->dtype == VM_BF16) ? b.q_bf16.p : nullptr,
+                                 (int32_t *)b.flags.p + c.nq, kernel == 2 ? (uint32_t *)b.seed.p : nullptr,
+                                 kernel == 2 ? SEED_BLOCK_WORDS : 0, kernel == 2 && s->dtype == VM_F32, split, pdl,
+                                 run >= 2 ? s->call_done : nullptr, seq - 2, st);
     if (rc != VM_OK) return rc;
     ++launches;
     const double eps = scan_eps(kernel, s->dtype, s->dim, split, s->rows_exact != nullptr);
@@ -758,9 +800,10 @@
     ScanArgs a;
     ScanInfo sinfo;
     a.rows = s->rows; a.inv_norms = s->inv_norms; a.dtype = s->dtype; a.n = s->size; a.dim = s->dim; a.ld = s->ld;
-    a.queries = (const float *)w.q_f32.p; a.nq = c.nq; a.kp = kp; a.cand = (uint64_t *)w.cand.p; a.stream = st;
-    a.slab = (uint64_t *)w.cand.p; a.scnt = (int *)w.scnt.p;
-    a.ubuf = (uint64_t *)w.ubuf.p; a.ucnt = (int *)w.seed.p + SEED_TAB_WORDS + 2 * MAXQ; a.ucap = SCAN_UNION_CAP;
+    a.queries = (const float *)b.q_f32.p; a.nq = c.nq; a.kp = kp; a.cand = (uint64_t *)b.cand.p; a.stream = st;
+    a.slab = (uint64_t *)b.cand.p; a.scnt = (int *)b.scnt.p;
+    a.ubuf = (uint64_t *)b.ubuf.p; a.ucnt = (int *)b.seed.p + SEED_TAB_WORDS + 2 * MAXQ; a.ucap = SCAN_UNION_CAP;
+    a.tile_ctr = (int *)b.seed.p + SEED_TILE_CTR;
     a.band = nextafterf((float)(2.0 * eps), INFINITY); a.ksel = c.k; a.split = split; a.pdl = pdl;
     const bool timing = (c.flags & VM_FLAG_TIMING) != 0;
     if (timing) {
@@ -780,32 +823,33 @@
         a.ctas = (int)imin64(tiles, s->sm_count);
 
         a.dump = tiles <= s->sm_count && tiles * SCAN_DUMP_TILE <= SCAN_DUMP_MAX_KEYS &&
-                 (size_t)tiles * c.nq * SCAN_DUMP_TILE * 8 <= w.cand.bytes &&
+                 (size_t)tiles * c.nq * SCAN_DUMP_TILE * 8 <= b.cand.bytes &&
                  select_rescore_fits((int)tiles, SCAN_DUMP_TILE, kp, s->exact_dtype(), s->dim, s->ld);
         s->last_band_ctas = a.dump ? 0 : a.ctas; s->last_band_nq = c.nq;
-        rc = launch_scan_tc(a, s->dtype == VM_BF16 ? w.q_bf16.p : w.q_f32.p, (uint32_t *)w.seed.p, (int *)w.flags.p + c.nq + 1, nullptr, &sinfo);
+        rc = launch_scan_tc(a, s->dtype == VM_BF16 ? b.q_bf16.p : b.q_f32.p, (uint32_t *)b.seed.p, (int *)b.flags.p + c.nq + 1, nullptr, &sinfo);
         launches += 1;
     }
     if (rc != VM_OK) return rc;
     if (timing) { VM_CUDA_CHECK(cudaEventRecord(s->evr[s->ev_cur][1], st)); s->timed = true; }
 
-    int32_t *flags = (int32_t *)w.flags.p;
+    int32_t *flags = (int32_t *)b.flags.p;
     int32_t *uncert = flags + c.nq;
-    RescoreArgs rs{(const uint64_t *)w.merged.p, kp, s->exact_rows(), s->inv_norms, s->exact_dtype(), s->ld, s->dim, s->size, q_dev,
+    RescoreArgs rs{(const uint64_t *)b.merged.p, kp, s->exact_rows(), s->inv_norms, s->exact_dtype(), s->ld, s->dim, s->size, q_dev,
                    c.q_dtype, c.nq, eps, c.sum_mode, fin, flags, uncert, s->extreme,
-                   kernel == 2 ? (float *)w.col_thr.p : nullptr, s->cum};
+                   kernel == 2 ? (float *)b.col_thr.p : nullptr, s->cum};
+    if (run >= 1) { rs.call_done = s->call_done; rs.call_need = seq - 1; }
     SelectArgs sel;
     const bool union_src = kernel == 2 && !a.dump;
     if (union_src) {
         sel.slab = a.slab; sel.scnt = a.scnt; sel.ctas = a.ctas; sel.ubuf = a.ubuf; sel.ucnt = a.ucnt; sel.ucap = a.ucap;
-        sel.seed_tab = a.ctas <= 256 ? (const uint32_t *)w.seed.p : nullptr; sel.nq_pad = nq_pad; sel.ksel = c.k; sel.band = a.band;
+        sel.seed_tab = a.ctas <= 256 ? (const uint32_t *)b.seed.p : nullptr; sel.nq_pad = nq_pad; sel.ksel = c.k; sel.band = a.band;
     } else { sel.cand = a.cand; sel.lists = a.ctas; sel.list_len = a.dump ? SCAN_DUMP_TILE : kp; sel.complete = a.dump ? 1 : 0; }
     rc = k_select_rescore(sel, rs, st, pdl);
     if (rc == VM_ERR_UNSUPPORTED && !a.dump) {
-        if (union_src) rc = k_slab_top(sel, c.nq, kp, (uint64_t *)w.merged.p, (int *)w.sel_inc.p, st);
-        else rc = k_merge_candidates(a.cand, a.ctas, c.nq, kp, (uint64_t *)w.merged.p, st);
+        if (union_src) rc = k_slab_top(sel, c.nq, kp, (uint64_t *)b.merged.p, (int *)b.sel_inc.p, st);
+        else rc = k_merge_candidates(a.cand, a.ctas, c.nq, kp, (uint64_t *)b.merged.p, st);
         if (rc != VM_OK) return rc;
-        rc = k_rescore(rs, st, union_src ? (const int *)w.sel_inc.p : nullptr);
+        rc = k_rescore(rs, st, union_src ? (const int *)b.sel_inc.p : nullptr);
         ++launches;
     }
     if (rc != VM_OK) return rc;
@@ -814,11 +858,13 @@
     ex.flags = flags;
     int n_uncert = 0, n_full = -1;
     auto run_collect = [&]() -> int {
-        VM_CUDA_CHECK(cudaMemsetAsync(w.col_cnt.p, 0, (size_t)c.nq * 4, st));
-        ScanCollect sc{(const float *)w.col_thr.p, (uint64_t *)w.col_buf.p, (int *)w.col_cnt.p, COLLECT_CAP, uncert};
-        int r = launch_scan_tc(a, s->dtype == VM_BF16 ? w.q_bf16.p : w.q_f32.p, nullptr, nullptr, &sc);
+        VM_CUDA_CHECK(cudaMemsetAsync(b.col_cnt.p, 0, (size_t)c.nq * 4, st));
+        ScanCollect sc{(const float *)b.col_thr.p, (uint64_t *)b.col_buf.p, (int *)b.col_cnt.p, COLLECT_CAP, uncert};
+        ScanArgs ac = a;
+        ac.tile_ctr = a.tile_ctr + 1;
+        int r = launch_scan_tc(ac, s->dtype == VM_BF16 ? b.q_bf16.p : b.q_f32.p, nullptr, nullptr, &sc);
         if (r != VM_OK) return r;
-        return k_collect_rescore((const uint64_t *)w.col_buf.p, (const int *)w.col_cnt.p, COLLECT_CAP, rs, st);
+        return k_collect_rescore((const uint64_t *)b.col_buf.p, (const int *)b.col_cnt.p, COLLECT_CAP, rs, st);
     };
     if (c.flags & VM_FLAG_ASYNC) {
         if (c.flags & FLAG_INTERNAL_CAPTURE) {
@@ -929,6 +975,7 @@
     }
     memcpy(w.h_q, c.queries, (size_t)c.nq * s->dim * dtype_size(c.q_dtype));
     ++s->n_batches; s->n_queries += c.nq;
+    s->pipe_run = 0;
     VM_CUDA_CHECK(cudaGraphLaunch(ge->exec, s->gstream));
     VM_CUDA_CHECK(wait_stream(s->gstream, s));
     const int uncertified = ge->stats.scan_kernel != 0 ? *w.h_uncert : 0;
@@ -1009,6 +1056,7 @@
             if (sharded) c.flags |= VM_FLAG_ASYNC;
             else c.h = out_b;
         }
+        c.sharded = sharded;
         if ((rc = topk_batch(c)) != VM_OK) return rc;
         if (!sharded) continue;
         const ResultBlock ws = ResultBlock::at(w.o_idx.p, nb, k);
diff --git a/real-time-brain-inspired-video-memory_b200/csrc/common.cuh b/real-time-brain-inspired-video-memory_b200/csrc/common.cuh
--- a/real-time-brain-inspired-video-memory_b200/csrc/common.cuh
+++ b/real-time-brain-inspired-video-memory_b200/csrc/common.cuh
@@ -29,6 +29,25 @@
 __device__ __forceinline__ void pdl_wait() { asm volatile("griddepcontrol.wait;" ::: "memory"); }
 __device__ __forceinline__ void pdl_launch_dependents() { asm volatile("griddepcontrol.launch_dependents;" ::: "memory"); }
 
+__device__ __forceinline__ void wait_call_done(const unsigned *done, unsigned need)
+{
+    unsigned long long t0;
+    asm volatile("mov.u64 %0, %%globaltimer;" : "=l"(t0));
+    for (;;) {
+        unsigned v;
+        asm volatile("ld.acquire.gpu.global.u32 %0, [%1];" : "=r"(v) : "l"(done) : "memory");
+        if ((int)(v - need) >= 0) return;
+        __nanosleep(256);
+        unsigned long long t;
+        asm volatile("mov.u64 %0, %%globaltimer;" : "=l"(t));
+        if (t - t0 > 120000000000ull) __trap();
+    }
+}
+__device__ __forceinline__ void publish_call_done(unsigned *done, unsigned seq)
+{
+    asm volatile("st.release.gpu.global.u32 [%0], %1;" ::"l"(done), "r"(seq) : "memory");
+}
+
 template <typename... KArgs, typename... Args>
 static inline cudaError_t launch_pdl(void (*kernel)(KArgs...), dim3 grid, dim3 block, size_t smem, cudaStream_t st, bool pdl,
                                      Args &&...args)
@@ -84,6 +103,8 @@
 __host__ __device__ __forceinline__ float key_score(uint64_t k) { return f32_from_ordered((uint32_t)(k >> 32)); }
 
 static constexpr int SEED_TAB_WORDS = 256 * 64;
+static constexpr int SEED_TILE_CTR = SEED_TAB_WORDS + 3 * 64;
+static constexpr int SEED_BLOCK_WORDS = SEED_TILE_CTR + 4;
 #ifdef __CUDACC__
 __device__ __forceinline__ float seed_select(const uint32_t *seed_tab, int G, int nq_pad, int q, int k, int lane)
 {
@@ -210,6 +231,7 @@
     int ksel = 0;
     int split = 0;
     bool pdl = false;
+    int *tile_ctr = nullptr;
 };
 static constexpr int SCAN_UNION_CAP = 16384;
 static constexpr int SCAN_SLAB = 128;
@@ -256,6 +278,8 @@
     const int *extreme;
     float *collect_thr;
     unsigned long long *cum = nullptr;
+    const unsigned *call_done = nullptr;
+    unsigned call_need = 0;
 };
 struct SelectArgs {
     const uint64_t *cand = nullptr;
@@ -287,6 +311,8 @@
     FinalizeArgs fin;
     unsigned long long *cum = nullptr;
     int *done_ctr = nullptr;
-};
-
-}
+    unsigned *call_done = nullptr;
+    unsigned call_seq = 0;
+};
+
+}
diff --git a/real-time-brain-inspired-video-memory_b200/csrc/scan_tc.cu b/real-time-brain-inspired-video-memory_b200/csrc/scan_tc.cu
--- a/real-time-brain-inspired-video-memory_b200/csrc/scan_tc.cu
+++ b/real-time-brain-inspired-video-memory_b200/csrc/scan_tc.cu
@@ -10,6 +10,15 @@
 static constexpr int TC_THREADS = 192;
 static constexpr int TC_TMEM_COLS = 512;
 static constexpr int TC_MAX_STAGES = 8;
+static constexpr int TC_RING = 32;
+
+__device__ __forceinline__ int ring_tile(const uint64_t *ring, int j)
+{
+    const volatile uint64_t *p = ring + (j & (TC_RING - 1));
+    uint64_t v;
+    while ((uint32_t)((v = *p) >> 32) != (uint32_t)j) {}
+    return (int)(uint32_t)v;
+}
 
 struct CollectArgs {
     const float *thr;
@@ -32,7 +41,7 @@
 
 struct TcLayout {
     int nq_pad, KB, stages, split;
-    uint32_t off_b, off_a, off_tauf, off_lcnt, off_cmax, off_wmax, off_flags, off_bars, off_tmem, total;
+    uint32_t off_b, off_a, off_tauf, off_lcnt, off_cmax, off_wmax, off_flags, off_bars, off_ring, off_tmem, total;
 };
 
 static TcLayout make_layout(int dtype, int ld, int nq, int split = 0)
@@ -44,7 +53,7 @@
     L.split = (split && dtype == VM_BF16) ? 1 : 0;
     uint32_t o = 0;
     L.off_b = o; o += (uint32_t)L.KB * L.nq_pad * 128 * (L.split ? 2 : 1);
-    const uint32_t epi = (uint32_t)L.nq_pad * (4 + 4 + 4 + 16) + 64 + 8 * (2 * TC_MAX_STAGES + 1 + 2 * TC_ACC) + 16;
+    const uint32_t epi = (uint32_t)L.nq_pad * (4 + 4 + 4 + 16) + 64 + 8 * (2 * TC_MAX_STAGES + 1 + 2 * TC_ACC) + 8 * TC_RING + 16;
     int64_t room = 227 * 1024 - 2048 - (int64_t)o - epi;
     L.stages = (int)(room / TC_STAGE_BYTES);
     if (L.stages > TC_MAX_STAGES) L.stages = TC_MAX_STAGES;
@@ -56,6 +65,7 @@
     L.off_wmax = o; o += (uint32_t)L.nq_pad * 16;
     L.off_flags = o; o += 64;
     L.off_bars = o; o += 8 * (2 * TC_MAX_STAGES + 1 + 2 * TC_ACC);
+    L.off_ring = o; o += 8 * TC_RING;
     L.off_tmem = o; o += 16;
     L.total = o + 1024;
 #ifdef VIDMEM_AB_SMEMPAD
@@ -95,7 +105,8 @@
 __global__ void __launch_bounds__(DUMP ? TC_THREADS : TC_THREADS_SVC, 1)
 scan_tc_kernel(const __grid_constant__ CUtensorMap tmA, const __grid_constant__ CUtensorMap tmB,
                const float *__restrict__ inv_norms, int64_t n, int num_tiles, int nq, TcLayout L, uint64_t *__restrict__ dump_keys,
-               uint32_t *__restrict__ seed_tab, int *__restrict__ seed_ctr, CollectArgs col, BandArgs ub, int svc_sleep)
+               uint32_t *__restrict__ seed_tab, int *__restrict__ seed_ctr, CollectArgs col, BandArgs ub, int svc_sleep,
+               int *__restrict__ tile_ctr)
 {
     const bool collect = !DUMP && col.thr != nullptr;
 #ifndef VIDMEM_AB_NOPDL
@@ -119,11 +130,14 @@
     uint64_t *full = bars, *empty = bars + TC_MAX_STAGES, *qfull = bars + 2 * TC_MAX_STAGES;
     uint64_t *tfull = qfull + 1, *tempty = tfull + TC_ACC;
     uint32_t *tmem_slot = (uint32_t *)(base + L.off_tmem);
+    uint64_t *ring = (uint64_t *)(base + L.off_ring);
 
     const int warp = __shfl_sync(0xffffffffu, threadIdx.x >> 5, 0);
     const int lane = threadIdx.x & 31;
     const int nq_pad = L.nq_pad, KB = L.KB, stages = L.stages;
     constexpr int ELEMS = TF32 ? 32 : 64;
+    const int tile0 = (int)blockIdx.x < num_tiles ? (int)blockIdx.x : -1;
+    const int pre = !collect && tile0 >= 0 ? (stages < KB ? stages : KB) : 0;
 
     if (warp == 0 && lane == 0) {
         tma_prefetch_desc(&tmA);
@@ -132,7 +146,13 @@
         mbar_init(qfull, 1);
         for (int a = 0; a < TC_ACC; ++a) { mbar_init(&tfull[a], 1); mbar_init(&tempty[a], 4); }
         fence_barrier_init();
-    }
+        for (int kb = 0; kb < pre; ++kb) {
+            mbar_arrive_expect_tx(&full[kb], TC_STAGE_BYTES);
+            tma_load_2d(&tmA, &full[kb], sA + (size_t)kb * TC_STAGE_BYTES, kb * ELEMS, tile0 * TC_BLOCK_M, L2_EVICT_FIRST);
+        }
+    }
+    if (warp == 0) ring[lane] = ~0ull;
+    static_assert(TC_RING == 32, "one ring slot per lane of warp 0");
     if (warp == 1) tmem_alloc(tmem_slot, TC_TMEM_COLS);
 #ifndef VIDMEM_AB_NOPDL
     if (!collect) pdl_wait();
@@ -161,10 +181,18 @@
                     tma_load_2d(&tmB, qfull, sB + (size_t)(part * KB + kb) * nq_pad * 128, kb * ELEMS, part * nq_pad, L2_EVICT_LAST);
         }
         __syncwarp();
-        int stage = 0;
-        uint32_t phase = 0;
-        for (int tile = blockIdx.x; tile < num_tiles; tile += gridDim.x) {
-            for (int kb = 0; kb < KB; ++kb) {
+        int stage = pre == stages ? 0 : pre;
+        uint32_t phase = pre == stages ? 1u : 0u;
+        for (int j = 0;; ++j) {
+            int tile = 0;
+            if (lane == 0) {
+                tile = j == 0 ? tile0 : (DUMP ? blockIdx.x + j * (int)gridDim.x : (int)gridDim.x + atomicAdd(tile_ctr, 1));
+                if (tile >= num_tiles) tile = -1;
+                *(volatile uint64_t *)(ring + (j & (TC_RING - 1))) = ((uint64_t)(uint32_t)j << 32) | (uint32_t)tile;
+            }
+            tile = __shfl_sync(0xffffffffu, tile, 0);
+            if (tile < 0) break;
+            for (int kb = j == 0 ? pre : 0; kb < KB; ++kb) {
                 mbar_wait(&empty[stage], phase ^ 1);
                 if (elect_one()) {
                     mbar_arrive_expect_tx(&full[stage], TC_STAGE_BYTES);
@@ -182,7 +210,7 @@
         uint32_t phase = 0, acc_phase = 0;
         const uint64_t da0 = make_smem_desc_sw128(smem_u32(sA)), db0 = make_smem_desc_sw128(smem_u32(sB));
         const uint32_t kb_step = (uint32_t)(nq_pad * 128) >> 4, lo_step = (uint32_t)(KB * nq_pad * 128) >> 4;
-        for (int tile = blockIdx.x; tile < num_tiles; tile += gridDim.x) {
+        for (int j = 0; ring_tile(ring, j) >= 0; ++j) {
             mbar_wait(&tempty[acc], acc_phase ^ 1);
             tc_fence_after();
             const uint32_t d_tmem = tmem_base + (uint32_t)(acc * nq_pad);
@@ -212,7 +240,7 @@
         int acc = 0;
         uint32_t acc_phase = 0;
         if constexpr (DUMP) {
-            for (int tile = blockIdx.x; tile < num_tiles; tile += gridDim.x) {
+            for (int j = 0, tile; (tile = ring_tile(ring, j)) >= 0; ++j) {
                 const int64_t r = (int64_t)tile * TC_BLOCK_M + row_in_tile;
                 const float iv = r < n ? __ldg(inv_norms + r) : -1.0f;
                 mbar_wait(&tfull[acc], acc_phase);
@@ -235,19 +263,24 @@
             }
         } else {
         if (ub.use_seed && !collect) {
-            const int64_t row0 = (int64_t)blockIdx.x * TC_BLOCK_M + row_in_tile;
-            const float inv0 = row0 < n ? __ldg(inv_norms + row0) : -1.0f;
-            mbar_wait(&tfull[0], 0);
-            tc_fence_after();
+            const int tile0 = ring_tile(ring, 0);
+            const int64_t row0 = (int64_t)tile0 * TC_BLOCK_M + row_in_tile;
+            const float inv0 = tile0 >= 0 && row0 < n ? __ldg(inv_norms + row0) : -1.0f;
+            if (tile0 >= 0) {
+                mbar_wait(&tfull[0], 0);
+                tc_fence_after();
+            }
             const uint32_t taddr0 = tmem_base + ((uint32_t)(quad * 32) << 16);
             for (int c = 0; c < nq_pad; c += 16) {
                 uint32_t v[16];
-                tmem_ld16(taddr0 + c, v);
-                tmem_ld_wait();
+                if (tile0 >= 0) {
+                    tmem_ld16(taddr0 + c, v);
+                    tmem_ld_wait();
+                }
 #pragma unroll
                 for (int j = 0; j < 16; ++j) {
                     const float sc = inv0 >= 0.0f ? __uint_as_float(v[j]) * inv0 : -INFINITY;
-                    const uint32_t mx = __reduce_max_sync(0xffffffffu, f32_ordered(sc));
+                    const uint32_t mx = tile0 >= 0 ? __reduce_max_sync(0xffffffffu, f32_ordered(sc)) : 0u;
                     if (lane == 0) wmax[(warp - 2) * nq_pad + c + j] = mx;
                 }
             }
@@ -296,11 +329,13 @@
         }
         if (!collect && e == 0) s_done[1] = 1;
         uint64_t *my_slab = collect ? nullptr : ub.slab + (size_t)blockIdx.x * nq * SCAN_SLAB;
-        int64_t row = (int64_t)blockIdx.x * TC_BLOCK_M + row_in_tile;
-        float inv = row < n ? __ldg(inv_norms + row) : -1.0f;
-        for (int tile = blockIdx.x; tile < num_tiles; tile += gridDim.x) {
-            const int64_t row_next = row + (int64_t)gridDim.x * TC_BLOCK_M;
-            const float inv_next = (tile + (int)gridDim.x < num_tiles && row_next < n) ? __ldg(inv_norms + row_next) : -1.0f;
+        int tile = ring_tile(ring, 0);
+        int64_t row = (int64_t)tile * TC_BLOCK_M + row_in_tile;
+        float inv = tile >= 0 && row < n ? __ldg(inv_norms + row) : -1.0f;
+        for (int j = 0; tile >= 0; ++j) {
+            const int tile_next = ring_tile(ring, j + 1);
+            const int64_t row_next = (int64_t)tile_next * TC_BLOCK_M + row_in_tile;
+            const float inv_next = (tile_next >= 0 && row_next < n) ? __ldg(inv_norms + row_next) : -1.0f;
             const bool valid = inv >= 0.0f;
             mbar_wait(&tfull[acc], acc_phase);
             tc_fence_after();
@@ -370,6 +405,7 @@
             __syncwarp();
             if (lane == 0) mbar_arrive(&tempty[acc]);
             if (++acc == TC_ACC) { acc = 0; acc_phase ^= 1; }
+            tile = tile_next;
             row = row_next;
             inv = inv_next;
         }
@@ -507,13 +543,14 @@
 #else
     const int svc_sleep = a.dtype == VM_F32 ? 500 : 200;
 #endif
+    VM_REQUIRE(dump || a.tile_ctr, VM_ERR_BADARG, "tcgen05 scan: tile counter missing");
     if (info && !sc) { info->stages = L.stages; info->variant = dump ? 1 : 2; }
     const bool pdl = a.pdl && !sc;
 #ifdef VIDMEM_AB_CLASSIC_LAUNCH
-#define LAUNCH_IMPL(TF, DU, SP) scan_tc_kernel<TF, DU, SP><<<a.ctas, DU ? TC_THREADS : TC_THREADS_SVC, L.total, a.stream>>>(tmA, tmB, a.inv_norms, a.n, num_tiles, a.nq, L, a.cand, seed_tab, seed_ctr, col, ub, svc_sleep)
+#define LAUNCH_IMPL(TF, DU, SP) scan_tc_kernel<TF, DU, SP><<<a.ctas, DU ? TC_THREADS : TC_THREADS_SVC, L.total, a.stream>>>(tmA, tmB, a.inv_norms, a.n, num_tiles, a.nq, L, a.cand, seed_tab, seed_ctr, col, ub, svc_sleep, a.tile_ctr)
 #else
 #define LAUNCH_IMPL(TF, DU, SP) VM_CUDA_CHECK(launch_pdl(scan_tc_kernel<TF, DU, SP>, dim3(a.ctas), dim3(DU ? TC_THREADS : TC_THREADS_SVC), L.total, a.stream, pdl, \
-                                 tmA, tmB, a.inv_norms, a.n, num_tiles, a.nq, L, a.cand, seed_tab, seed_ctr, col, ub, svc_sleep))
+                                 tmA, tmB, a.inv_norms, a.n, num_tiles, a.nq, L, a.cand, seed_tab, seed_ctr, col, ub, svc_sleep, a.tile_ctr))
 #endif
 #define LAUNCH_TC(TF, DU, SP)                                                                                                \
     do {                                                                                                                   \
diff --git a/real-time-brain-inspired-video-memory_b200/csrc/select.cu b/real-time-brain-inspired-video-memory_b200/csrc/select.cu
--- a/real-time-brain-inspired-video-memory_b200/csrc/select.cu
+++ b/real-time-brain-inspired-video-memory_b200/csrc/select.cu
@@ -572,7 +572,8 @@
                                                                    FinalizeArgs f, int32_t *__restrict__ flags,
                                                                    int32_t *__restrict__ uncertified_count,
                                                                    const int *__restrict__ extreme, float *__restrict__ collect_thr,
-                                                                   unsigned long long *__restrict__ cum, const float *__restrict__ inv_norms)
+                                                                   unsigned long long *__restrict__ cum, const float *__restrict__ inv_norms,
+                                                                   const unsigned *__restrict__ call_done, unsigned call_need)
 {
     extern __shared__ __align__(16) unsigned char sr_smem[];
     uint64_t *skeys = reinterpret_cast<uint64_t *>(sr_smem);
@@ -597,6 +598,7 @@
     if (tid == 0) { s_m = 0; s_nz = 0; s_cnt = 0; s_band = 0; s_viol = 0; s_thr = -INFINITY; }
     if (tid < 64) s_top[tid] = 0;
     pdl_wait();
+    if (call_done && tid == 0) wait_call_done(call_done, call_need);
     __syncthreads();
 
     const bool union_mode = src.slab != nullptr;
@@ -951,17 +953,31 @@
 static constexpr int XS_CG = 24;
 static constexpr int XS_PITCH = XS_CG * 16 + 16;
 
-template <bool NEUMAIER, typename T>
+template <bool NEUMAIER, typename T, bool LEAN>
 __global__ void __launch_bounds__(XS_THREADS) exact_scan_kernel(const T *__restrict__ rows, const float *__restrict__ inv_norms,
                                                                int64_t n, int ld, int dim, const void *__restrict__ queries,
                                                                int q_dtype, int nq, int32_t *__restrict__ flags, int k,
                                                                double *__restrict__ xlist_score, uint32_t *__restrict__ xlist_row,
                                                                int32_t *__restrict__ xlist_cnt, unsigned long long *__restrict__ cum,
-                                                               int *__restrict__ done_ctr, FinalizeArgs f, uint8_t *__restrict__ taken)
+                                                               int *__restrict__ done_ctr, FinalizeArgs f, uint8_t *__restrict__ taken,
+                                                               unsigned *__restrict__ call_done, unsigned call_seq)
 {
     pdl_launch_dependents();
     pdl_wait();
-    if (flags && flags[nq] == 0) return;
+    const bool work = !(flags && flags[nq] == 0);
+    if (!work) {
+        if (call_done == nullptr) return;
+        __syncthreads();
+        if (threadIdx.x == 0) {
+            int t;
+            asm volatile("atom.acq_rel.gpu.global.add.s32 %0, [%1], 1;" : "=r"(t) : "l"(done_ctr) : "memory");
+            if (t == (int)gridDim.x - 1) {
+                *done_ctr = 0;
+                publish_call_done(call_done, call_seq);
+            }
+        }
+        return;
+    }
     if (flags && cum && blockIdx.x == 0 && threadIdx.x == 0) atomicAdd(cum + 3, (unsigned long long)flags[nq]);
     extern __shared__ __align__(16) unsigned char xs_smem[];
     double *sq = reinterpret_cast<double *>(xs_smem);
@@ -992,6 +1008,54 @@
         __syncthreads();
         const double n1 = s_n1;
         const int64_t ntiles = (n + 127) / 128;
+        auto tile_done = [&](int64_t r, bool live) {
+            double sc = 0.0;
+            bool hit = false;
+            if (live && !is_rr) {
+                const double n2 = __dsqrt_rn(s_rrv[rt]);
+                sc = (n1 == 0.0 || n2 == 0.0) ? 0.0 : __ddiv_rn(s_dotv[rt], __dmul_rn(n1, n2));
+                const int lc = l_cnt;
+                hit = lc < k || better(sc, (uint32_t)r, l_score[lc - 1], l_row[lc - 1]);
+            }
+            if (hit) {
+                const int p = atomicAdd(&c_cnt, 1);
+                c_score[p] = sc;
+                c_row[p] = (uint32_t)r;
+            }
+            const int cc = __syncthreads_count(hit ? 1 : 0);
+            const int lc = l_cnt;
+            if (cc > 0) {
+                for (int e = tid; e < lc + cc; e += XS_THREADS) {
+                    const double se = e < lc ? l_score[e] : c_score[e - lc];
+                    const uint32_t re = e < lc ? l_row[e] : c_row[e - lc];
+                    int rank = 0;
+                    for (int i = 0; i < lc; ++i) rank += better(l_score[i], l_row[i], se, re) ? 1 : 0;
+                    for (int i = 0; i < cc; ++i) rank += better(c_score[i], c_row[i], se, re) ? 1 : 0;
+                    if (rank < k) { n_score[rank] = se; n_row[rank] = re; }
+                }
+                __syncthreads();
+                const int nl = min(k, lc + cc);
+                for (int e = tid; e < nl; e += XS_THREADS) { l_score[e] = n_score[e]; l_row[e] = n_row[e]; }
+                if (tid == 0) { l_cnt = nl; c_cnt = 0; }
+                __syncthreads();
+            }
+        };
+        if constexpr (LEAN) {
+            for (int64_t tile = blockIdx.x; tile < ntiles; tile += gridDim.x) {
+                const int64_t r = tile * 128 + rt;
+                const bool live = r < n && inv_norms[r] >= 0.0f;
+                if (live) {
+                    const T *row = rows + r * (int64_t)ld;
+                    RefSum acc;
+                    acc.init();
+                    if (!is_rr) ref_sum_range<NEUMAIER>(acc, 0, dim, [&](int i) { return __dmul_rn(sq[i], load_elem(row, i)); });
+                    else ref_sum_range<NEUMAIER>(acc, 0, dim, [&](int i) { const double y = load_elem(row, i); return __dmul_rn(y, y); });
+                    if (is_rr) s_rrv[rt] = acc.result<NEUMAIER>(); else s_dotv[rt] = acc.result<NEUMAIER>();
+                }
+                __syncthreads();
+                tile_done(r, live);
+            }
+        } else {
         const int my_tiles = (int)((ntiles - blockIdx.x + gridDim.x - 1) / gridDim.x);
         const int total_steps = my_tiles > 0 ? my_tiles * nchunks : 0;
         auto issue = [&](int st) {
@@ -1038,38 +1102,10 @@
             if (live) { if (is_rr) s_rrv[rt] = acc.result<NEUMAIER>(); else s_dotv[rt] = acc.result<NEUMAIER>(); }
             acc.init();
             __syncthreads();
-            double sc = 0.0;
-            bool hit = false;
-            if (live && !is_rr) {
-                const double n2 = __dsqrt_rn(s_rrv[rt]);
-                sc = (n1 == 0.0 || n2 == 0.0) ? 0.0 : __ddiv_rn(s_dotv[rt], __dmul_rn(n1, n2));
-                const int lc = l_cnt;
-                hit = lc < k || better(sc, (uint32_t)r, l_score[lc - 1], l_row[lc - 1]);
-            }
-            if (hit) {
-                const int p = atomicAdd(&c_cnt, 1);
-                c_score[p] = sc;
-                c_row[p] = (uint32_t)r;
-            }
-            const int cc = __syncthreads_count(hit ? 1 : 0);
-            const int lc = l_cnt;
-            if (cc > 0) {
-                for (int e = tid; e < lc + cc; e += XS_THREADS) {
-                    const double se = e < lc ? l_score[e] : c_score[e - lc];
-                    const uint32_t re = e < lc ? l_row[e] : c_row[e - lc];
-                    int rank = 0;
-                    for (int i = 0; i < lc; ++i) rank += better(l_score[i], l_row[i], se, re) ? 1 : 0;
-                    for (int i = 0; i < cc; ++i) rank += better(c_score[i], c_row[i], se, re) ? 1 : 0;
-                    if (rank < k) { n_score[rank] = se; n_row[rank] = re; }
-                }
-                __syncthreads();
-                const int nl = min(k, lc + cc);
-                for (int e = tid; e < nl; e += XS_THREADS) { l_score[e] = n_score[e]; l_row[e] = n_row[e]; }
-                if (tid == 0) { l_cnt = nl; c_cnt = 0; }
-                __syncthreads();
-            }
+            tile_done(r, live);
         }
         cp_async_wait<0>();
+        }
         __syncthreads();
         const int lc = l_cnt;
         const int64_t base = ((int64_t)blockIdx.x * nq + q) * k;
@@ -1092,7 +1128,15 @@
         exact_merge_query<XS_THREADS>(xlist_score, xlist_row, xlist_cnt, (int)gridDim.x, nq, k, q, f, taken, w_s, w_r, w_p, &s_out);
         if (tid == 0) flags[q] = 0;
     }
-    if (tid == 0) { *done_ctr = 0; flags[nq] = 0; }
+    __syncthreads();
+    if (tid == 0) {
+        *done_ctr = 0;
+        flags[nq] = 0;
+        if (call_done) {
+            __threadfence();
+            publish_call_done(call_done, call_seq);
+        }
+    }
 }
 
 __global__ void __launch_bounds__(256) exact_merge_kernel(const double *__restrict__ xlist_score, const uint32_t *__restrict__ xlist_row,
@@ -1356,7 +1400,7 @@
         VM_CUDA_CHECK((max_smem_once<select_rescore_kernel<NEU, T>>(180 * 1024)));
         VM_CUDA_CHECK(launch_pdl(select_rescore_kernel<NEU, T>, dim3(a.nq), dim3(SR_THREADS), smem, st, pdl, src, a.nq, a.kp,
                                  (const T *)a.rows, a.ld, a.dim, a.n_rows, a.queries, a.q_dtype, a.eps, a.fin, a.flags,
-                                 a.uncertified_count, a.extreme, a.collect_thr, a.cum, a.inv_norms));
+                                 a.uncertified_count, a.extreme, a.collect_thr, a.cum, a.inv_norms, a.call_done, a.call_need));
         VM_CUDA_CHECK(cudaGetLastError());
         return VM_OK;
     });
@@ -1392,15 +1436,28 @@
 int k_exact(const ExactArgs &a, cudaStream_t st, bool pdl)
 {
     VM_REQUIRE((size_t)a.dim * sizeof(double) <= 40 * 1024, VM_ERR_UNSUPPORTED, "exact scan: dim %d too large", a.dim);
-    const size_t smem = (size_t)((a.dim + 1) & ~1) * sizeof(double) + (size_t)3 * 128 * XS_PITCH + 16;
     const bool conditional = a.flags != nullptr && a.done_ctr != nullptr;
+    const bool lean = conditional && pdl;
+    const size_t smem = (size_t)((a.dim + 1) & ~1) * sizeof(double) + (lean ? 0 : (size_t)3 * 128 * XS_PITCH) + 16;
     const int rc = with_row_type(a.dtype, a.sum_mode, [&](auto neu, auto *tag) -> int {
         using T = std::remove_pointer_t<decltype(tag)>;
         constexpr bool NEU = decltype(neu)::value;
-        VM_CUDA_CHECK((max_smem_once<exact_scan_kernel<NEU, T>>(200 * 1024)));
-        VM_CUDA_CHECK(launch_pdl(exact_scan_kernel<NEU, T>, dim3(a.ctas), dim3(XS_THREADS), smem, st, pdl && conditional, (const T *)a.rows,
-                                 a.inv_norms, a.n, a.ld, a.dim, a.queries, a.q_dtype, a.nq, a.flags, a.k, a.xlist_score, a.xlist_row,
-                                 a.xlist_cnt, a.cum, conditional ? a.done_ctr : (int *)nullptr, a.fin, a.taken));
+        auto launch = [&](auto kernel) -> int {
+            VM_CUDA_CHECK(launch_pdl(kernel, dim3(a.ctas), dim3(XS_THREADS), smem, st, pdl && conditional, (const T *)a.rows,
+                                     a.inv_norms, a.n, a.ld, a.dim, a.queries, a.q_dtype, a.nq, a.flags, a.k, a.xlist_score, a.xlist_row,
+                                     a.xlist_cnt, a.cum, conditional ? a.done_ctr : (int *)nullptr, a.fin, a.taken,
+                                     conditional ? a.call_done : (unsigned *)nullptr, a.call_seq));
+            return VM_OK;
+        };
+        int r;
+        if (lean) {
+            VM_CUDA_CHECK((max_smem_once<exact_scan_kernel<NEU, T, true>>(48 * 1024)));
+            r = launch(exact_scan_kernel<NEU, T, true>);
+        } else {
+            VM_CUDA_CHECK((max_smem_once<exact_scan_kernel<NEU, T, false>>(200 * 1024)));
+            r = launch(exact_scan_kernel<NEU, T, false>);
+        }
+        if (r != VM_OK) return r;
         VM_CUDA_CHECK(cudaGetLastError());
         return VM_OK;
     });
diff --git a/real-time-brain-inspired-video-memory_b200/csrc/store.cu b/real-time-brain-inspired-video-memory_b200/csrc/store.cu
--- a/real-time-brain-inspired-video-memory_b200/csrc/store.cu
+++ b/real-time-brain-inspired-video-memory_b200/csrc/store.cu
@@ -70,10 +70,11 @@
 __global__ void normalize_queries_kernel(const void *__restrict__ q, int q_dtype, int nq, int nq_pad, int dim, int ld,
                                          float *__restrict__ out_f32, __nv_bfloat16 *__restrict__ out_bf16,
                                          int32_t *__restrict__ zero_me, uint32_t *__restrict__ zero_tab, int zero_tab_n,
-                                         int tf32_round, int split)
+                                         int tf32_round, int split, const unsigned *__restrict__ call_done, unsigned call_need)
 {
     pdl_launch_dependents();
-    pdl_wait();
+    if (call_done) wait_call_done(call_done, call_need);
+    else pdl_wait();
     if (zero_me && blockIdx.x == 0 && threadIdx.x < 2) zero_me[threadIdx.x] = 0;
     for (int i = blockIdx.x * blockDim.x + threadIdx.x; i < zero_tab_n; i += gridDim.x * blockDim.x) zero_tab[i] = 0u;
     int lane = threadIdx.x & 31;
@@ -171,12 +172,12 @@
 
 int k_normalize_queries(const void *q, int q_dtype, int nq, int nq_pad, int dim, int ld, float *out_f32,
                         void *out_bf16, int32_t *zero_me, uint32_t *zero_tab, int zero_tab_n, int tf32_round, int split, bool pdl,
-                        cudaStream_t st)
+                        const unsigned *call_done, unsigned call_need, cudaStream_t st)
 {
     int threads = 128;
     int grid = (nq_pad * 32 + threads - 1) / threads;
     VM_CUDA_CHECK(launch_pdl(normalize_queries_kernel, dim3(grid), dim3(threads), 0, st, pdl, q, q_dtype, nq, nq_pad, dim, ld, out_f32,
-                             (__nv_bfloat16 *)out_bf16, zero_me, zero_tab, zero_tab_n, tf32_round, split));
+                             (__nv_bfloat16 *)out_bf16, zero_me, zero_tab, zero_tab_n, tf32_round, split, call_done, call_need));
     VM_CUDA_CHECK(cudaGetLastError());
     return VM_OK;
 }
```

After: 264,700, median of 6. 1.02x the previous value.
